# robotvisionmu/DenseMonoSLAM

Hardware: AMD Instinct MI355X
Metric: frames/sec ICP+RGB+fusion @640x480 (higher is better)
Workload: dtype f32; 1 GPU; TUM fr1/desk-like 640x480 full 3-level ICP+RGB tracking (SO3 + {10,5,4} GN iterations) + surfel index-map fusion; synthetic box-room RGB-D stream, loop closure off (--o), NID keyframing off (--nkf); cameras_per_gpu=1, n_pred=2, n_pred_project_passes=1, surfels_per_map=246557, surfels_total=246557, exchange=none (1 camera)

## Files before the change

densemonoslam_amd/csrc/fill.hpp:

```cpp
#pragma once
#include "surfel.hpp"

namespace dms {

struct FillArgs {
  const float4* ex_vertex;
  const float4* ex_normal;
  const uchar4* ex_image;
  const unsigned short* depth;
  const uchar4* rgba;
  const unsigned* mirror_src;
  unsigned* mirror_dst;
  int mirror_words;
  int* dense_flag;
  int rows_blocks;
  unsigned* dense_cnt;
  const unsigned* sample_mask;
  unsigned char* thumb_block;
  const unsigned* thumb_mask;
  int thumb_w, thumb_h;
  const float* thumb_pose_src;
  float* thumb_pose_dst;
  int* thumb_tick_dst;
  int thumb_tick;
  float4* out_vertex;
  float4* out_normal;
  uchar4* out_image;
  int cols, rows;
  float cx, cy, ifx, ify;
  int pass_geom, pass_rgb;
};

__device__ __forceinline__ f3 fill_vertex_at(const FillArgs& a, int sx, int sy, int x, int y) {
  const float z = (float)a.depth[(size_t)sy * a.cols + sx] / 1000.0f;
  return mk3((((float)x - a.cx) * z) * a.ifx, (((float)y - a.cy) * z) * a.ify, z);
}

__device__ __forceinline__ void fill_pixel_out(const FillArgs& a, int px, int py, const float4& sv, const float4& sn, const uchar4& si, float4& ov,
                                               float4& on, uchar4& oi) {
  const size_t i = (size_t)py * a.cols + px;
  const float colsf = (float)a.cols, rowsf = (float)a.rows;
  const float tcx = ((float)px + 0.5f) / colsf, tcy = ((float)py + 0.5f) / rowsf;
  const int x = (int)(tcx * colsf), y = (int)(tcy * rowsf);
  {
    if (sv.z == 0.f || a.pass_geom == 1) {
      const f3 v = fill_vertex_at(a, px, py, x, y);
      ov = make_float4(v.x, v.y, v.z, 1.f);
    } else {
      ov = sv;
    }
    a.out_vertex[i] = ov;
  }
  {
    if (sn.z == 0.f || a.pass_geom == 1) {
      const f3 v = fill_vertex_at(a, px, py, x, y);
      const int sxp = texel(tcx + (1.0f / colsf), colsf, a.cols);
      const int syp = texel(tcy + (1.0f / rowsf), rowsf, a.rows);
      const f3 vx = fill_vertex_at(a, sxp, py, x + 1, y);
      const f3 vy = fill_vertex_at(a, px, syp, x, y + 1);
      const f3 n = normalized3(cross3(vx - v, vy - v));
      on = make_float4(n.x, n.y, n.z, 1.f);
    } else {
      on = sn;
    }
    a.out_normal[i] = on;
  }
  {
    if ((si.x == 0 && si.y == 0 && si.z == 0) || a.pass_rgb == 1)
      oi = a.rgba[i];
    else
      oi = si;
    a.out_image[i] = oi;
  }
}
__device__ __forceinline__ void fill_pixel(const FillArgs& a, int px, int py, const float4& sv, const float4& sn, const uchar4& si) {
  float4 ov, on;
  uchar4 oi;
  fill_pixel_out(a, px, py, sv, sn, si, ov, on, oi);
}

__device__ __forceinline__ void fill_thumb(const FillArgs& a, int px, int py, const float4& ov, const float4& on, const uchar4& oi) {
  const unsigned cw = a.thumb_mask[px >> 5], rw = a.thumb_mask[64 + (py >> 5)];
  if (!((cw >> (px & 31)) & (rw >> (py & 31)) & 1u)) return;
  const int i = (int)a.thumb_mask[128 + (px >> 5)] + __popc(cw & ((1u << (px & 31)) - 1u));
  const int j = (int)a.thumb_mask[192 + (py >> 5)] + __popc(rw & ((1u << (py & 31)) - 1u));
  const size_t n = (size_t)a.thumb_w * a.thumb_h, k = (size_t)j * a.thumb_w + i;
  reinterpret_cast<uchar4*>(a.thumb_block)[k] = oi;
  reinterpret_cast<float4*>(a.thumb_block + thumb_vertex_off(n))[k] = ov;
  reinterpret_cast<float4*>(a.thumb_block + thumb_normal_off(n))[k] = on;
}

inline bool thumb_sample_masks(int cols, int rows, unsigned* words256) {
  for (int i = 0; i < 256; ++i) words256[i] = 0u;
  const int tw = cols / 8, th = rows / 8;
  if (tw < 1 || th < 1 || cols > 2048 || rows > 2048) return false;
  int last = -1;
  for (int i = 0; i < tw; ++i) {
    const int sx = texel(((float)i + 0.5f) / (float)tw, (float)cols, cols);
    if (sx <= last) return false;
    last = sx;
    words256[sx >> 5] |= 1u << (sx & 31);
  }
  last = -1;
  for (int j = 0; j < th; ++j) {
    const int sy = texel(((float)j + 0.5f) / (float)th, (float)rows, rows);
    if (sy <= last) return false;
    last = sy;
    words256[64 + (sy >> 5)] |= 1u << (sy & 31);
  }
  for (int w = 1; w < 64; ++w) {
    words256[128 + w] = words256[128 + w - 1] + (unsigned)__builtin_popcount(words256[w - 1]);
    words256[192 + w] = words256[192 + w - 1] + (unsigned)__builtin_popcount(words256[64 + w - 1]);
  }
  return true;
}

inline void fill_sample_masks(int cols, int rows, unsigned* words128) {
  for (int i = 0; i < 128; ++i) words128[i] = 0u;
  const int dw = cols / 20, dh = rows / 20;
  for (int i = 0; i < dw; ++i) {
    const int sx = texel(((float)i + 0.5f) / (float)dw, (float)cols, cols);
    words128[sx >> 5] |= 1u << (sx & 31);
  }
  for (int j = 0; j < dh; ++j) {
    const int sy = texel(((float)j + 0.5f) / (float)dh, (float)rows, rows);
    words128[64 + (sy >> 5)] |= 1u << (sy & 31);
  }
}

template <int NT>
__device__ __forceinline__ void fill_dense_test(const FillArgs& a, int t, int* s_sum ) {
  const int dw = a.cols / 20, dh = a.rows / 20;
  int sum = 0;
  for (int k = t; k < dw * dh; k += NT) {
    const int i = k % dw, j = k / dw;
    const float u = ((float)i + 0.5f) / (float)dw, v = ((float)j + 0.5f) / (float)dh;
    const int sx = texel(u, (float)a.cols, a.cols), sy = texel(v, (float)a.rows, a.rows);
    const uchar4 c = a.ex_image[(size_t)sy * a.cols + sx];
    sum += (c.x > 0 && c.y > 0 && c.z > 0) ? 1 : 0;
  }
  for (int off = 32; off > 0; off >>= 1) sum += __shfl_down(sum, off, 64);
  if ((t & 63) == 0) s_sum[t >> 6] = sum;
  __syncthreads();
  if (t == 0) {
    int tot = 0;
    for (int w = 0; w < NT / 64; ++w) tot += s_sum[w];
    const bool dense = (float)tot / (float)(dh * dw) > 0.95f;
    *a.dense_flag = dense ? 0 : 1;
  }
}

__device__ __forceinline__ int dense_from_counters(const unsigned* cnt, int samples) {
  unsigned tot = 0;
#pragma unroll
  for (int k = 0; k < 16; ++k) tot += cnt[k * 16];
  return ((float)(int)tot / (float)samples > 0.95f) ? 0 : 1;
}

}
```

densemonoslam_amd/csrc/fusion_frame.hip:

```cpp
#include <atomic>
#include <chrono>
#include <map>
#include <string>
#include <vector>

#include "../../include/dmslam_render_cloud.h"
#include "internal.hpp"
#include "host_util.hpp"
#include "late_frame.hpp"
#include "smallmath.hpp"
#include "surfel.hpp"
#include "canon.hpp"
#include "frame_state.hpp"
#include "live_bodies.hpp"
#include "fill.hpp"
#include "track_init.hpp"

namespace dms {

__global__ void k_rgb_to_rgba(const unsigned char* __restrict__ rgb, uchar4* __restrict__ rgba, int n) {
  for (int i = blockIdx.x * blockDim.x + threadIdx.x; i < n; i += blockDim.x * gridDim.x)
    rgba[i] = make_uchar4(rgb[3 * i + 0], rgb[3 * i + 1], rgb[3 * i + 2], 255);
}

// ... 153 lines not shown
  char* gloop = nullptr;
  char* h_gloop = nullptr;
  size_t gloop_bytes = 0;
  LoopState* loop = nullptr;
  char* h_loop = nullptr;
  size_t loop_bytes = 0;
  char* arena = nullptr;
  size_t arena_bytes = 0;
  struct LiveImages {
    dms_image2d rgba, depth_raw, depth_filtered, depth_metric, depth_metric_filtered;
  } live[2];
  dms_image2d rgba, depth_raw, depth_filtered, depth_metric, depth_metric_filtered;
  hipStream_t s_prep = nullptr;
  hipEvent_t ev_prep_done[2] = {nullptr, nullptr}, ev_main_done[4] = {nullptr, nullptr, nullptr, nullptr}, ev_inputs = nullptr;
  bool fused_live = true;
  int prep_blocks = 38;
  LateFrame late;
  int late_owner = -1;
  double host_wait_prep_ms = 0.0;
  int host_lag = 2;
  bool inputs_armed = false;
  int last_prep = -1;
  long frames = 0;
  dms_image2d kf_img[DMS_NUM_PYRS], kf_dmap[DMS_NUM_PYRS], kf_old_img[DMS_NUM_PYRS], kf_old_dmap[DMS_NUM_PYRS];
  void* nid_ws = nullptr;
  size_t nid_ws_bytes = 0;
  float* nid_host = nullptr;
  int frames_since_fusion = 0;
  float last_nid = 0.f;
  bool loop_solver = false;
  int graph_sample_rate = 5000;
  dms_deform* deform = nullptr;
  int deforms = 0;
  std::vector<float> relative_cons;
  bool in_frame = false, cur_bootstrap = false, cur_fuse_now = true;
  int live_set = 0, lastnext_set = 0;
  bool prev_handed_on = false;
  bool tracking_ok = true, lost = false;
  int tracking_count = 0;
  int cur_k2 = 0;
  dms_image2d depth_synth;
  dms_indexmap_out imap;
  dms_predict_out pred, fill;
  void* rgba_tmp = nullptr;
  void* untr = nullptr;
  unsigned long long* zbuf = nullptr;
  unsigned long long* zbuf2 = nullptr;
  unsigned long long* zbuf_assoc = nullptr;
  bool zbuf_assoc_dirty = false;
  bool zbuf_assoc_keep_dirty = false;
  unsigned* tickets = nullptr;
  bool fold_track_init = true;
  bool dense_by_counters = false;
  double host_wait_ms = 0.0;
  bool pre_valid = false;
  int pre_tick = 0;
  unsigned long pre_version = 0;
  struct LazyRecord {
    bool pending = false;
    float confidence = 0.f, maxDepth = 0.f;
    int tick = 0, timeIdx = 0, timeDelta = 0;
    int pass_geom = 0, pass_rgb = 0;
    dms_image2d depth_filtered, rgba;
    dms_model* model = nullptr;
    unsigned long version = 0;
    hipStream_t stream = nullptr;
  } lazy;
  dms_pose_block* lazy_pose = nullptr;
  bool lazy_observed = false;
  long lazy_deferred = 0, lazy_materialised = 0, lazy_stale = 0;
  FrameState* state = nullptr;
  FrameState* h_state_dev = nullptr;
  FrameState* h_state = nullptr;
  int last_slot = 0;
  int timeouts_reported = 0;
  int range_failures_reported = 0;
  void* h_track = nullptr;
  int tick = 1;
  bool map_initialised = false;
  int fused_last = 0;
  bool profiling = false;
  StageClock clock;
};

namespace {

dms_image2d mk_img(void* p, int rows, int cols, size_t elem) {
  dms_image2d i;
  i.data = p;
  i.pitch = (size_t)cols * elem;
  i.rows = rows;
  i.cols = cols;
  return i;
}

void layout(dms_fusion* f, Carver& c) {
  const int W = f->p.width, H = f->p.height;
  const size_t N = (size_t)W * H;
  for (int k = 0; k < 2; ++k) {
    f->live[k].rgba = mk_img(c.take(N * 4), H, W, 4);
    f->live[k].depth_raw = mk_img(c.take(N * 2), H, W, 2);
    f->live[k].depth_filtered = mk_img(c.take(N * 2), H, W, 2);
    f->live[k].depth_metric = mk_img(c.take(N * 4), H, W, 4);
    f->live[k].depth_metric_filtered = mk_img(c.take(N * 4), H, W, 4);
  }
  f->rgba = f->live[0].rgba;
// ... 1 lines not shown
  f->depth_filtered = f->live[0].depth_filtered;
  f->depth_metric = f->live[0].depth_metric;
  f->depth_metric_filtered = f->live[0].depth_metric_filtered;
  f->fb_rgba = mk_img(c.take(N * 4), H, W, 4);
  f->fb_dm = mk_img(c.take(N * 4), H, W, 4);
  f->fb_dmf = mk_img(c.take(N * 4), H, W, 4);
  f->imap.index = mk_img(c.take(N * 4), H, W, 4);
  f->imap.vertConf = mk_img(c.take(N * 16), H, W, 16);
  f->imap.colorTime = mk_img(c.take(N * 16), H, W, 16);
  f->imap.normRad = mk_img(c.take(N * 16), H, W, 16);
  f->pred.image = mk_img(c.take(N * 4), H, W, 4);
  f->pred.vertex = mk_img(c.take(N * 16), H, W, 16);
  f->pred.normal = mk_img(c.take(N * 16), H, W, 16);
  f->pred.time = mk_img(c.take(N * 2), H, W, 2);
  f->fill.image = mk_img(c.take(N * 4), H, W, 4);
  f->fill.vertex = mk_img(c.take(N * 16), H, W, 16);
  f->fill.normal = mk_img(c.take(N * 16), H, W, 16);
  f->fill.time = f->pred.time;
  for (int l = 0; l < DMS_NUM_PYRS; ++l) {
    const int h = H >> l, w = W >> l;
    f->kf_img[l] = mk_img(c.take((size_t)h * w), h, w, 1);
    f->kf_dmap[l] = mk_img(c.take((size_t)h * w * 4), h, w, 4);
    f->kf_old_img[l] = mk_img(c.take((size_t)h * w), h, w, 1);
    f->kf_old_dmap[l] = mk_img(c.take((size_t)h * w * 4), h, w, 4);
  }
  {
    const int nb = f->p.nid_bins_depth > f->p.nid_bins_img ? f->p.nid_bins_depth : f->p.nid_bins_img;
    f->nid_ws_bytes = nid_workspace_bytes(nb > 0 ? nb : 1);
    f->nid_ws = c.take(f->nid_ws_bytes);
  }
  memset(&f->pred_old, 0, sizeof(f->pred_old));
  if (f->p.local_loop_closure || f->p.hybrid_loops) {
    f->pred_old.image = mk_img(c.take(N * 4), H, W, 4);
    f->pred_old.vertex = mk_img(c.take(N * 16), H, W, 16);
    f->pred_old.normal = mk_img(c.take(N * 16), H, W, 16);
    f->pred_old.time = mk_img(c.take(N * 2), H, W, 2);
  }
  if (f->p.hybrid_loops) {
    f->gloop_bytes = 256 + (size_t)(W / 20) * (H / 20) * 8 * sizeof(float);
    f->gloop = (char*)c.take(f->gloop_bytes);
    f->orb_pose = (dms_pose_block*)c.take(2 * sizeof(dms_pose_block));
  }
  if (f->p.local_loop_closure) {
    f->loop_bytes = up256(sizeof(LoopState)) + (size_t)(W / 20) * (H / 20) * 8 * sizeof(float);
    f->loop = (LoopState*)c.take(f->loop_bytes);
  }
  f->depth_synth = mk_img(c.take(N * 4), H, W, 4);
  f->rgba_tmp = c.take(N * 4);
  f->untr = c.take(N * 16);
  f->zbuf = (unsigned long long*)c.take(N * 8);
  f->zbuf2 = (unsigned long long*)c.take(N * 8);
  f->zbuf_assoc = (unsigned long long*)c.take(N * 8);
  f->tickets = (unsigned*)c.take(2048 + 512 + 1024);
  f->state = (FrameState*)c.take(sizeof(FrameState));
  f->lazy_pose = (dms_pose_block*)c.take(sizeof(dms_pose_block));
}

void drain(dms_fusion* f) {
  static const bool timeline = getenv("DMS_TIMELINE") != nullptr;
  if (timeline && !f->clock.pending.empty()) {
    hipEvent_t base = f->clock.pending.front().start;
    for (auto& p : f->clock.pending) {
      float a = 0.f, b = 0.f;
      (void)hipEventElapsedTime(&a, base, p.start);
      (void)hipEventElapsedTime(&b, base, p.stop);
      fprintf(stderr, "[timeline] %-14s %9.3f -> %9.3f ms\n", p.name.c_str(), a, b);
    }
  }
  f->clock.drain();
}

enum class Predict { view, final, tracking };
struct PredictOpts {
  float confidence;
  void* state_mirror = nullptr;
  bool one_call = false;
  bool have_prior = false;
  const TrackInitArgs* track_init = nullptr;
  bool* track_init_taken = nullptr;
};

int predict_body(dms_fusion* f, hipStream_t s, Predict kind, const PredictOpts& o) {
  const bool dense_test = kind == Predict::tracking;
  int rc;
  f->lazy.pending = false;
  FillArgs fa;
  const FillArgs* fused = nullptr;
  if ((rc = fill_args(&f->pred, &f->depth_filtered, &f->rgba, &f->cam, f->lost ? 1 : 0, (f->lost || f->p.frameToFrameRGB) ? 1 : 0, &f->fill,
                      o.state_mirror ? f->state : nullptr, o.state_mirror, (int)sizeof(FrameState), dense_test ? &f->state->fill_in : nullptr, &fa)))
    return rc;
  f->dense_by_counters = false;
  if (f->p.fused_fill_in && f->p.width <= 2048 && f->p.height <= 2048 && (!dense_test || f->p.hybrid_tracking)) {
    fused = &fa;
    if (dense_test) {
      fa.dense_cnt = f->tickets;
      fa.sample_mask = f->tickets + 512;
      f->dense_by_counters = true;
    }
    if (kind == Predict::final && f->armed_now.block && f->thumb_masks_ok) {
      fa.thumb_block = f->armed_now.block;
      fa.thumb_mask = f->tickets + 640;
      fa.thumb_w = f->p.width / 8;
      fa.thumb_h = f->p.height / 8;
      fa.thumb_pose_src = f->state->cur.pose;
      fa.thumb_pose_dst = f->armed_now.pose_dst;
      fa.thumb_tick_dst = f->armed_now.tick_dst;
      fa.thumb_tick = f->armed_now.tick;
      f->armed_written = true;
    }
  }
  {
    StageTimer t(f->clock, s, "predict", f->profiling);
    const int W = f->p.width, H = f->p.height;
    bool done = false;
    if (kind == Predict::tracking && f->pre_valid) {
      if (!o.have_prior && f->pre_tick == f->tick && f->pre_version == f->model->version) {
        if ((rc = splat_predict(f->model, &f->state->cur, &f->cam, f->p.maxDepthProcessed, o.confidence, f->tick, f->p.timeIdx, f->tick,
                                f->p.timeDelta, 1, f->zbuf2, &f->pred, nullptr, 1, s, nullptr, nullptr, 1, fused, fused ? o.track_init : nullptr)))
          return rc;
        done = true;
      } else if ((rc = clear_zbuf(f->zbuf2, W * H, s))) {
        return rc;
      }
      f->pre_valid = false;
    }
    if (!done) {
      const int next_tick = f->lost ? f->tick : f->tick + 1;
      const float second[3] = {0.7f, (float)next_tick, (float)next_tick};
      const bool dual = kind == Predict::final && f->p.share_projection && f->p.hybrid_tracking && f->model->sharers == 1;
      if (dual && f->pre_valid && (rc = clear_zbuf(f->zbuf2, W * H, s))) return rc;
      const bool defer = dual && o.one_call && fused && o.state_mirror && f->p.lazy_final_prediction && !f->lazy_observed && !f->armed_now.block &&
                         !f->p.nid_keyframing && !f->p.local_loop_closure && !f->p.hybrid_loops && !f->lost && !f->cur_bootstrap;
      if (defer) {
        const ProjectRider rider = {(const unsigned*)f->state, (unsigned*)o.state_mirror, (int)(sizeof(FrameState) / 4),
                                    (const unsigned*)&f->state->cur, (unsigned*)f->lazy_pose, (int)(sizeof(dms_pose_block) / 4)};
        if ((rc = splat_project_only(f->model, &f->state->cur, &f->cam, f->p.maxDepthProcessed, second[0], next_tick, f->p.timeIdx, next_tick,
                                     f->p.timeDelta, 1, f->zbuf2, s, &rider)))
          return rc;
        dms_fusion::LazyRecord& r = f->lazy;
        r.pending = true;
        r.confidence = o.confidence;
        r.maxDepth = f->p.maxDepthProcessed;
        r.tick = f->tick;
        r.timeIdx = f->p.timeIdx;
        r.timeDelta = f->p.timeDelta;
        r.pass_geom = 0;
        r.pass_rgb = f->p.frameToFrameRGB ? 1 : 0;
        r.depth_filtered = f->depth_filtered;
        r.rgba = f->rgba;
        r.model = f->model;
        r.version = f->model->version;
        r.stream = s;
        f->lazy_deferred += 1;
      } else if ((rc = splat_predict(f->model, &f->state->cur, &f->cam, f->p.maxDepthProcessed, o.confidence, f->tick, f->p.timeIdx, f->tick,
                              f->p.timeDelta, 1, f->zbuf, &f->pred, nullptr, 1, s, dual ? second : nullptr, dual ? f->zbuf2 : nullptr, 0,
                              fused, fused ? o.track_init : nullptr)))
        return rc;
      if (dual) {
        f->pre_valid = true;
        f->pre_tick = next_tick;
        f->pre_version = f->model->version;
      }
    }
  }
  if (o.track_init_taken) *o.track_init_taken = fused != nullptr && o.track_init && o.track_init->blocks > 0;
  if (!fused) {
    StageTimer t(f->clock, s, "fill_in", f->profiling);
    if ((rc = fill_in(&f->pred, &f->depth_filtered, &f->rgba, &f->cam, f->lost ? 1 : 0, (f->lost || f->p.frameToFrameRGB) ? 1 : 0, &f->fill,
                      s, o.state_mirror ? f->state : nullptr, o.state_mirror, (int)sizeof(FrameState), dense_test ? &f->state->fill_in : nullptr)))
      return rc;
  }
  return DMS_OK;
}

int predict_view(dms_fusion* f, float confidence, hipStream_t s) { return predict_body(f, s, Predict::view, PredictOpts{confidence}); }

int predict_tracking(dms_fusion* f, hipStream_t s, bool have_prior, const TrackInitArgs* track_init, bool* track_init_taken) {
  return predict_body(f, s, Predict::tracking, PredictOpts{0.7f, nullptr, false, have_prior, track_init, track_init_taken});
}

int predict_final(dms_fusion* f, hipStream_t s, void* state_mirror, bool one_call) {
  return predict_body(f, s, Predict::final, PredictOpts{f->p.confidence, state_mirror, one_call});
}

int materialise_final_prediction(dms_fusion* f, hipStream_t consumer, bool consumer_known) {
  f->lazy_observed = true;
  if (!f->lazy.pending) return DMS_OK;
  const dms_fusion::LazyRecord r = f->lazy;
  f->lazy.pending = false;
  f->lazy_materialised += 1;
  if (r.model != f->model || r.version != f->model->version) f->lazy_stale += 1;
  int rc;
  FillArgs fa;
  if ((rc = fill_args(&f->pred, &r.depth_filtered, &r.rgba, &f->cam, r.pass_geom, r.pass_rgb, &f->fill, nullptr, nullptr, 0, nullptr, &fa))) return rc;
  {
    StageTimer t(f->clock, r.stream, "predict", f->profiling);
    if ((rc = splat_predict(f->model, f->lazy_pose, &f->cam, r.maxDepth, r.confidence, r.tick, r.timeIdx, r.tick, r.timeDelta, 1, f->zbuf, &f->pred,
                            nullptr, 1, r.stream, nullptr, nullptr, 0, &fa, nullptr)))
      return rc;
  }
  if (!consumer_known || consumer != r.stream) DMS_HIP(hipStreamSynchronize(r.stream));
  return DMS_OK;
}

int global_loop_device(dms_fusion* f, const float* orbTcwOld, const float* orbTcwNew, int active_new, hipStream_t s) {
  int rc;
  Pose16 a, b;
  memcpy(a.v, orbTcwOld, sizeof(a.v));
  memcpy(b.v, orbTcwNew, sizeof(b.v));
  hipLaunchKernelGGL(k_pose_blocks2, dim3(1), dim3(64), 0, s, f->orb_pose, a, b);
  DMS_CHECK_LAUNCH();
  f->lazy.pending = false;
  StageTimer t(f->clock, s, "global_loop", f->profiling);
  const int act = active_new ? 1 : 0;
  if ((rc = splat_predict(f->model, f->orb_pose + act, &f->cam, f->p.maxDepthProcessed, f->p.confidence, f->tick, f->p.timeIdx, f->tick,
                          f->p.timeDelta, 1, f->zbuf, &f->pred, nullptr, 1, s)))
    return rc;
  if ((rc = splat_predict(f->model, f->orb_pose + (1 - act), &f->cam, f->p.maxDepthProcessed, f->p.confidence, 0, f->p.timeIdx,
                          f->tick - f->p.timeDelta, f->p.timeDelta, 0, f->zbuf, &f->pred_old, nullptr, 1, s)))
    return rc;
  hipLaunchKernelGGL(k_global_loop_constraints, dim3(1), dim3(256), 0, s, (const float4*)f->pred.vertex.data,
                     (const unsigned short*)f->pred_old.time.data, f->p.width, f->p.height, f->p.maxDepthProcessed, f->orb_pose, active_new ? 1 : 0,
                     (int*)f->gloop, (float*)(f->gloop + 256));
  DMS_CHECK_LAUNCH();
  DMS_HIP(hipMemcpyAsync(f->h_gloop, f->gloop, f->gloop_bytes, hipMemcpyDeviceToHost, s));
  f->gloop_ran = true;
  return DMS_OK;
}

}

// ... 46 lines not shown
                           unsigned char* slot_flag, unsigned int* winner, size_t winner_count, dms_stream s) {
  return model_fuse_scratch(m, slot_pos4, slot_col4, slot_nrm4, slot_best, slot_flag, winner, winner_count, (hipStream_t)s);
}
int dms_model_clean(dms_model* m, const dms_pose_block* pose, int time, int timeIdx, const dms_indexmap_out* im,
                    const dms_image2d* depth_synth, const dms_camera* cam, float confThreshold, const float* graph_host, int graph_nodes,
                    int timeDelta, float maxDepth, int isFern, dms_stream s) {
  return model_clean(m, pose, time, timeIdx, im, depth_synth, cam, confThreshold, graph_host, graph_nodes, timeDelta, maxDepth, isFern, 0,
                     nullptr, (hipStream_t)s);
}
int dms_fill_in(const dms_predict_out* ex, const dms_image2d* d, const dms_image2d* rgba, const dms_camera* cam, int pg, int pr,
                dms_predict_out* out, dms_stream s) {
  return fill_in(ex, d, rgba, cam, pg, pr, out, (hipStream_t)s);
}
int dms_resize_nn(const dms_image2d* src, dms_image2d* dst, int elem, dms_stream s) { return resize_nn(src, dst, elem, (hipStream_t)s); }

void dms_fusion_default_params(dms_fusion_params* p, int width, int height, float fx, float fy, float cx, float cy) {
  if (!p) return;
  memset(p, 0, sizeof(*p));
  p->width = width;
  p->height = height;
  p->fx = fx;
  p->fy = fy;
  p->cx = cx;
  p->cy = cy;
  p->timeDelta = 200;
  p->confidence = 10.0f;
  p->depthCut = 3.0f;
  p->icpWeight = 10.0f;
  p->fastOdom = 0;
  p->so3 = 1;
  p->frameToFrameRGB = 0;
  p->pyramid = 1;
  p->hybrid_tracking = 1;
  p->rgbOnly = 0;
  p->timeIdx = 0;
  p->maxDepthProcessed = 25.0f;
  p->model_capacity = 0;
  p->pipeline_ingest = 1;
  p->global_predict = 0;
  p->nid_keyframing = 0;
  p->nid_threshold = 0.80f;
  p->nid_depth_lambda = 0.7f;
  p->nid_bins_img = 64;
  p->nid_bins_depth = 500;
  p->nid_pyramid_level = 0;
  p->local_loop_closure = 0;
  p->reloc = 0;
  p->num_sensors = 3;
  p->share_projection = 1;
  p->fused_fill_in = 1;
  p->hybrid_loops = 0;
  p->lazy_final_prediction = 1;
  p->fused_associate = 1;
}

static int set_depth_bias(dms_fusion* f) {
  const int b = canon::depth_exp_bias(f->p.depthCut);
  int rc = dms_odometry_debug_set(f->odom, "depth_exp_bias", b);
  if (!rc && f->odom_m2m) rc = dms_odometry_debug_set(f->odom_m2m, "depth_exp_bias", b);
  return rc;
}

static std::atomic<int> g_live_contexts{0};
int dms_fusion_allow_late_frame(dms_fusion* f, int allow) {
  DMS_REQUIRE(f && allow >= -1 && allow <= 1, "bad argument");
  f->late_owner = allow;
  return DMS_OK;
}

int dms_fusion_create(dms_fusion** out, const dms_fusion_params* p) {
  DMS_REQUIRE(out && p, "null argument");
  DMS_REQUIRE(p->width >= 40 && p->height >= 40, "resolution too small");
  DMS_REQUIRE(p->timeIdx >= 0 && p->timeIdx < DMS_MAX_SENSORS, "timeIdx out of range");
  DMS_REQUIRE(p->num_sensors >= 0 && p->num_sensors <= DMS_MAX_SENSORS, "num_sensors out of range");
  DMS_REQUIRE(p->timeIdx < (p->num_sensors == 0 ? 3 : p->num_sensors), "timeIdx must be one of the num_sensors time slots");
  DMS_REQUIRE(!p->nid_keyframing || (p->nid_bins_img >= 1 && p->nid_bins_img <= 256 && p->nid_bins_depth >= 1 && p->nid_bins_depth <= 4096 &&
                                     p->nid_pyramid_level >= 0 && p->nid_pyramid_level < DMS_NUM_PYRS),
              "bad NID key-framing parameters");
  dms_fusion* f = new dms_fusion();
  f->p = *p;
  f->cam.fx = p->fx;
  f->cam.fy = p->fy;
  f->cam.cx = p->cx;
  f->cam.cy = p->cy;
  if (f->p.num_sensors == 0) f->p.num_sensors = 3;
  int rc = dms_model_create(&f->model, p->model_capacity, p->width, p->height);
  if (rc) {
    delete f;
    return rc;
  }
  (void)dms_model_set_num_sensors(f->model, f->p.num_sensors);
  f->own_model = f->model;
  f->clusters[0] = f->model;
  rc = dms_odometry_create(&f->odom, p->width, p->height, p->cx, p->cy, p->fx, p->fy, 0.f, 0.f);
  if (rc) {
    dms_model_destroy(f->own_model ? f->own_model : f->model);
    delete f;
    return rc;
  }
  rc = odometry_enable_ring(f->odom);
  if (!rc && p->local_loop_closure) rc = dms_odometry_create(&f->odom_m2m, p->width, p->height, p->cx, p->cy, p->fx, p->fy, 0.f, 0.f);
  if (!rc) rc = set_depth_bias(f);
  if (!rc && f->odom_m2m) odometry_set_early_exit(f->odom_m2m, 1);
  if (rc) {
    dms_odometry_destroy(f->odom);
    dms_model_destroy(f->own_model ? f->own_model : f->model);
    delete f;
    return rc;
  }
  Carver sz;
  sz.pad = 16;
  layout(f, sz);
  f->arena_bytes = up256(sz.off);
  hipError_t e = hipMalloc((void**)&f->arena, f->arena_bytes);
  if (e == hipSuccess) {
    int prio = 1;
    if (const char* pp = getenv("DMS_PREP_PRIORITY")) prio = atoi(pp);
    int least = 0, greatest = 0;
    if (prio != 0 && hipDeviceGetStreamPriorityRange(&least, &greatest) == hipSuccess && least != greatest)
      e = hipStreamCreateWithPriority(&f->s_prep, hipStreamNonBlocking, prio > 0 ? least : greatest);
    else
      e = hipStreamCreateWithFlags(&f->s_prep, hipStreamNonBlocking);
  }
  for (int k = 0; k < 2 && e == hipSuccess; ++k) e = hipEventCreateWithFlags(&f->ev_prep_done[k], hipEventDisableTiming);
  for (int k = 0; k < 4 && e == hipSuccess; ++k) e = hipEventCreateWithFlags(&f->ev_main_done[k], hipEventDisableTiming);
  {
    const int tiles = ((p->width + 63) / 64) * ((p->height + 15) / 16);
    int cap = 40;
    const int free_cus = odometry_free_cus(f->odom);
    if (free_cus >= 16 && free_cus < cap) cap = free_cus;
    const int rounds = (tiles + cap - 1) / cap;
    f->prep_blocks = (tiles + rounds - 1) / rounds;
  }
  if (const char* pb = getenv("DMS_PREP_BLOCKS")) f->prep_blocks = atoi(pb);
  if (const char* fl = getenv("DMS_FUSED_LIVE")) f->fused_live = atoi(fl) != 0;
  if (const char* ft = getenv("DMS_FOLD_TRACK_INIT")) f->fold_track_init = atoi(ft) != 0;
  if (const char* hl = getenv("DMS_HOST_LAG")) f->host_lag = atoi(hl) == 3 ? 3 : 2;
  if (const char* lm = getenv("DMS_LATE_MAIN")) f->late.forced = atoi(lm) != 0 ? 1 : 0;
  if (const char* lz = getenv("DMS_LAZY_FINAL_PREDICTION")) f->p.lazy_final_prediction = atoi(lz) != 0 ? 1 : 0;
  if (const char* fa = getenv("DMS_FUSED_ASSOCIATE")) f->p.fused_associate = atoi(fa) != 0 ? 1 : 0;
  if (e == hipSuccess) e = hipEventCreateWithFlags(&f->ev_inputs, hipEventDisableTiming);
  if (e == hipSuccess) e = hipMemset(f->arena, 0, f->arena_bytes);
  if (e == hipSuccess) e = hipHostMalloc((void**)&f->h_state, 4 * sizeof(FrameState), hipHostMallocMapped);
  if (e == hipSuccess) e = hipHostGetDevicePointer((void**)&f->h_state_dev, f->h_state, 0);
  if (e == hipSuccess) e = hipHostMalloc((void**)&f->nid_host, 2 * sizeof(float), hipHostMallocDefault);
  if (e == hipSuccess && f->loop_bytes) {
    e = hipHostMalloc((void**)&f->h_loop, 4 * f->loop_bytes, hipHostMallocDefault);
    if (e == hipSuccess) memset(f->h_loop, 0, 4 * f->loop_bytes);
  }
  if (e == hipSuccess && f->gloop_bytes) {
    e = hipHostMalloc((void**)&f->h_gloop, f->gloop_bytes, hipHostMallocDefault);
    if (e == hipSuccess) memset(f->h_gloop, 0, f->gloop_bytes);
  }
  if (e != hipSuccess) {
    if (f->arena) (void)hipFree(f->arena);
    if (f->odom_m2m) dms_odometry_destroy(f->odom_m2m);
    dms_odometry_destroy(f->odom);
    dms_model_destroy(f->own_model ? f->own_model : f->model);
    delete f;
    return hip_fail(e, "dms_fusion_create allocation", __FILE__, __LINE__);
  }
  Carver c;
  c.base = f->arena;
  c.pad = 16;
  layout(f, c);
  {
    unsigned masks[128];
    fill_sample_masks(p->width < 2048 ? p->width : 2048, p->height < 2048 ? p->height : 2048, masks);
    (void)hipMemcpy(f->tickets + 512, masks, sizeof(masks), hipMemcpyHostToDevice);
    unsigned tm[256];
    f->thumb_masks_ok = thumb_sample_masks(p->width, p->height, tm);
    (void)hipMemcpy(f->tickets + 640, tm, sizeof(tm), hipMemcpyHostToDevice);
  }
  Pose16 I;
  for (int i = 0; i < 16; ++i) I.v[i] = (i % 5 == 0) ? 1.f : 0.f;
  hipLaunchKernelGGL(k_pose_set, dim3(1), dim3(64), 0, 0, f->state, I);
  (void)clear_zbuf(f->zbuf, p->width * p->height, 0);
  (void)clear_zbuf(f->zbuf2, p->width * p->height, 0);
  (void)clear_zbuf(f->zbuf_assoc, p->width * p->height, 0);
  for (int l = 0; l < DMS_NUM_PYRS; ++l)
    (void)hipMemsetD32((hipDeviceptr_t)f->kf_old_dmap[l].data, 0x7fffffff, (size_t)f->kf_old_dmap[l].rows * f->kf_old_dmap[l].cols);
  (void)hipDeviceSynchronize();
  memset(f->h_state, 0, 4 * sizeof(FrameState));
  g_live_contexts += 1;
  *out = f;
  return DMS_OK;
}

int dms_fusion_destroy(dms_fusion* f) {
  if (!f) return DMS_OK;
  g_live_contexts -= 1;
  (void)hipDeviceSynchronize();
  drain(f);
  for (int k = 0; k < 2; ++k)
    if (f->ev_prep_done[k]) (void)hipEventDestroy(f->ev_prep_done[k]);
  for (int k = 0; k < 4; ++k)
    if (f->ev_main_done[k]) (void)hipEventDestroy(f->ev_main_done[k]);
  if (f->ev_inputs) (void)hipEventDestroy(f->ev_inputs);
  if (f->s_prep) (void)hipStreamDestroy(f->s_prep);
  if (f->arena) (void)hipFree(f->arena);
  if (f->h_state) (void)hipHostFree(f->h_state);
  if (f->nid_host) (void)hipHostFree(f->nid_host);
  if (f->h_loop) (void)hipHostFree(f->h_loop);
  if (f->h_gloop) (void)hipHostFree(f->h_gloop);
  if (f->odom_m2m) dms_odometry_destroy(f->odom_m2m);
  if (f->deform) dms_deform_destroy(f->deform);
  dms_odometry_destroy(f->odom);
  dms_model* const own = f->own_model ? f->own_model : f->model;
  if (f->model && f->model != own) f->model->sharers -= 1;
  for (auto& kv : f->clusters)
    if (kv.second && kv.second != own) dms_model_destroy(kv.second);
  dms_model_destroy(own);
  delete f;
  return DMS_OK;
}

static int snapshot_feedback(dms_fusion* f, hipStream_t s) {
  const size_t N = (size_t)f->p.width * f->p.height;
  DMS_HIP(hipMemcpyAsync(f->fb_rgba.data, f->rgba.data, N * 4, hipMemcpyDeviceToDevice, s));
  DMS_HIP(hipMemcpyAsync(f->fb_dm.data, f->depth_metric.data, N * 4, hipMemcpyDeviceToDevice, s));
  DMS_HIP(hipMemcpyAsync(f->fb_dmf.data, f->depth_metric_filtered.data, N * 4, hipMemcpyDeviceToDevice, s));
  f->fb_time = f->tick;
  f->fb_valid = true;
  return DMS_OK;
}
// ... 207 lines not shown

static int join_prep_stream(dms_fusion* f, int k2, hipStream_t s, hipStream_t sp) {
  DMS_HIP(hipEventRecord(f->ev_prep_done[k2], sp));
  if (f->late.on) {
    const auto t0 = std::chrono::steady_clock::now();
    DMS_HIP(hipEventSynchronize(f->ev_prep_done[k2]));
    f->host_wait_prep_ms += std::chrono::duration<double, std::milli>(std::chrono::steady_clock::now() - t0).count();
  } else {
    DMS_HIP(hipStreamWaitEvent(s, f->ev_prep_done[k2], 0));
  }
  f->last_prep = k2;
  return DMS_OK;
}

static int bootstrap_frame(dms_fusion* f, const float* inPose16, hipStream_t s) {
  int rc;
  Pose16 prior;
  if (inPose16)
    memcpy(prior.v, inPose16, sizeof(prior.v));
  else
    for (int i = 0; i < 16; ++i) prior.v[i] = (i % 5 == 0) ? 1.f : 0.f;
  hipLaunchKernelGGL(k_pose_set, dim3(1), dim3(64), 0, s, f->state, prior);
  DMS_CHECK_LAUNCH();
  if (!f->adopting) {
    StageTimer t(f->clock, s, "initialise", f->profiling);
    if ((rc = model_initialise(f->model, &f->rgba, &f->depth_metric, &f->depth_metric_filtered, &f->cam, f->tick, f->p.timeIdx,
                               (float)(int)f->p.maxDepthProcessed, s)))
      return rc;
    if ((rc = snapshot_feedback(f, s))) return rc;
    if (f->req_cluster != f->cur_cluster && !f->clusters.count(f->req_cluster) && f->model == f->own_model) {
      f->clusters[f->cur_cluster] = nullptr;
      f->clusters[f->req_cluster] = f->model;
      f->cur_cluster = f->req_cluster;
    }
  }
  f->map_initialised = true;
  f->prev_handed_on = true;
  return DMS_OK;
}

static int track_frame(dms_fusion* f, const float* inPose16, float weightMultiplier, hipStream_t s) {
  int rc;
  if (inPose16) {
    Pose16 prior;
    memcpy(prior.v, inPose16, sizeof(prior.v));
    hipLaunchKernelGGL(k_frame_begin, dim3(1), dim3(64), 0, s, f->state, prior, 1);
    DMS_CHECK_LAUNCH();
  }
  const TrackFold fold = {f->state->cur.pose, f->p.pyramid, f->p.fastOdom, f->p.so3, 0};
  TrackInitArgs early;
  memset(&early, 0, sizeof(early));
  bool early_taken = false;
  const bool want_early = f->p.hybrid_tracking && f->fold_track_init && !f->lost && odometry_early_init_args(f->odom, &fold, &early) != 0;
  if ((rc = predict_tracking(f, s, inPose16 != nullptr, want_early ? &early : nullptr, &early_taken))) return rc;
  if (want_early && !early_taken) odometry_early_init_args(f->odom, nullptr, &early);
  if (!f->p.hybrid_tracking) {
    hipLaunchKernelGGL(k_frame_after_track, dim3(1), dim3(64), 0, s, f->state, weightMultiplier);
    DMS_CHECK_LAUNCH();
    return DMS_OK;
  }
  {
    StageTimer t(f->clock, s, "odom_init", f->profiling);
    if ((rc = odometry_initModel_fused(f->odom, f->pred.vertex.data, f->pred.normal.data, f->pred.image.data, f->fill.vertex.data,
                                       f->fill.normal.data, f->fill.image.data, &f->state->fill_in, f->p.frameToFrameRGB ? 1 : 0,
                                       f->state->cur.pose, s, 1,
                                       f->dense_by_counters ? f->tickets : nullptr, (f->p.width / 20) * (f->p.height / 20),
                                       f->fold_track_init ? &fold : nullptr)))
      return rc;
    odometry_alias_next_depth(f->odom);
  }
  {
    StageTimer t(f->clock, s, "track", f->profiling);
    if ((rc = odometry_track_enqueue(f->odom, nullptr, nullptr, f->state->cur.pose, f->p.rgbOnly, f->p.icpWeight, f->p.pyramid,
                                     f->p.fastOdom, f->p.so3, 0, s, f->state, weightMultiplier)))
      return rc;
    f->prev_handed_on = f->p.so3 != 0;
  }
  return DMS_OK;
}

static int check_relocalisation(dms_fusion* f, hipStream_t s) {
  int rc;
  dms_track_result tr;
  if ((rc = dms_odometry_fetch_result(f->odom, &tr, s))) return rc;
  f->tracking_ok = (double)tr.lastICPError < 1e-04;
  if (f->lost) return DMS_OK;
  double cov[36];
  if ((rc = dms_odometry_getCovariance(f->odom, cov))) return rc;
  for (int i = 0; i < 6; ++i)
    if (cov[i * 7] > 1e-04) {
      f->tracking_ok = false;
      break;
    }
  if (!f->tracking_ok) {
    f->tracking_count += 1;
    if (f->tracking_count > 10) f->lost = true;
  } else {
    f->tracking_count = 0;
  }
  return DMS_OK;
}

static int local_loop_candidate(dms_fusion* f, hipStream_t s) {
  int rc;
  {
    StageTimer t(f->clock, s, "predict_old", f->profiling);
    if ((rc = splat_predict(f->model, &f->state->cur, &f->cam, f->p.maxDepthProcessed, f->p.confidence, 0, f->p.timeIdx,
                            f->tick - f->p.timeDelta, f->p.timeDelta, 0, f->zbuf, &f->pred_old, nullptr, 1, s)))
      return rc;
  }
  {
    StageTimer t(f->clock, s, "loop_init", f->profiling);
    if ((rc = odometry_initModel_fused(f->odom_m2m, f->pred_old.vertex.data, f->pred_old.normal.data, f->pred_old.image.data,
                                       f->pred_old.vertex.data, f->pred_old.normal.data, f->pred_old.image.data, &f->state->fill_in, 0,
                                       f->state->cur.pose, s)))
      return rc;
// ... 170 lines not shown
      if ((rc = fuse_measurements(f, s))) return rc;
      if ((rc = index_map_for_clean(f, timeDeltaEff, s))) return rc;
      if (graph_nodes > 0 && (rc = synthesise_depth(f, timeDeltaEff, s))) return rc;
      if ((rc = clean_map(f, graph_host, graph_dev, graph_nodes, timeDeltaEff, s))) return rc;
      surfels_written = true;
      fused = 1;
    }
    f->frames_since_fusion = fuse_now ? 0 : f->frames_since_fusion + 1;
  }
  if (!surfels_written) {
    hipLaunchKernelGGL(k_frame_end, dim3(1), dim3(64), 0, s, f->state, f->model->d_count);
    DMS_CHECK_LAUNCH();
  }
  const int k4 = (int)(f->frames % 4);
  if ((rc = predict_final(f, s, f->h_state_dev + k4, one_call))) return rc;
  f->last_slot = k4;
  DMS_HIP(hipEventRecord(f->ev_main_done[k4], s));
  f->fused_last = fused;
  if (!f->lost) f->tick += 1;
  f->frames += 1;
  return DMS_OK;
}

static int close_local_loop(dms_fusion* f, hipStream_t s, const float** table_dev, int* nodes, const float** est_pose) {
  *nodes = 0;
  DMS_HIP(hipStreamSynchronize(s));
  const char* slot = f->h_loop + (size_t)f->last_slot * f->loop_bytes;
  const LoopState* L = (const LoopState*)slot;
  if (!L->ok || L->n_constraints <= 0) return DMS_OK;
  int rc;
  if ((rc = dms_deform_sample_model(f->deform, f->model, f->graph_sample_rate, (dms_stream)s))) return rc;
  if ((rc = dms_deform_clear_constraints(f->deform))) return rc;
  const float* rows = (const float*)((const char*)f->loop + up256(sizeof(LoopState)));
  if ((rc = deform_add_rows(f->deform, rows, 8, L->n_constraints, f->tick, f->deforms == 0, s))) return rc;
  if ((rc = dms_deform_constrain(f->deform, f->tick, 0, (dms_stream)s))) return rc;
  dms_deform_result res;
  const float* rel = nullptr;
  if ((rc = deform_fetch(f->deform, &res, &rel))) return rc;
  if (!res.applied || res.nodes <= 0) return DMS_OK;
  const int* count_dev;
  if ((rc = dms_deform_graph_device(f->deform, table_dev, &count_dev))) return rc;
  *nodes = res.nodes;
  *est_pose = L->est_pose;
  f->deforms += 1;
  const int n = res.relative_rows, step = n / 3 > 0 ? n / 3 : 1;
  for (int i = 0; i < n; i += step) f->relative_cons.insert(f->relative_cons.end(), rel + (size_t)i * 8, rel + (size_t)(i + 1) * 8);
  return DMS_OK;
}

int dms_fusion_process_frame(dms_fusion* f, const void* rgb_dev, int rgb_channels, const unsigned short* depth_dev, const float* inPose16,
                             float weightMultiplier, dms_stream st) {
  DMS_REQUIRE(!f || !f->loop_solver || (f->model->sharers == 1 && f->clusters.size() == 1 && f->req_cluster == 0),
              "the loop solver needs a map this camera owns alone, without clusters");
  int rc = dms_fusion_process_frame_begin(f, rgb_dev, rgb_channels, depth_dev, inPose16, weightMultiplier, st);
  if (rc) return rc;
  if (f->loop_solver && f->p.local_loop_closure && !f->cur_bootstrap && !f->lost) {
    const float* table_dev = nullptr;
    const float* est_pose = nullptr;
    int nodes = 0;
    if ((rc = close_local_loop(f, (hipStream_t)st, &table_dev, &nodes, &est_pose))) {
      const int rc_end = process_frame_end(f, nullptr, 0, nullptr, st, true);
      (void)rc_end;
      return rc;
    }
    if (nodes > 0) return process_frame_end(f, nullptr, nodes, est_pose, st, true, table_dev);
  }
  return process_frame_end(f, nullptr, 0, nullptr, st, true);
}

int dms_fusion_set_loop_solver(dms_fusion* f, int on, int sampleRate) {
  DMS_REQUIRE(f, "null argument");
  DMS_REQUIRE(!f->in_frame, "between process_frame_begin and _end");
  if (!on) {
    f->loop_solver = false;
    return DMS_OK;
  }
  if (sampleRate <= 0) sampleRate = 5000;
  DMS_REQUIRE(sampleRate >= 2, "sampleRate below 2");
  DMS_REQUIRE(f->p.local_loop_closure, "the context was created without local_loop_closure");
  DMS_REQUIRE(f->model == f->clusters[0] && f->model->sharers == 1 && f->clusters.size() == 1 && f->req_cluster == 0,
              "the loop solver needs a map this camera owns alone, without clusters");
  const int cons = (f->p.width / 20) * (f->p.height / 20);
  DMS_REQUIRE(cons >= 1 && cons <= DMS_DEFORM_MAX_CONSTRAINTS, "the frame size gives more constraint samples than the solver takes");
  if (!f->deform) {
    if (int rc = dms_deform_create(&f->deform, DMS_DEFORM_MAX_NODES - 1, cons)) return rc;
  }
  f->loop_solver = true;
  f->graph_sample_rate = sampleRate;
  return DMS_OK;
}

dms_deform* dms_fusion_deformation(dms_fusion* f) { return f ? f->deform : nullptr; }
int dms_fusion_get_deforms(dms_fusion* f) { return f ? f->deforms : 0; }
int dms_fusion_get_relative_constraints(dms_fusion* f, float* rows8_host, int max_rows, int* n) {
  DMS_REQUIRE(f && n && (rows8_host || max_rows == 0), "null argument");
  *n = (int)(f->relative_cons.size() / 8);
  for (int i = 0; i < *n && i < max_rows; ++i) memcpy(rows8_host + (size_t)i * 8, f->relative_cons.data() + (size_t)i * 8, 8 * sizeof(float));
  return DMS_OK;
}

int dms_fusion_process_frame_end(dms_fusion* f, const float* graph_host, int graph_nodes, const float* newPose16, dms_stream st) {
  return process_frame_end(f, graph_host, graph_nodes, newPose16, st, false);
}

int dms_fusion_get_lazy_stats(dms_fusion* f, int* eager, long* deferred, long* materialised, long* stale) {
  DMS_REQUIRE(f, "null argument");
  if (eager) *eager = (f->p.lazy_final_prediction && !f->lazy_observed) ? 0 : 1;
  if (deferred) *deferred = f->lazy_deferred;
  if (materialised) *materialised = f->lazy_materialised;
  if (stale) *stale = f->lazy_stale;
  return DMS_OK;
}

static int report_timeouts(dms_fusion* f, const FrameState* hs) {
  if (hs->track_range_failures != f->range_failures_reported) {
    const int n = hs->track_range_failures - f->range_failures_reported;
    f->range_failures_reported = hs->track_range_failures;
    if (hs->track_timeouts == f->timeouts_reported) {
      set_error("dms_fusion: %d frame(s) since the last fetch found no fixed-point range for a cross-pixel sum of the tracker (non-finite "
                "input maps?); those frames kept their prior pose and were not fused", n);
      return DMS_ERR_TIMEOUT;
    }
  }
  if (hs->track_timeouts == f->timeouts_reported) return DMS_OK;
  const int n = hs->track_timeouts - f->timeouts_reported;
  f->timeouts_reported = hs->track_timeouts;
  (void)dms_odometry_fall_back_to_launches(f->odom);
  if (f->odom_m2m) (void)dms_odometry_fall_back_to_launches(f->odom_m2m);
  set_error("dms_fusion: %d frame(s) since the last fetch had a resident tracker kernel time out at a grid-wide wait (its blocks were not "
            "all on the device: another process on this GPU?); those frames kept their prior pose and were not fused.  "
            "This camera's trackers have switched to launch-per-phase kernels (DMS_TRACK_MODE=launches)",
            n);
  return DMS_ERR_TIMEOUT;
}

static void fill_loop(const dms_fusion* f, dms_frame_result* r) {
  r->tracking_ok = f->tracking_ok ? 1 : 0;
  r->lost = f->lost ? 1 : 0;
  if (!f->h_loop || f->lost) return;
  const LoopState* L = (const LoopState*)(f->h_loop + (size_t)f->last_slot * f->loop_bytes);
  r->loop_ok = L->ok;
  r->loop_constraints = L->n_constraints;
  r->loop_icp_error = L->icp_error;
  r->loop_icp_count = L->icp_count;
  memcpy(r->loop_pose, L->est_pose, sizeof(r->loop_pose));
  memcpy(r->loop_cov_diag, L->cov_diag, sizeof(r->loop_cov_diag));
}

int dms_fusion_fetch_loop(dms_fusion* f, dms_frame_result* r, dms_stream st) {
  DMS_REQUIRE(f && r, "null argument");
  DMS_REQUIRE(f->in_frame && (f->p.local_loop_closure || f->gloop_ran),
              "only between process_frame_begin and _end, with local_loop_closure or after dms_fusion_set_orb_loop");
  memset(r, 0, sizeof(*r));
  DMS_HIP(hipStreamSynchronize((hipStream_t)st));
  if (f->cur_bootstrap) return DMS_OK;
  if (!(f->p.local_loop_closure && !f->lost)) {
    const int k4 = (int)(f->frames % 4);
    DMS_HIP(hipMemcpyAsync(f->h_state + k4, f->state, sizeof(FrameState), hipMemcpyDeviceToHost, (hipStream_t)st));
    DMS_HIP(hipStreamSynchronize((hipStream_t)st));
    f->last_slot = k4;
  }
  const FrameState* hs = f->h_state + f->last_slot;
  memcpy(r->pose, hs->cur.pose, sizeof(r->pose));
// ... 364 lines not shown
```

densemonoslam_amd/csrc/fusion_map.hip:

```cpp
#include <vector>

#include "exact_arith.hpp"
#include "scan.hpp"
#include "smallmath.hpp"
#include "surfel.hpp"
#include "fill.hpp"
#include "internal.hpp"
#include "host_util.hpp"
#include "track_init.hpp"

namespace dms {

static void model_layout(dms_model* m, Carver& c) {
  for (int b = 0; b < 2; ++b) {
    m->buf[b].pos = c.take<float4>(m->cap);
    m->buf[b].col = c.take<float4>(m->cap);
    m->buf[b].nrm = c.take<float4>(m->cap);
    m->buf[b].times = c.take<float>(m->cap * DMS_MAX_SENSORS);
  }
  m->d_count = c.take<unsigned>(8);
  m->d_count_alt = m->d_count ? m->d_count + 4 : nullptr;
  m->slot_pos = c.take<float4>(m->slots);
  m->slot_col = c.take<float4>(m->slots);
  m->slot_nrm = c.take<float4>(m->slots);
  m->slot_best = c.take<unsigned>(m->slots);
  m->slot_flag = c.take<unsigned char>(m->slots);
  m->winner = c.take<unsigned>(m->cap);
  const size_t total = m->cap + (size_t)m->width * m->height;
  m->keep = c.take<unsigned char>(total);
  m->block_count = c.take<unsigned>(total / kScanChunk + 2);
  m->block_offset = c.take<unsigned>(total / kScanChunk + 2);
  m->clean_first = c.take<unsigned>(4);
  m->nodes = c.take<float>((size_t)m->max_nodes * 16);
}

__global__ void k_fill_u32(unsigned* p, size_t n, unsigned v) {
  for (size_t i = blockIdx.x * (size_t)blockDim.x + threadIdx.x; i < n; i += (size_t)blockDim.x * gridDim.x) p[i] = v;
}

}

using namespace dms;

extern "C" {

int dms_model_create(dms_model** out, size_t capacity, int width, int height) {
  DMS_REQUIRE(out && width >= 16 && height >= 16, "bad argument");
  dms_model* m = new dms_model();
  m->cap = capacity ? capacity : (size_t)5700 * 5700;
  m->width = width;
  m->height = height;
  m->slot_h = (height + 1) / 2;
  m->slots = ((width + 1) / 2) * m->slot_h;
  Carver sz;
  model_layout(m, sz);
  m->arena_bytes = up256(sz.off);
  hipError_t e = hipMalloc((void**)&m->arena, m->arena_bytes);
  if (e != hipSuccess) {
    delete m;
    return hip_fail(e, "hipMalloc(model)", __FILE__, __LINE__);
  }
  Carver c;
// ... 879 lines not shown
        else
          hi = mid;
      }
      const int j = lo;
      SplatSurfel s;
      s.pos = mk3(s_par[0][j], s_par[1][j], s_par[2][j]);
      s.nrm = mk3(s_par[3][j], s_par[4][j], s_par[5][j]);
      s.rad = s_par[6][j];
      const int x0 = s_box[0][j], w = s_box[1][j];
      const int py = s_box[2][j] + (int)(u - s_off[j]);
      const unsigned long long id = (unsigned long long)(base + (unsigned)j);
      const int pass = DUAL ? s_box[3][j] : 1;
      const float dyn = (((float)py + 0.5f) - s_par[8][j]) * (1.f / a.fy);
      const float left = s_par[9][j] - dyn * dyn;
      if (left < 0.f) continue;
      const float rx = fminf(sqrtf(left) * a.fx, 1.0e9f), xwc = s_par[7][j];
      const int xa = max(x0, (int)ceilf(fmaxf(xwc - rx - 0.5f, -1.0e9f)));
      const int xb = min(x0 + w - 1, (int)floorf(fminf(xwc + rx - 0.5f, 1.0e9f)));
      const bool use1 = !DUAL || (pass & 1), use2 = DUAL && (pass & 2);
      for (int px0 = xa; px0 <= xb; px0 += 4) {
        unsigned long long z1[4], z2[4];
#pragma unroll
        for (int k = 0; k < 4; ++k) {
          const int px = px0 + k;
          const size_t q = (size_t)px * a.rows + py;
          const bool in = px <= xb;
          z1[k] = (in && use1) ? zbuf[q] : 0ull;
          z2[k] = (in && use2) ? zbuf2[q] : 0ull;
        }
        unsigned long long key[4];
#pragma unroll
        for (int k = 0; k < 4; ++k) {
          const int px = px0 + k;
          key[k] = ~0ull;
          f3 c;
          float zw;
          if (px <= xb && splat_fragment_lean(ray, a, s, px, py, c, zw)) {
            const unsigned d = depth24(zw);
            if (d < 0xFFFFFFu) key[k] = ((unsigned long long)d << 32) | id;
          }
        }
#pragma unroll
        for (int k = 0; k < 4; ++k) {
          const size_t q = (size_t)(px0 + k) * a.rows + py;
          if (key[k] < z1[k]) atomicMin(zbuf + q, key[k]);
          if (DUAL && key[k] < z2[k]) atomicMin(zbuf2 + q, key[k]);
        }
      }
    }
    __syncthreads();
  }
}

template <bool DEPTH_ONLY, bool FILL>
__global__ __launch_bounds__(256) void k_splat_resolve(ProjArgs a, SurfelPlanes sp, size_t cap, unsigned long long* __restrict__ zbuf,
                                                       uchar4* __restrict__ image, float4* __restrict__ vertex, float4* __restrict__ normal,
                                                       unsigned short* __restrict__ timeImg, float* __restrict__ depthOut, int clear_after,
                                                       FillArgs fa, TrackInitArgs ti) {
  const unsigned nres = gridDim.x - (FILL ? (unsigned)ti.blocks : 0u);
  if (FILL && blockIdx.x >= nres) {
    track_init_body((int)(blockIdx.x - nres), ti.blocks, (int)threadIdx.x, (int)blockDim.x, ti.st, ti.prior, ti.prior_pose16, ti.fx, ti.fy, ti.cx, ti.cy,
                    ti.so3, ti.first_level, ti.sync_words, ti.n_sync, ti.inject_timeout, nullptr);
    return;
  }
  if (FILL) {
    if (fa.mirror_words > 0 && blockIdx.x == 0 && (int)threadIdx.x < fa.mirror_words) fa.mirror_dst[threadIdx.x] = fa.mirror_src[threadIdx.x];
    if (fa.thumb_block && blockIdx.x == 0) {
      if (fa.thumb_pose_dst && threadIdx.x < 16) fa.thumb_pose_dst[threadIdx.x] = fa.thumb_pose_src[threadIdx.x];
      if (fa.thumb_tick_dst && threadIdx.x == 16) *fa.thumb_tick_dst = fa.thumb_tick;
    }
  }
  const int tiles_y = (a.rows + 7) >> 3, tiles_x = (a.cols + 7) >> 3, ntiles = tiles_x * tiles_y;
  const int lane = threadIdx.x & 63, wave = threadIdx.x >> 6, waves_per_block = blockDim.x >> 6;
  for (int t = xcd_block(blockIdx.x, nres, a.xcd) * waves_per_block + wave; t < ntiles; t += nres * waves_per_block) {
    const int tx = t / tiles_y, ty = t - tx * tiles_y;
    const int px = tx * 8 + (lane >> 3), py = ty * 8 + (lane & 7);
    if (px >= a.cols || py >= a.rows) continue;
    const int p = py * a.cols + px;
    const unsigned long long key = zbuf[(size_t)px * a.rows + py];
    if (clear_after) zbuf[(size_t)px * a.rows + py] = kZClear;
    bool sampled = false;
    if (FILL) {
      if (fa.dense_cnt) sampled = ((fa.sample_mask[px >> 5] >> (px & 31)) & (fa.sample_mask[64 + (py >> 5)] >> (py & 31)) & 1u) != 0u;
    }
    if ((unsigned)(key >> 32) >= 0xFFFFFFu) {
      if (DEPTH_ONLY) {
        depthOut[p] = 0.f;
      } else {
        image[p] = make_uchar4(0, 0, 0, 0);
        vertex[p] = make_float4(0.f, 0.f, 0.f, 0.f);
        normal[p] = make_float4(0.f, 0.f, 0.f, 0.f);
        timeImg[p] = 0;
        if (FILL) {
          float4 ov, on;
          uchar4 oi;
          fill_pixel_out(fa, px, py, make_float4(0.f, 0.f, 0.f, 0.f), make_float4(0.f, 0.f, 0.f, 0.f), make_uchar4(0, 0, 0, 0), ov, on, oi);
          if (fa.thumb_block) fill_thumb(fa, px, py, ov, on, oi);
        }
      }
      continue;
    }
    const unsigned i = (unsigned)(key & 0xFFFFFFFFull);
    SplatSurfel s;
    splat_vertex(a, sp.pos[i], sp.nrm + i, sp.times[(size_t)a.timeIdx * cap + i], s);
    f3 c;
    float zw;
    splat_fragment(a, s, px, py, c, zw);
    if (DEPTH_ONLY) {
      depthOut[p] = c.z;
      continue;
    }
    const float4 cc = sp.col[i];
    const f3 rgb = decode_color(cc.x);
    const uchar4 o_img = make_uchar4((unsigned char)f2i_rn(rgb.x * 255.0f), (unsigned char)f2i_rn(rgb.y * 255.0f),
                                     (unsigned char)f2i_rn(rgb.z * 255.0f), 255);
    image[p] = o_img;
    if (FILL && sampled && o_img.x > 0 && o_img.y > 0 && o_img.z > 0) atomicAdd(fa.dense_cnt + ((px + py) & 15) * 16, 1u);
    const float z = c.z;
    const float fcx = (float)px + 0.5f, fcy = (float)py + 0.5f;
    const float4 o_v = make_float4(((fcx - a.cx) * z) * (1.f / a.fx), ((fcy - a.cy) * z) * (1.f / a.fy), z, s.conf);
    const float4 o_n = make_float4(s.nrm.x, s.nrm.y, s.nrm.z, s.rad);
    vertex[p] = o_v;
    normal[p] = o_n;
    const float tz = cc.z;
    unsigned tv = tz > 0.f ? (unsigned)f2i_rz(tz) : 0u;
    if (tv > 65535u) tv = 65535u;
    timeImg[p] = (unsigned short)tv;
    if (FILL) {
      float4 ov, on;
      uchar4 oi;
      fill_pixel_out(fa, px, py, o_v, o_n, o_img, ov, on, oi);
      if (fa.thumb_block) fill_thumb(fa, px, py, ov, on, oi);
    }
  }
}

int splat_predict(dms_model* m, const dms_pose_block* pose, const dms_camera* cam, float maxDepth, float confThreshold, int time,
                  int timeIdx, int maxTime, int timeDelta, int active, unsigned long long* zbuf, dms_predict_out* out,
                  dms_image2d* depth_out, int zclean, hipStream_t s, const float* second_conf_time_maxtime, unsigned long long* zbuf2,
                  int resolve_only, const FillArgs* fill, const TrackInitArgs* init) {
  DMS_REQUIRE(m && pose && cam && zbuf, "null argument");
  DMS_REQUIRE(!init || init->blocks == 0 || (fill && !depth_out), "the tracker set-up rides on the fused resolve + fill-in pass only");
  DMS_REQUIRE(!m->pending_update, "a deferred update pass is still pending (index_map applies it)");
  DMS_REQUIRE(timeIdx >= 0 && timeIdx < DMS_MAX_SENSORS, "timeIdx out of range");
  DMS_REQUIRE(fabsf(cam->fx) > 1e-18f && fabsf(cam->fx) < 1e18f && fabsf(cam->fy) > 1e-18f && fabsf(cam->fy) < 1e18f && maxDepth > 1e-18f && maxDepth < 1e18f,
              "focal lengths and depth cut-off must be finite, non-zero and within 1e-18 .. 1e18");
  const int W = m->width, H = m->height;
  if (depth_out)
    DMS_REQUIRE(dense_img(*depth_out, 4, W, H), "depth target must be dense W×H f32");
  else
    DMS_REQUIRE(out && dense_img(out->image, 4, W, H) && dense_img(out->vertex, 16, W, H) && dense_img(out->normal, 16, W, H) &&
                    dense_img(out->time, 2, W, H),
                "prediction targets must be dense W×H");
  ProjArgs a;
  fill_proj(a, m, pose, cam, maxDepth, time, timeIdx, timeDelta);
  a.confThreshold = confThreshold;
  a.maxTime = maxTime;
  a.actv = active ? 1 : 0;
  const int n = W * H;
  if (!zclean) {
    hipLaunchKernelGGL(k_clear_zbuf, dim3(min((n + 255) / 256, 2048)), dim3(256), 0, s, zbuf, n);
    DMS_CHECK_LAUNCH();
  }
  SplatSecond b2 = {0.f, 0, 0};
  const ProjectRider no_rider = {nullptr, nullptr, 0, nullptr, nullptr, 0};
  if (resolve_only) {
  } else if (second_conf_time_maxtime && zbuf2) {
    b2.confThreshold = second_conf_time_maxtime[0];
    b2.time = (int)second_conf_time_maxtime[1];
    b2.maxTime = (int)second_conf_time_maxtime[2];
    hipLaunchKernelGGL(k_splat_project<true>, dim3(surfel_grid(m->count_upper)), dim3(256), 0, s, a, m->buf[m->cur], m->cap, m->d_count, zbuf, b2,
                       zbuf2, no_rider);
  } else {
    hipLaunchKernelGGL(k_splat_project<false>, dim3(surfel_grid(m->count_upper)), dim3(256), 0, s, a, m->buf[m->cur], m->cap, m->d_count, zbuf,
                       b2, (unsigned long long*)nullptr, no_rider);
  }
  DMS_CHECK_LAUNCH();
  const FillArgs no_fill = {};
  TrackInitArgs no_init;
  memset(&no_init, 0, sizeof(no_init));
  const dim3 rg(min((n + 255) / 256, 2048));
  if (depth_out) {
    hipLaunchKernelGGL((k_splat_resolve<true, false>), rg, dim3(256), 0, s, a, m->buf[m->cur], m->cap, zbuf, (uchar4*)nullptr,
                       (float4*)nullptr, (float4*)nullptr, (unsigned short*)nullptr, (float*)depth_out->data, zclean, no_fill, no_init);
  } else if (fill) {
    DMS_REQUIRE(fill->ex_image == (const uchar4*)out->image.data && fill->ex_vertex == (const float4*)out->vertex.data &&
                    fill->ex_normal == (const float4*)out->normal.data && fill->cols == W && fill->rows == H &&
                    (!fill->dense_cnt || (fill->sample_mask && W <= 2048 && H <= 2048)) && fill->mirror_words <= 256,
                "fill-in arguments do not describe this prediction");
    const TrackInitArgs& ti = (init && init->blocks > 0) ? *init : no_init;
    hipLaunchKernelGGL((k_splat_resolve<false, true>), dim3(rg.x + ti.blocks), dim3(256), 0, s, a, m->buf[m->cur], m->cap, zbuf, (uchar4*)out->image.data,
                       (float4*)out->vertex.data, (float4*)out->normal.data, (unsigned short*)out->time.data, (float*)nullptr, zclean, *fill, ti);
  } else {
    hipLaunchKernelGGL((k_splat_resolve<false, false>), rg, dim3(256), 0, s, a, m->buf[m->cur], m->cap, zbuf, (uchar4*)out->image.data,
                       (float4*)out->vertex.data, (float4*)out->normal.data, (unsigned short*)out->time.data, (float*)nullptr, zclean, no_fill, no_init);
  }
  DMS_CHECK_LAUNCH();
  return DMS_OK;
}

int splat_project_only(dms_model* m, const dms_pose_block* pose, const dms_camera* cam, float maxDepth, float confThreshold, int time,
                       int timeIdx, int maxTime, int timeDelta, int active, unsigned long long* zbuf, hipStream_t s, const ProjectRider* rider) {
  DMS_REQUIRE(m && pose && cam && zbuf, "null argument");
  DMS_REQUIRE(!m->pending_update, "a deferred update pass is still pending (index_map applies it)");
  DMS_REQUIRE(timeIdx >= 0 && timeIdx < DMS_MAX_SENSORS, "timeIdx out of range");
  DMS_REQUIRE(fabsf(cam->fx) > 1e-18f && fabsf(cam->fx) < 1e18f && fabsf(cam->fy) > 1e-18f && fabsf(cam->fy) < 1e18f && maxDepth > 1e-18f && maxDepth < 1e18f,
              "focal lengths and depth cut-off must be finite, non-zero and within 1e-18 .. 1e18");
  DMS_REQUIRE(!rider || (rider->mirror_words >= 0 && rider->mirror_words <= 256 && rider->copy_words >= 0 && rider->copy_words <= 256 &&
                         (rider->mirror_words == 0 || (rider->mirror_src && rider->mirror_dst)) &&
                         (rider->copy_words == 0 || (rider->copy_src && rider->copy_dst))),
              "a rider copies at most 256 dwords (one block)");
  ProjArgs a;
  fill_proj(a, m, pose, cam, maxDepth, time, timeIdx, timeDelta);
  a.confThreshold = confThreshold;
  a.maxTime = maxTime;
  a.actv = active ? 1 : 0;
  const SplatSecond b2 = {0.f, 0, 0};
  const ProjectRider no_rider = {nullptr, nullptr, 0, nullptr, nullptr, 0};
  hipLaunchKernelGGL(k_splat_project<false>, dim3(surfel_grid(m->count_upper)), dim3(256), 0, s, a, m->buf[m->cur], m->cap, m->d_count, zbuf,
                     b2, (unsigned long long*)nullptr, rider ? *rider : no_rider);
  DMS_CHECK_LAUNCH();
  return DMS_OK;
}

}

extern "C" {
int dms_model_consume(dms_model* dst, const dms_model* src, const float* relativeTransform16, dms_stream s) {
  return dms::model_consume(dst, src, relativeTransform16, (hipStream_t)s);
}
int dms_model_consume_records(dms_model* dst, const float* records_dev, unsigned int count, const float* relativeTransform16, dms_stream s) {
  return dms::model_consume_records(dst, records_dev, count, relativeTransform16, (hipStream_t)s);
}
int dms_model_export_records(dms_model* m, float* records_dev, unsigned int max_count, unsigned int* count, dms_stream s) {
  return dms::model_export_records(m, records_dev, max_count, count, (hipStream_t)s);
}
}
// ... 1 lines not shown
```

densemonoslam_amd/csrc/internal.hpp:

```cpp
#pragma once
#include "common.hpp"
#include "../../include/dmslam_deform.h"
#include "../../include/dmslam_render_panels.h"

namespace dms {


struct TrackInitArgs;
struct FillArgs;
struct FrameState;
struct LoopState;

struct ProjectRider {
  const unsigned* mirror_src;
  unsigned* mirror_dst;
  int mirror_words;
  const unsigned* copy_src;
  unsigned* copy_dst;
  int copy_words;
};

int pyrDown(const dms_image2d* src, dms_image2d* dst, hipStream_t s);
int createVMap(const dms_camera* intr, const dms_image2d* depth, dms_image2d* vmap, float cutoff, hipStream_t s);
int createNMap(const dms_image2d* vmap, dms_image2d* nmap, hipStream_t s);
int transformMaps(const dms_image2d* vs, const dms_image2d* ns, const dms_mat33* R, const dms_float3* t, dms_image2d* vd,
                  dms_image2d* nd, hipStream_t s);
int copyMaps(const float* vsrc, const float* nsrc, dms_image2d* vd, dms_image2d* nd, hipStream_t s);
int resizeMap(const dms_image2d* in, dms_image2d* out, bool normalize, hipStream_t s);
int pyrDownGaussF(const dms_image2d* src, dms_image2d* dst, hipStream_t s);
int pyrDownUcharGauss(const dms_image2d* src, dms_image2d* dst, hipStream_t s);
int verticesToDepth(const float* vsrc, dms_image2d* dst, float cutOff, hipStream_t s);
int modelPyramidFused(const void* vA, const void* nA, const void* iA, const void* vB, const void* nB, const void* iB, const int* flag_dev,
                      int force_b_img, const float* pose16_dev, dms_image2d* vmaps, dms_image2d* nmaps, dms_image2d* depths,
                      dms_image2d* images, float cutOff, hipStream_t s, bool skip_last_step = false, const unsigned* dense_cnt = nullptr,
                      int dense_samples = 0, int* flag_out = nullptr, const TrackInitArgs* init = nullptr);
int verticesToDepth2D(const dms_image2d* vsrc, dms_image2d* dst, float cutOff, hipStream_t s);
int imageToIntensity(const dms_image2d* rgba, dms_image2d* dst, hipStream_t s);
int derivativeGate(const dms_image2d* src, dms_image2d* dx, dms_image2d* dy, dms_image2d* gate, float minScale, hipStream_t s);
int derivativeImages(const dms_image2d* src, dms_image2d* dx, dms_image2d* dy, hipStream_t s);
int projectToPointCloud(const dms_image2d* depth, dms_image2d* cloud, const dms_camera* intr, int level, hipStream_t s);
int liveLevelsFused(const dms_image2d* depth, const dms_image2d* vmap, const dms_image2d* nmap, const dms_image2d* image, const dms_image2d* dx,
                    const dms_image2d* dy, const dms_image2d* gate, const dms_camera* cam0, float cutoff, const float* minScale, hipStream_t s);
int selectCopy16(void* dst, const void* a, const void* b, const int* flag_dev, int force_b, size_t n16, hipStream_t s);
int transformMapsDev(dms_image2d* v, dms_image2d* n, const float* pose16_dev, hipStream_t s);

size_t reduce_workspace_bytes();
int icpStep(const dms_mat33* Rcurr, const dms_float3* tcurr, const dms_image2d* vmap_curr, const dms_image2d* nmap_curr,
            const dms_mat33* Rprev_inv, const dms_float3* tprev, const dms_camera* intr, const dms_image2d* vmap_g_prev,
            const dms_image2d* nmap_g_prev, float distThres, float angleThres, void* workspace, size_t workspace_bytes, float* A,
            float* b, float* residual, int threads, int blocks, hipStream_t s);
int rgbStep(const dms_image2d* corresImg, float sigma, const dms_image2d* cloud, float fx, float fy, const dms_image2d* dIdx,
            const dms_image2d* dIdy, float sobelScale, void* workspace, size_t workspace_bytes, float* A, float* b, int threads,
            int blocks, hipStream_t s);
int computeRgbResidual(float minScale, const dms_image2d* dIdx, const dms_image2d* dIdy, const dms_image2d* lastDepth,
                       const dms_image2d* nextDepth, const dms_image2d* lastImage, const dms_image2d* nextImage,
                       dms_image2d* corresImg, void* workspace, size_t workspace_bytes, float maxDepthDelta, const dms_float3* kt,
                       const dms_mat33* krkinv, int* sigmaSum, int* count, int threads, int blocks, hipStream_t s);
int so3Step(const dms_image2d* lastImage, const dms_image2d* nextImage, const dms_mat33* imageBasis, const dms_mat33* kinv,
            const dms_mat33* krlr, void* workspace, size_t workspace_bytes, float* A, float* b, float* residual, int threads,
            int blocks, hipStream_t s);

int depth_bilateral(const dms_image2d* src, dms_image2d* dst, float maxD, hipStream_t s, int narrow_blocks = 0,
                    const dms_image2d* metric_filtered = nullptr, const dms_image2d* depth_l0 = nullptr, const dms_image2d* vmap_l0 = nullptr,
                    const dms_camera* cam_l0 = nullptr, float vmap_cutoff = 0.f);
int depth_metric(const dms_image2d* src, dms_image2d* dst, float maxD, hipStream_t s);
int fill_in(const dms_predict_out* ex, const dms_image2d* depth, const dms_image2d* rgba, const dms_camera* cam, int pass_geom,
            int pass_rgb, dms_predict_out* out, hipStream_t s, const void* mirror_src = nullptr, void* mirror_dst = nullptr,
            int mirror_bytes = 0, int* dense_flag = nullptr);
int fill_args(const dms_predict_out* ex, const dms_image2d* depth, const dms_image2d* rgba, const dms_camera* cam, int pass_geom, int pass_rgb,
              dms_predict_out* out, const void* mirror_src, void* mirror_dst, int mirror_bytes, int* dense_flag, FillArgs* res);
int resize_nn(const dms_image2d* src, dms_image2d* dst, int elem, hipStream_t s);

int model_initialise(dms_model* m, const dms_image2d* rgba, const dms_image2d* dm, const dms_image2d* dmf, const dms_camera* cam, int time,
                     int timeIdx, float maxDepth, hipStream_t s);
int index_map(dms_model* m, const dms_pose_block* pose, const dms_camera* cam, int time, int timeIdx, float maxDepth, int timeDelta,
              unsigned long long* zbuf, dms_indexmap_out* out, int transposed, int zclean, hipStream_t s,
              unsigned long long* zbuf_also = nullptr);
int index_project(dms_model* m, const dms_pose_block* pose, const dms_camera* cam, int time, int timeIdx, float maxDepth, int timeDelta,
                  unsigned long long* zbuf, int zclean, hipStream_t s);
int clear_zbuf(unsigned long long* zbuf, int n, hipStream_t s);
int untranspose(const void* src, void* dst, int cols, int rows, int elem, hipStream_t s);
int splat_predict(dms_model* m, const dms_pose_block* pose, const dms_camera* cam, float maxDepth, float confThreshold, int time,
                  int timeIdx, int maxTime, int timeDelta, int active, unsigned long long* zbuf, dms_predict_out* out,
                  dms_image2d* depth_out, int zclean, hipStream_t s, const float* second_conf_time_maxtime = nullptr,
                  unsigned long long* zbuf2 = nullptr, int resolve_only = 0, const FillArgs* fill = nullptr, const TrackInitArgs* init = nullptr);
int splat_project_only(dms_model* m, const dms_pose_block* pose, const dms_camera* cam, float maxDepth, float confThreshold, int time,
                       int timeIdx, int maxTime, int timeDelta, int active, unsigned long long* zbuf, hipStream_t s, const ProjectRider* rider);
int model_sample_graph(dms_model* m, int sampleRate, float* rows4_host, int max_rows, int* n_host, hipStream_t s);
int model_flush_pending(dms_model* m, hipStream_t s);

int model_fuse(dms_model* m, const dms_pose_block* pose, int time, int timeIdx, const dms_image2d* rgba, const dms_image2d* dr,
               const dms_image2d* drf, const dms_indexmap_out* im, const dms_camera* cam, float depthCutoff, float weighting,
               const float* weighting_dev, int transposed, hipStream_t s, int defer_update = 0);
int model_fuse_zbuf(dms_model* m, const dms_pose_block* pose, int time, int timeIdx, const dms_image2d* rgba, const dms_image2d* dr,
                    const dms_image2d* drf, const unsigned long long* zbuf, const dms_camera* cam, float depthCutoff, float weighting,
                    const float* weighting_dev, hipStream_t s, int defer_update = 0);
int model_fuse_scratch(dms_model* m, float* slot_pos4, float* slot_col4, float* slot_nrm4, unsigned* slot_best, unsigned char* slot_flag,
                       unsigned* winner, size_t winner_count, hipStream_t s);
int model_clean(dms_model* m, const dms_pose_block* pose, int time, int timeIdx, const dms_indexmap_out* im, const dms_image2d* depth_synth,
                const dms_camera* cam, float confThreshold, const float* graph_host, int graph_nodes, int timeDelta, float maxDepth,
                int isFern, int transposed, unsigned* count_out2, hipStream_t s, const float* graph_dev = nullptr);

int deform_add_rows(dms_deform* d, const float* rows_dev, int stride, int n, int srcTime, int pin, hipStream_t s);
int deform_fetch(dms_deform* d, dms_deform_result* res, const float** rel8);

struct TrackFold {
  const float* prior_pose16;
  int pyramid, fastOdom, so3, interMap;
};
int odometry_track_enqueue(dms_odometry* o, const float* trans, const float* rot, const float* prior_pose16_dev, int rgbOnly,
                           float icpWeight, int pyramid, int fastOdom, int so3, int interMap, hipStream_t s, FrameState* frame = nullptr,
                           float weightMultiplier = 1.f);
int odometry_result_pose(dms_odometry* o, float* pose16_dev, hipStream_t s);
int odometry_early_init_args(dms_odometry* o, const TrackFold* fold, TrackInitArgs* ti);
int odometry_initModel_fused(dms_odometry* o, const void* vA, const void* nA, const void* iA, const void* vB, const void* nB,
                             const void* iB, const int* flag_dev, int force_b_img, const float* pose16_dev, hipStream_t s,
                             int defer_last_step = 0, unsigned* dense_cnt = nullptr, int dense_samples = 0, const TrackFold* fold = nullptr);
int odometry_initLive_fused(dms_odometry* o, const void* verts, const void* norms, const void* rgba, const int* any_flag_dev,
                            hipStream_t s);
int odometry_enable_ring(dms_odometry* o);
int odometry_free_cus(const dms_odometry* o);
void odometry_set_early_exit(dms_odometry* o, int on);
int odometry_next_buffers(dms_odometry* o, int level, dms_image2d* nextImage, dms_image2d* nextDepth);
int odometry_loop_candidate(dms_odometry* o, FrameState* frame, const dms_image2d* vertex, const dms_image2d* oldTime, float maxDepth,
                            LoopState* out, float* cons, hipStream_t s);
void odometry_bind_live(dms_odometry* o, int k);
void odometry_bind_lastnext(dms_odometry* o, int k);
int odometry_initRGB_image(dms_odometry* o, const dms_image2d* rgba, hipStream_t s);
int odometry_live_views(dms_odometry* o, dms_image2d* depth, dms_image2d* vmap, dms_image2d* nmap, dms_image2d* image, dms_image2d* dx,
                        dms_image2d* dy, dms_image2d* gate, float* minScale, bool mark_derivatives);
void odometry_alias_next_depth(dms_odometry* o);

size_t nid_workspace_bytes(int num_bins);
int computeNIDImg(const dms_image2d* img_kf, const dms_image2d* img_kf_old, const dms_image2d* dmap_kf, const dms_image2d* dmap_kf_old,
                  const dms_image2d* img_curr, int num_bins, void* workspace, size_t workspace_bytes, float* nid_host, float* nid_dev,
                  hipStream_t s);
int computeNIDDepth(const dms_image2d* dmap_kf, const dms_image2d* dmap_kf_old, const dms_image2d* dmap_curr, int num_bins, float max_depth,
                    void* workspace, size_t workspace_bytes, float* nid_host, float* nid_dev, hipStream_t s);

int drawPanelColumn(dms_render_target* t, dms_panels* p, const dms_image2d* rgba, const dms_image2d* depth_u16, const dms_image2d* model_rgba,
                    const dms_image2d* vertex, const dms_viewport* viewports, float depth_cutoff, int which_mask, hipStream_t s);

}
```

densemonoslam_amd/csrc/model_bodies.hpp:

```cpp
#pragma once
#include "common.hpp"
#include "fill.hpp"
#include "live_bodies.hpp"

namespace dms {

struct ModelSrc {
  const float4* vA;
  const float4* nA;
  const uchar4* iA;
  const float4* vB;
  const float4* nB;
  const uchar4* iB;
  const int* flag;
  const unsigned* dense_cnt;
  int dense_samples;
  int* flag_out;
  int force_b_img;
  const float* pose16;
};

__device__ __forceinline__ bool model_use_b(const ModelSrc& m) {
  return (m.dense_cnt ? dense_from_counters(m.dense_cnt, m.dense_samples) : *m.flag) != 0;
}

struct Pose34 {
  M33 R;
  f3 t;
};
__device__ __forceinline__ Pose34 load_pose34(const float* pose16) {
  Pose34 p;
  if (!pose16) {
    p.R.r0 = p.R.r1 = p.R.r2 = p.t = mk3(0.f, 0.f, 0.f);
    return p;
  }
  p.R.r0 = mk3(pose16[0], pose16[1], pose16[2]);
  p.R.r1 = mk3(pose16[4], pose16[5], pose16[6]);
  p.R.r2 = mk3(pose16[8], pose16[9], pose16[10]);
  p.t = mk3(pose16[3], pose16[7], pose16[11]);
  return p;
}
__device__ __forceinline__ void raw_maps(const float4 v, const float4 q, f3& rv, f3& rn) {
  const bool ok = !(v.z == 0.f);
  const float n = qnan();
  rv = ok ? mk3(v.x, v.y, v.z) : mk3(n, n, n);
  rn = ok ? mk3(q.x, q.y, q.z) : mk3(n, n, n);
}
__device__ __forceinline__ void store_transformed(View<float> vmap, View<float> nmap, int rows, int y, int x, const f3& rv, const f3& rn,
                                                  const Pose34& P, bool xf) {
  if (!isnan(rv.x)) {
    const f3 d = xf ? mul(P.R, rv) + P.t : rv;
    vmap.at(y, x) = d.x;
    vmap.at(y + rows, x) = d.y;
    vmap.at(y + 2 * rows, x) = d.z;
  } else {
    vmap.at(y, x) = qnan();
  }
  if (!isnan(rn.x)) {
    const f3 d = xf ? mul(P.R, rn) : rn;
    nmap.at(y, x) = d.x;
    nmap.at(y + rows, x) = d.y;
    nmap.at(y + 2 * rows, x) = d.z;
  } else {
    nmap.at(y, x) = qnan();
  }
}

__device__ __forceinline__ void model_level0_body(int tx, int ty, int BYv, int bx, int by, const ModelSrc& m, int rows, int cols, View<float> vmap,
                                                  View<float> nmap, View<float> depth, View<unsigned char> inten, float cutOff) {
  const int x = bx * 64 + tx;
  const int y = by * BYv + ty;
  if (x >= cols || y >= rows) return;
  const bool useB = model_use_b(m);
  const size_t i = (size_t)y * cols + x;
  const float4 v = useB ? m.vB[i] : m.vA[i];
  const float4 q = useB ? m.nB[i] : m.nA[i];
  const uchar4 c = (useB || m.force_b_img) ? m.iB[i] : m.iA[i];
  const Pose34 P = load_pose34(m.pose16);
  f3 rv, rn;
  raw_maps(v, q, rv, rn);
  store_transformed(vmap, nmap, rows, y, x, rv, rn, P, m.pose16 != nullptr);
  depth.at(y, x) = (v.z > cutOff || v.z <= 0.f) ? qnan() : v.z;
  const float f = ((float)c.x * 0.114f + (float)c.y * 0.299f) + (float)c.z * 0.587f;
  inten.at(y, x) = (unsigned char)f2i_rz(f);
}

template <bool NORMALIZE>
__device__ __forceinline__ f3 resize4(const f3& a, const f3& b, const f3& c, const f3& d) {
  if (isnan(a.x) || isnan(b.x) || isnan(c.x) || isnan(d.x)) return mk3(qnan(), qnan(), qnan());
  f3 n;
  n.x = (a.x + b.x + c.x + d.x) / 4;
  n.y = (a.y + b.y + c.y + d.y) / 4;
  n.z = (a.z + b.z + c.z + d.z) / 4;
  if (NORMALIZE) n = normalized3(n);
  return n;
}

__device__ __forceinline__ void model_levels12_body(int tx, int ty, int BYv, int bx, int by, const ModelSrc& m, int cols0, int rows1, int cols1, int rows2,
                                                    int cols2, View<float> v1, View<float> n1, View<float> v2, View<float> n2) {
  const int lane = tx, k = lane & 3;
  const int x2 = bx * 16 + (lane >> 2);
  const int y2 = by * BYv + ty;
  const int x1 = 2 * x2 + (k & 1), y1 = 2 * y2 + (k >> 1);
  const bool useB = model_use_b(m);
  const float4* vs = useB ? m.vB : m.vA;
  const float4* ns = useB ? m.nB : m.nA;
  const Pose34 P = load_pose34(m.pose16);
  f3 lv = mk3(0.f, 0.f, 0.f), ln = mk3(0.f, 0.f, 0.f);
  if (x1 < cols1 && y1 < rows1) {
    f3 rv[4], rn[4];
#pragma unroll
    for (int j = 0; j < 4; ++j) {
      const size_t i = (size_t)(2 * y1 + (j >> 1)) * cols0 + (2 * x1 + (j & 1));
      raw_maps(vs[i], ns[i], rv[j], rn[j]);
    }
    lv = resize4<false>(rv[0], rv[1], rv[2], rv[3]);
    ln = resize4<true>(rn[0], rn[1], rn[2], rn[3]);
    store_transformed(v1, n1, rows1, y1, x1, lv, ln, P, m.pose16 != nullptr);
  }
  f3 qv[4], qn[4];
#pragma unroll
  for (int j = 0; j < 4; ++j) {
    const int src = (lane & ~3) | j;
    qv[j] = mk3(__shfl(lv.x, src, 64), __shfl(lv.y, src, 64), __shfl(lv.z, src, 64));
    qn[j] = mk3(__shfl(ln.x, src, 64), __shfl(ln.y, src, 64), __shfl(ln.z, src, 64));
  }
  if (k == 0 && x2 < cols2 && y2 < rows2) {
    const f3 a = resize4<false>(qv[0], qv[1], qv[2], qv[3]);
    const f3 b = resize4<true>(qn[0], qn[1], qn[2], qn[3]);
    store_transformed(v2, n2, rows2, y2, x2, a, b, P, m.pose16 != nullptr);
  }
}

template <int BYV>
__device__ __forceinline__ void model_pyr_step1_body(int tx, int ty, int bx, int by, const ModelSrc& m, int rows0, int cols0, float cutOff, View<float> ddst,
                                                     View<unsigned char> idst) {
  constexpr int BX = 64, BY = BYV;
  constexpr int TW = 2 * BX + 3, TH = 2 * BY + 3;
  __shared__ float s_d[TH][TW + 1];
  __shared__ unsigned char s_c[TH][TW + 1];
  const bool useB = model_use_b(m);
  const float4* vs = useB ? m.vB : m.vA;
  const uchar4* is = (useB || m.force_b_img) ? m.iB : m.iA;
  const int sx0 = 2 * (bx * BX) - 2, sy0 = 2 * (by * BY) - 2;
  for (int e = ty * BX + tx; e < TH * TW; e += BX * BY) {
    const int r = e / TW, c = e - r * TW;
    const int gy = sy0 + r, gx = sx0 + c;
    float sv = qnan();
    unsigned char cv = 0;
    if (gx >= 0 && gy >= 0 && gx < cols0 && gy < rows0) {
      const size_t i = (size_t)gy * cols0 + gx;
      const float z = vs[i].z;
      sv = (z > cutOff || z <= 0.f) ? qnan() : z;
      const uchar4 cc = is[i];
      cv = (unsigned char)f2i_rz(((float)cc.x * 0.114f + (float)cc.y * 0.299f) + (float)cc.z * 0.587f);
    }
    s_d[r][c] = sv;
    s_c[r][c] = cv;
  }
  __syncthreads();
  const int x = bx * BX + tx;
  const int y = by * BY + ty;
  if (x >= ddst.cols || y >= ddst.rows) return;
  const live::Tile<float, TW + 1> dt = {&s_d[0][0], sy0, sx0};
  const live::Tile<unsigned char, TW + 1> ct = {&s_c[0][0], sy0, sx0};
  ddst.at(y, x) = live::float_half(dt, x, y, cols0, rows0);
  idst.at(y, x) = live::u8_half(ct, x, y, cols0, rows0);
}

template <int NT>
__device__ __forceinline__ void model_pyr_step2_body(int t, int bx, int by, const ModelSrc& m, int rows0, int cols0, float cutOff, int rows1, int cols1,
                                                     View<float> ddst2, View<unsigned char> idst2) {
  constexpr int OX = 16, OY = 8;
  constexpr int W1 = 2 * OX + 3, H1 = 2 * OY + 3, W0 = 2 * W1 + 3, H0 = 2 * H1 + 3;
  __shared__ float s_d0[H0][W0 + 1];
  __shared__ unsigned char s_c0[H0][W0 + 1];
  __shared__ float s_d1[H1][W1 + 1];
  __shared__ unsigned char s_c1[H1][W1 + 1];
  const bool useB = model_use_b(m);
  const float4* vs = useB ? m.vB : m.vA;
  const uchar4* is = (useB || m.force_b_img) ? m.iB : m.iA;
  const int x1o = 2 * (bx * OX) - 2, y1o = 2 * (by * OY) - 2;
  const int x0o = 2 * x1o - 2, y0o = 2 * y1o - 2;
  for (int e = t; e < H0 * W0; e += NT) {
    const int r = e / W0, c = e - r * W0;
    const int gy = y0o + r, gx = x0o + c;
    float sv = qnan();
    unsigned char cv = 0;
    if (gx >= 0 && gy >= 0 && gx < cols0 && gy < rows0) {
      const size_t i = (size_t)gy * cols0 + gx;
      const float z = vs[i].z;
      sv = (z > cutOff || z <= 0.f) ? qnan() : z;
      const uchar4 cc = is[i];
      cv = (unsigned char)f2i_rz(((float)cc.x * 0.114f + (float)cc.y * 0.299f) + (float)cc.z * 0.587f);
    }
    s_d0[r][c] = sv;
    s_c0[r][c] = cv;
  }
  __syncthreads();
  {
    const live::Tile<float, W0 + 1> dt = {&s_d0[0][0], y0o, x0o};
    const live::Tile<unsigned char, W0 + 1> ct = {&s_c0[0][0], y0o, x0o};
    for (int e = t; e < H1 * W1; e += NT) {
      const int r = e / W1, c = e - r * W1;
      const int gy = y1o + r, gx = x1o + c;
      if (gx >= 0 && gy >= 0 && gx < cols1 && gy < rows1) {
        s_d1[r][c] = live::float_half(dt, gx, gy, cols0, rows0);
        s_c1[r][c] = live::u8_half(ct, gx, gy, cols0, rows0);
      }
    }
  }
  __syncthreads();
  for (int e = t; e < OX * OY; e += NT) {
    const int x = bx * OX + (e % OX), y = by * OY + (e / OX);
    if (x >= ddst2.cols || y >= ddst2.rows) continue;
    const live::Tile<float, W1 + 1> dt = {&s_d1[0][0], y1o, x1o};
    const live::Tile<unsigned char, W1 + 1> ct = {&s_c1[0][0], y1o, x1o};
    ddst2.at(y, x) = live::float_half(dt, x, y, cols1, rows1);
    idst2.at(y, x) = live::u8_half(ct, x, y, cols1, rows1);
  }
}

}
```

densemonoslam_amd/csrc/track.hip:

```cpp
#include <hip/hip_ext.h>
#include <math.h>

#include <map>
#include <string>
#include <vector>

#include "internal.hpp"
#include "host_util.hpp"
#include "pixel_ops.hpp"
#include "smallmath.hpp"
#include "gn_scalar.hpp"
#include "canon.hpp"
#include "pyr_body.hpp"
#include "frame_state.hpp"
#include "track_init.hpp"
#include "model_bodies.hpp"
#include "surfel.hpp"
#include <mutex>

namespace dms {

constexpr bool kTrackerFma = true;

struct Buf {
  void* p = nullptr;
  size_t pitch = 0;
  int rows = 0, cols = 0;
  dms_image2d img() const {
    dms_image2d i;
    i.data = p;
    i.pitch = pitch;
    i.rows = rows;
    i.cols = cols;
    return i;
  }
};

}

using namespace dms;

struct dms_odometry {
  bool early_exit = false;
  bool resident = true;
  int early_exit_force = -1;
  int persist_target = 160;
  int max_resident_blocks = 256;
  int budget_cap = 0;
  bool unchained_ok = false;
  bool fell_back = false;
  int last_shape_P[DMS_NUM_PYRS] = {1, 1, 1}, last_shape_nb[DMS_NUM_PYRS] = {0, 0, 0};
  bool deferred_pyr = false;
  bool init_folded = false;
  bool early_init = false, so3_in_model = false;
  bool so3_beside_model = false;
  int folded_so3 = 0, folded_first_level = 0;
  const float* folded_prior = nullptr;
  unsigned* dense_cnt_zero = nullptr;
  int inject_timeouts = 0;
  int width, height;
  float cx, cy, fx, fy, distThres, angleThres;
  float sobelScale, maxDepthDeltaRGB, maxDepthRGB;
  float minGrad[DMS_NUM_PYRS];
  char* arena = nullptr;
  size_t arena_bytes = 0;
  Buf depth_tmp[3], vmaps_g_prev[3], nmaps_g_prev[3], vmaps_curr[3], nmaps_curr[3];
  Buf lastDepth[3], nextDepth[3], lastImage[3], nextImage[3], lastNextImage[3];
  Buf nextdIdx[3], nextdIdy[3], nextGate[3], pointClouds[3], corresImg[3];
  struct LiveSet {
    Buf depth_tmp[3], vmaps_curr[3], nmaps_curr[3], nextImage[3], nextdIdx[3], nextdIdy[3], nextGate[3];
  };
  LiveSet ring[3];
  char* ring_arena = nullptr;
  bool ring_enabled = false;
  const void* deriv_of = nullptr;
  float* vmaps_tmp = nullptr;
  float* nmaps_tmp = nullptr;
  long long* part_icp = nullptr;
  long long* part_rgb = nullptr;
  long long* part_so3 = nullptr;
  int* part_cnt = nullptr;
  unsigned* tickets = nullptr;
  unsigned long long* ar = nullptr;
  int first_delay = -1;
  bool long_levels_resident = true;
  bool fuse_coarse = false;
  unsigned* rider_cnt = nullptr;
  unsigned rider_issued = 0;
  int first_delay_lvl[4] = {-1, -1, -1, -1};
  int first_delay_for(int nb, int stage = -1) const {
    if (stage >= 0 && stage < 4 && first_delay_lvl[stage] >= 0) return first_delay_lvl[stage];
    return first_delay >= 0 ? first_delay : (nb >= 96 ? 24 : 8);
  }
  int depth_bias = 0;
  int exp_bias = 0;
  long long* prof = nullptr;
  TrackState* state = nullptr;
  TrackState* host_state = nullptr;
  bool profiling = false;
  bool profiling_level0_only = false;
  StageClock clock;
};

namespace dms {

__global__ void k_track_init(TrackState* st, Prior prior, const float* __restrict__ prior_pose16, float fx, float fy, float cx, float cy,
// ... 1050 lines not shown
      const float dx = tc[0] - s.tprev[0], dy = tc[1] - s.tprev[1], dz = tc[2] - s.tprev[2];
      const float n = sqrtf(dx * dx + dy * dy + dz * dz);
      const bool timed_out = __hip_atomic_load(&st->sync_timeout, __ATOMIC_RELAXED, __HIP_MEMORY_SCOPE_AGENT) != 0;
      if (timed_out || (L.fin_rgb && (double)n > 0.3)) {
        for (int i = 0; i < 9; ++i) Rc[i] = sv->Rcurr[i] = s.Rprev[i];
        for (int i = 0; i < 3; ++i) tc[i] = sv->tcurr[i] = s.tprev[i];
        if (!timed_out) sv->rejected_jump = 1;
      }
      for (int i = 0; i < 3; ++i) sv->out_trans[i] = tc[i];
      for (int i = 0; i < 9; ++i) sv->out_rot[i] = Rc[i];
      const bool own = L.frame && L.pose16_out == L.frame->cur.pose;
      if (L.pose16_out) {
        for (int i = 0; i < 3; ++i) {
          for (int j = 0; j < 3; ++j) L.pose16_out[i * 4 + j] = Rc[i * 3 + j];
          L.pose16_out[i * 4 + 3] = tc[i];
        }
        if (!own) {
          L.pose16_out[12] = 0.f;
          L.pose16_out[13] = 0.f;
          L.pose16_out[14] = 0.f;
          L.pose16_out[15] = 1.f;
        }
      }
      if (L.frame) {
        if (own) {
          for (int i = 0; i < 3; ++i) {
            for (int j = 0; j < 3; ++j) s_held[i * 4 + j] = Rc[i * 3 + j];
            s_held[i * 4 + 3] = tc[i];
          }
        }
        frame_after_track_body(L.frame, L.weightMultiplier, __hip_atomic_load(&st->sync_timeout, __ATOMIC_RELAXED, __HIP_MEMORY_SCOPE_AGENT), own ? s_held : nullptr);
      }
    }
  }
  phase(8);
  if (L.prof && blockIdx.x == 0 && tid == 0) {
    phase(9);
    for (int i = 0; i < 10; ++i) L.prof[L.level * 16 + i] += s_prof[i];
  }
}

template <bool ICP, bool RGB, int P, bool EXIT>
__global__ __launch_bounds__(kPB) void k_gn_level(TrackState* st, GnArgs a, LevelArgs L) {
  gn_level_body<ICP, RGB, P, EXIT, false>(st, st, a, L, (int)gridDim.x);
}

struct So3Extra {
  int nb_so3, gx, gy;
  unsigned* zero16;
  View<const float> dsrc;
  View<float> ddst;
  View<const unsigned char> isrc;
  View<unsigned char> idst;
};

struct So3Args {
  const unsigned char* lastImage;
  size_t last_pitch;
  const unsigned char* nextImage;
  size_t next_pitch;
  int cols, rows;
  unsigned long long* ar;
  SolveCam cam;
  int first_gn_level, max_iter, exp_bias, first_delay;
};

template <bool FUSED>
__device__ __forceinline__ void so3_body(TrackState* st, TrackState& s, const So3Args& q, const int nb) {
  const unsigned char* lastImage = q.lastImage;
  const unsigned char* nextImage = q.nextImage;
  const size_t last_pitch = q.last_pitch, next_pitch = q.next_pitch;
  const int cols = q.cols, rows = q.rows, first_gn_level = q.first_gn_level, max_iter = q.max_iter, exp_bias = q.exp_bias, first_delay = q.first_delay;
  unsigned long long* ar = q.ar;
  const SolveCam cam = q.cam;
  __shared__ int s_viol;
  __shared__ int s_E[4];
  __shared__ double s_bias[2][32];
  __shared__ double s_red[kPWaves][32];
  __shared__ float s_sums[32];
  int eb_mine = 0;
  const int tid = threadIdx.x;
  if (!FUSED) {
    const int* src = reinterpret_cast<const int*>(st);
    int* dst = reinterpret_cast<int*>(&s);
    for (int i = tid; i < (int)(sizeof(TrackState) / 4); i += kPB) dst[i] = src[i];
  }
  if (tid == 0) {
    int E[4];
    canon::static_so3(cols * rows, E);
    for (int c = 0; c < 4; ++c) s_E[c] = canon::clamp_e(E[c] + exp_bias);
  }
  __syncthreads();
  if (s.so3_done) return;
  if (tid < 32) {
    canon::write_bias<3>(s_E, s_bias, tid);
    eb_mine = canon::value_exp<3>(s_E, tid);
  }
  __syncthreads();
  const int N = cols * rows;
  const int i = blockIdx.x * kPB + tid;
  const bool live = i < N;
  const int ic = live ? i : i % N;
  const int y = ic / cols, x = ic - y * cols;
  int pool_used = 0, retries = 0;
  bool on_pool = false, failed = false;
  for (int it = 0; it < max_iter;) {
    const So3Params p = so3_params_of(&s, cols, rows);
// ... 30 lines not shown
        break;
      }
      if (tid == 0) canon::retry_step<3>(s_E);
      __syncthreads();
      if (tid < 32) {
        canon::write_bias<3>(s_E, s_bias, tid);
        eb_mine = canon::value_exp<3>(s_E, tid);
      }
      __syncthreads();
      continue;
    }
    on_pool = false;
    if (tid == 0) {
      sc::so3_solve_core(&s, s_sums, cam.fx, cam.fy, cam.cx, cam.cy, it == max_iter - 1 ? 1 : 0, first_gn_level);
    } else if (tid >= 64 && tid < 96) {
      int E[4];
#pragma unroll
      for (int c = 0; c < 4; ++c) E[c] = s_E[c];
      canon::next_exponents<3>(s_sums, E);
      canon::write_bias<3>(E, s_bias, tid - 64);
      if (tid - 64 < 4) s_E[tid - 64] = E[tid - 64];
    }
    __syncthreads();
    if (s.so3_done) break;
    if (tid < 32) eb_mine = canon::value_exp<3>(s_E, tid);
    ++it;
  }
  __syncthreads();
  if (FUSED || blockIdx.x == 0) {
    if (tid == 0) {
      if (failed) __hip_atomic_store(&st->sync_timeout, 2, __ATOMIC_RELAXED, __HIP_MEMORY_SCOPE_AGENT);
      s.sync_timeout = __hip_atomic_load(&st->sync_timeout, __ATOMIC_RELAXED, __HIP_MEMORY_SCOPE_AGENT);
      s.canon_retries += retries;
      if (failed && !s.so3_done) {
        s.so3_done = 1;
        double Rt[16];
        for (int q2 = 0; q2 < 16; ++q2) Rt[q2] = s.resultRt[q2];
        sc::gn_params(Rt, sc::kpre_of(cam.fx, cam.fy, cam.cx, cam.cy, first_gn_level), s.krkinv, s.kt);
      }
    }
    __syncthreads();
    if (!FUSED) {
      const int* src = reinterpret_cast<const int*>(&s);
      int* dst = reinterpret_cast<int*>(st);
      for (int k = tid; k < (int)(sizeof(TrackState) / 4); k += kPB) dst[k] = src[k];
    }
  }
}

__global__ __launch_bounds__(kPB) void k_so3_level(TrackState* st, const unsigned char* lastImage, size_t last_pitch,
                                                   const unsigned char* nextImage, size_t next_pitch, int cols, int rows,
                                                   unsigned long long* ar, SolveCam cam, int first_gn_level, int max_iter, int exp_bias, int first_delay, So3Extra ex) {
  if ((int)blockIdx.x >= ex.nb_so3) {
    const int c = (int)blockIdx.x - ex.nb_so3, by = c / ex.gx, bx = c - by * ex.gx;
    model_pyr_step_pixel(bx * 64 + (int)(threadIdx.x & 63), by * (kPB / 64) + (int)(threadIdx.x >> 6), ex.dsrc, ex.ddst, ex.isrc, ex.idst);
    return;
  }
  if (ex.zero16 && blockIdx.x == 0 && threadIdx.x < 16) ex.zero16[threadIdx.x * 16] = 0u;
  __shared__ TrackState s;
  const So3Args q = {lastImage, last_pitch, nextImage, next_pitch, cols, rows, ar, cam, first_gn_level, max_iter, exp_bias, first_delay};
  so3_body<false>(st, s, q, ex.nb_so3);
}

struct ModelGroups {
  ModelSrc m;
  int g0x, g0y, g12x, g12y, gsx, gsy, g2x, g2y;
  int rows0, cols0, rows1, cols1, rows2, cols2;
  float cutOff;
  View<float> v0, n0, depth0, v1, n1, v2, n2, depth1, depth2;
  View<unsigned char> inten0, inten1, inten2;
};

__global__ __launch_bounds__(kPB) void k_so3_model(TrackState* st, So3Args q, int nb_so3, ModelGroups G) {
  if ((int)blockIdx.x < nb_so3) {
    __shared__ TrackState s;
    so3_body<false>(st, s, q, nb_so3);
    return;
  }
  const int t = (int)threadIdx.x, tx = t & 63, ty = t >> 6;
  constexpr int BYv = kPB / 64;
  const int b = (int)blockIdx.x - nb_so3;
  if (G.m.dense_cnt && b == 0 && t == 0) *G.m.flag_out = model_use_b(G.m) ? 1 : 0;
  const int nb12 = G.g12x * G.g12y, nbs = G.gsx * G.gsy, nb2 = G.g2x * G.g2y;
  if (b < nb12) {
    model_levels12_body(tx, ty, BYv, b % G.g12x, b / G.g12x, G.m, G.cols0, G.rows1, G.cols1, G.rows2, G.cols2, G.v1, G.n1, G.v2, G.n2);
  } else if (b < nb12 + nbs) {
    const int c = b - nb12;
    model_pyr_step1_body<BYv>(tx, ty, c % G.gsx, c / G.gsx, G.m, G.rows0, G.cols0, G.cutOff, G.depth1, G.inten1);
  } else if (b < nb12 + nbs + nb2) {
    const int c = b - nb12 - nbs;
    model_pyr_step2_body<kPB>(t, c % G.g2x, c / G.g2x, G.m, G.rows0, G.cols0, G.cutOff, G.rows1, G.cols1, G.depth2, G.inten2);
  } else {
    const int c = b - nb12 - nbs - nb2;
    model_level0_body(tx, ty, BYv, c % G.g0x, c / G.g0x, G.m, G.rows0, G.cols0, G.v0, G.n0, G.depth0, G.inten0, G.cutOff);
  }
}

struct CoarseArgs {
  So3Args so3;
  GnArgs a2, a1;
  LevelArgs L2, L1;
  int run_so3, run_l2, run_l1;
  unsigned* rider_cnt;
  unsigned rider_target;
};

template <bool ICP, bool RGB, int P1, bool EXIT>
// ... 649 lines not shown
  return (o->resident && nbp <= kMaxPersistBlocks && nbp <= budget_of(o)) ? nbp : 0;
}

int odometry_track_enqueue(dms_odometry* o, const float* trans, const float* rot, const float* prior_pose16_dev, int rgbOnly,
                           float icpWeight, int pyramid, int fastOdom, int so3, int interMap, hipStream_t s, FrameState* frame,
                           float weightMultiplier) {
  DMS_REQUIRE(o && ((trans && rot) || prior_pose16_dev), "null argument");
  const bool icp = !rgbOnly && icpWeight > 0;
  const bool rgb = rgbOnly || icpWeight < 100;
  DMS_REQUIRE(icp || rgb, "neither ICP nor RGB term active");
  int rc;

  Prior prior;
  memset(&prior, 0, sizeof(prior));
  if (!prior_pose16_dev) {
    memcpy(prior.v, trans, 3 * sizeof(float));
    memcpy(prior.v + 3, rot, 9 * sizeof(float));
  }

  if (rgb && o->deriv_of != o->nextImage[0].p) {
    if ((rc = nextDerivatives(o, s))) return rc;
  }

  int iterations[DMS_NUM_PYRS];
  iterations[0] = interMap ? 50 : fastOdom ? 3 : 10;
  iterations[1] = interMap ? 50 : pyramid ? 5 : 0;
  iterations[2] = interMap ? 50 : pyramid ? 4 : 0;
  int first_level = 0;
  for (int l = DMS_NUM_PYRS - 1; l >= 0; --l)
    if (iterations[l] > 0) {
      first_level = l;
      break;
    }

  const bool folded = o->init_folded;
  So3Extra ex;
  memset(&ex, 0, sizeof(ex));
  const bool so3_ran = o->so3_in_model;
  unsigned* first_gn_zero16 = nullptr;
  if (so3_ran) {
    o->so3_in_model = false;
    o->early_init = false;
    DMS_REQUIRE(so3 && o->folded_so3 == 1 && o->folded_first_level == first_level && o->folded_prior == prior_pose16_dev && prior_pose16_dev && !o->deferred_pyr,
                "track call differs from the one its early set-up and SO3 stage were prepared for");
    first_gn_zero16 = o->dense_cnt_zero;
    o->dense_cnt_zero = nullptr;
  } else if (folded) {
    o->init_folded = false;
    DMS_REQUIRE(so3 && so3_resident_blocks(o) > 0 && o->folded_so3 == (so3 ? 1 : 0) && o->folded_first_level == first_level &&
                    o->folded_prior == prior_pose16_dev && prior_pose16_dev,
                "track call differs from the one its folded set-up was prepared for");
    ex.zero16 = o->dense_cnt_zero;
    o->dense_cnt_zero = nullptr;
    if (o->deferred_pyr) {
      o->deferred_pyr = false;
      dms_image2d d1 = o->lastDepth[1].img(), d2 = o->lastDepth[2].img(), i1 = o->lastImage[1].img(), i2 = o->lastImage[2].img();
      ex.gx = (d2.cols + 63) / 64;
      ex.gy = (d2.rows + kPB / 64 - 1) / (kPB / 64);
      ex.dsrc = view<const float>(&d1);
      ex.ddst = view<float>(&d2);
      ex.isrc = view<const unsigned char>(&i1);
      ex.idst = view<unsigned char>(&i2);
    }
  } else {
    StageTimer t(o->clock, s, "track_init", timed(o));
    const int zero_pairs = o->resident ? (int)((size_t)kArSets * kArWords / 2) : 0;
    const int ni = o->resident ? 16 : 1;
    unsigned* zero16 = o->dense_cnt_zero;
    o->dense_cnt_zero = nullptr;
    if (o->deferred_pyr) {
      o->deferred_pyr = false;
      dms_image2d d1 = o->lastDepth[1].img(), d2 = o->lastDepth[2].img(), i1 = o->lastImage[1].img(), i2 = o->lastImage[2].img();
      const int gx = (d2.cols + 63) / 64, gy = (d2.rows + 3) / 4;
      hipLaunchKernelGGL(k_track_init_pyr, dim3(gx * gy + ni), dim3(64, 4), 0, s, o->state, prior, prior_pose16_dev, o->fx, o->fy, o->cx, o->cy,
                         so3 ? 1 : 0, first_level, o->ar, zero_pairs, o->inject_timeouts > 0 ? 1 : 0, zero16, gx, gy, ni, view<const float>(&d1),
                         view<float>(&d2), view<const unsigned char>(&i1), view<unsigned char>(&i2));
    } else {
      hipLaunchKernelGGL(k_track_init, dim3(ni), dim3(256), 0, s, o->state, prior, prior_pose16_dev, o->fx, o->fy, o->cx, o->cy, so3 ? 1 : 0,
                         first_level, o->ar, zero_pairs, o->inject_timeouts > 0 ? 1 : 0, zero16);
    }
    DMS_CHECK_LAUNCH();
    if (o->inject_timeouts > 0) o->inject_timeouts -= 1;
  }

  PersistSection persist(s, budget_of(o), o->unchained_ok);

  auto level_below_of = [&](int l) {
    for (int q = l - 1; q >= 0; --q)
      if (iterations[q] > 0) return q;
    return l;
  };
  auto gn_args_of = [&](int l) {
    const int div = 1 << l;
    GnArgs a;
    memset(&a, 0, sizeof(a));
    a.maps.vcurr = (const float*)o->vmaps_curr[l].p;
    a.maps.vcurr_pitch = o->vmaps_curr[l].pitch;
    a.maps.ncurr = (const float*)o->nmaps_curr[l].p;
    a.maps.ncurr_pitch = o->nmaps_curr[l].pitch;
    a.maps.vprev = (const float*)o->vmaps_g_prev[l].p;
    a.maps.vprev_pitch = o->vmaps_g_prev[l].pitch;
    a.maps.nprev = (const float*)o->nmaps_g_prev[l].p;
    a.maps.nprev_pitch = o->nmaps_g_prev[l].pitch;
    a.fx = o->fx / div;
    a.fy = o->fy / div;
    a.cx = o->cx / div;
    a.cy = o->cy / div;
// ... 55 lines not shown
    pnb = 0;
    if (o->resident && (iterations[l] <= kArRing || o->long_levels_resident))
      persistent_shape(o->vmaps_curr[l].cols * (o->vmaps_curr[l].rows / 3), o->persist_target, budget_of(o), pP, pnb);
    o->last_shape_P[l] = pP;
    o->last_shape_nb[l] = pnb;
  };

  bool coarse = false;
  int cP1 = 1, cnb = 0;
  if (o->fuse_coarse && o->resident && so3 && !so3_ran && iterations[2] > 0 && iterations[1] > 0 && iterations[2] <= kArRing && iterations[1] <= kArRing) {
    int P2 = 1, nb2 = 0;
    level_shape(2, P2, nb2);
    level_shape(1, cP1, cnb);
    const int nbs = so3_resident_blocks(o);
    coarse = nbs > 0 && nb2 > 0 && cnb > 0 && P2 == 1 && cP1 <= 2 && nb2 <= cnb && nbs <= cnb;
  }
  if (coarse) {
    const Buf& li = o->lastNextImage[2];
    const Buf& ni = o->nextImage[2];
    CoarseArgs F;
    memset(&F, 0, sizeof(F));
    F.so3 = {(const unsigned char*)li.p, li.pitch, (const unsigned char*)ni.p, ni.pitch, ni.cols, ni.rows, o->ar, SolveCam{o->fx, o->fy, o->cx, o->cy},
             first_level, 10, o->exp_bias + o->depth_bias, o->first_delay_for(cnb, 3)};
    F.a2 = gn_args_of(2);
    F.a1 = gn_args_of(1);
    F.L2 = level_args_of(2, cnb);
    F.L1 = level_args_of(1, cnb);
    F.run_so3 = F.run_l2 = F.run_l1 = 1;
    F.rider_cnt = o->rider_cnt;
    o->rider_issued += (unsigned)(ex.gx * ex.gy);
    F.rider_target = o->rider_issued;
    ex.nb_so3 = cnb;
    persist.begin();
    StageTimer t(o->clock, s, "track_coarse", timed(o));
    const bool ee = F.L1.early_exit != 0;
    if (icp && rgb)
      launch_track_coarse<true, true>(cP1, ee, cnb + ex.gx * ex.gy, s, o->state, F, ex);
    else if (icp)
      launch_track_coarse<true, false>(cP1, ee, cnb + ex.gx * ex.gy, s, o->state, F, ex);
    else
      launch_track_coarse<false, true>(cP1, ee, cnb + ex.gx * ex.gy, s, o->state, F, ex);
    DMS_CHECK_LAUNCH();
  } else if (so3 && !so3_ran) {
    const int L = 2;
    const Buf& li = o->lastNextImage[L];
    const Buf& ni = o->nextImage[L];
    const int nb = reduce_blocks_for(li.rows * li.cols);
    const int nbp = so3_resident_blocks(o);
    if (nbp > 0) {
      persist.begin();
      StageTimer t(o->clock, s, "so3_level", timed(o));
      SolveCam cam = {o->fx, o->fy, o->cx, o->cy};
      ex.nb_so3 = nbp;
      hipLaunchKernelGGL(k_so3_level, dim3(nbp + ex.gx * ex.gy), dim3(kPB), 0, s, o->state, (const unsigned char*)li.p, li.pitch,
                         (const unsigned char*)ni.p, ni.pitch, ni.cols, ni.rows, o->ar, cam, first_level, 10, o->exp_bias + o->depth_bias, o->first_delay_for(nbp, 3), ex);
      DMS_CHECK_LAUNCH();
    } else
    for (int i = 0; i < 10; ++i) {
      {
        StageTimer t(o->clock, s, "so3_pass", timed(o));
        SolveCam cam = {o->fx, o->fy, o->cx, o->cy};
        hipLaunchKernelGGL(k_so3_pass, dim3(nb), dim3(kBlock), 0, s, o->state, (const unsigned char*)li.p, li.pitch,
                           (const unsigned char*)ni.p, ni.pitch, ni.cols, ni.rows, o->part_so3, o->tickets, cam, i, i == 9 ? 1 : 0, first_level,
                           o->exp_bias + o->depth_bias);
        DMS_CHECK_LAUNCH();
      }
    }
  }

  bool finalized_in_kernel = false;
  for (int l = DMS_NUM_PYRS - 1; l >= 0; --l) {
    if (coarse && l >= 1) continue;
    int pP = 1, pnb = 0;
    level_shape(l, pP, pnb);
    const bool persistent = pnb > 0;
    if (rgb && !persistent) {
      dms_camera k = {o->fx, o->fy, o->cx, o->cy};
      dms_image2d d = o->lastDepth[l].img(), c = o->pointClouds[l].img();
      if ((rc = projectToPointCloud(&d, &c, &k, l, s))) return rc;
    }
    if (iterations[l] == 0) continue;
    const GnArgs a = gn_args_of(l);
    const int nb = track_blocks_for(a.cols * a.rows);
    const int level_below = level_below_of(l);
    if (persistent) {
      LevelArgs L = level_args_of(l, pnb);
      if (first_gn_zero16) {
        L.zero16 = first_gn_zero16;
        first_gn_zero16 = nullptr;
      }
      if (l == 0) finalized_in_kernel = true;
      persist.begin();
      static const char* const kLevelTimer[3] = {"gn_level0", "gn_level1", "gn_level2"};
      StageTimer t(o->clock, s, kLevelTimer[l], timed(o, l == 0));
      hipEvent_t done = (l == 0) ? persist.closing_event() : nullptr;
      if (icp && rgb)
        launch_gn_level<true, true>(pP, pnb, s, o->state, a, L, done);
      else if (icp)
        launch_gn_level<true, false>(pP, pnb, s, o->state, a, L, done);
      else
        launch_gn_level<false, true>(pP, pnb, s, o->state, a, L, done);
      DMS_CHECK_LAUNCH();
      continue;
    }
    for (int j = 0; j < iterations[l]; ++j) {
      const int next_level = (j == iterations[l] - 1) ? level_below : l;
      SolveArgs q;
// ... 260 lines not shown
    dx[l] = o->nextdIdx[l].img();
    dy[l] = o->nextdIdy[l].img();
    gate[l] = o->nextGate[l].img();
    minScale[l] = rgb_min_scale(o, l);
  }
  if (mark_derivatives) o->deriv_of = o->nextImage[0].p;
  return DMS_OK;
}

int odometry_initRGB_image(dms_odometry* o, const dms_image2d* rgba, hipStream_t s) {
  int rc = populateImage(rgba, o->nextImage, s);
  if (rc) return rc;
  return nextDerivatives(o, s);
}

void odometry_alias_next_depth(dms_odometry* o) {
  for (int i = 0; i < DMS_NUM_PYRS; ++i) o->nextDepth[i] = o->lastDepth[i];
}

int odometry_next_buffers(dms_odometry* o, int level, dms_image2d* nextImage, dms_image2d* nextDepth) {
  DMS_REQUIRE(o && level >= 0 && level < DMS_NUM_PYRS, "bad argument");
  if (nextImage) *nextImage = o->nextImage[level].img();
  if (nextDepth) *nextDepth = o->nextDepth[level].img();
  return DMS_OK;
}

int odometry_early_init_args(dms_odometry* o, const TrackFold* fold, TrackInitArgs* ti) {
  if (!o) return 0;
  if (!fold && o->early_init && ti->inject_timeout) o->inject_timeouts += 1;
  memset(ti, 0, sizeof(*ti));
  o->early_init = false;
  if (!fold || !o->so3_beside_model || !o->resident || !fold->prior_pose16 || !fold->so3 || fold->interMap || so3_resident_blocks(o) <= 0) return 0;
  const int it1 = fold->pyramid ? 5 : 0, it2 = fold->pyramid ? 4 : 0;
  ti->st = o->state;
  ti->prior_pose16 = fold->prior_pose16;
  ti->fx = o->fx;
  ti->fy = o->fy;
  ti->cx = o->cx;
  ti->cy = o->cy;
  ti->so3 = 1;
  ti->first_level = it2 > 0 ? 2 : (it1 > 0 ? 1 : 0);
  ti->sync_words = o->ar;
  ti->n_sync = (int)((size_t)kArSets * kArWords / 2);
  ti->inject_timeout = o->inject_timeouts > 0 ? 1 : 0;
  if (o->inject_timeouts > 0) o->inject_timeouts -= 1;
  ti->blocks = 16;
  o->early_init = true;
  o->folded_so3 = 1;
  o->folded_first_level = ti->first_level;
  o->folded_prior = fold->prior_pose16;
  return 1;
}

int odometry_initModel_fused(dms_odometry* o, const void* vA, const void* nA, const void* iA, const void* vB, const void* nB,
                             const void* iB, const int* flag_dev, int force_b_img, const float* pose16_dev, hipStream_t s,
                             int defer_last_step, unsigned* dense_cnt, int dense_samples, const TrackFold* fold) {
  dms_image2d v[DMS_NUM_PYRS], n[DMS_NUM_PYRS], d[DMS_NUM_PYRS], im[DMS_NUM_PYRS];
  for (int i = 0; i < DMS_NUM_PYRS; ++i) {
    v[i] = o->vmaps_g_prev[i].img();
    n[i] = o->nmaps_g_prev[i].img();
    d[i] = o->lastDepth[i].img();
    im[i] = o->lastImage[i].img();
  }
  o->deferred_pyr = defer_last_step != 0;
  DMS_REQUIRE(!dense_cnt || defer_last_step, "dense counters are zeroed by the track call that takes the deferred pyramid step");
  o->dense_cnt_zero = dense_cnt;
  TrackInitArgs ti;
  memset(&ti, 0, sizeof(ti));
  o->init_folded = false;
  if (fold && fold->prior_pose16 && fold->so3 && !fold->interMap && defer_last_step && so3_resident_blocks(o) > 0) {
    const int it1 = fold->pyramid ? 5 : 0, it2 = fold->pyramid ? 4 : 0;
    ti.st = o->state;
    ti.prior_pose16 = fold->prior_pose16;
    ti.fx = o->fx;
    ti.fy = o->fy;
    ti.cx = o->cx;
    ti.cy = o->cy;
    ti.so3 = 1;
    ti.first_level = it2 > 0 ? 2 : (it1 > 0 ? 1 : 0);
    ti.sync_words = o->ar;
    ti.n_sync = (int)((size_t)kArSets * kArWords / 2);
    ti.inject_timeout = (!o->early_init && o->inject_timeouts > 0) ? 1 : 0;
    if (!o->early_init && o->inject_timeouts > 0) o->inject_timeouts -= 1;
    ti.blocks = 16;
    o->init_folded = true;
    o->folded_so3 = 1;
    o->folded_first_level = ti.first_level;
    o->folded_prior = fold->prior_pose16;
  }
  if (o->early_init && o->init_folded) {
    o->init_folded = false;
    o->deferred_pyr = false;
    o->so3_in_model = true;
    ModelGroups G;
    memset(&G, 0, sizeof(G));
    G.m.vA = (const float4*)vA;
    G.m.nA = (const float4*)nA;
    G.m.iA = (const uchar4*)iA;
    G.m.vB = (const float4*)vB;
    G.m.nB = (const float4*)nB;
    G.m.iB = (const uchar4*)iB;
    G.m.flag = flag_dev;
    G.m.dense_cnt = dense_cnt;
    G.m.dense_samples = dense_samples;
    G.m.flag_out = const_cast<int*>(flag_dev);
    G.m.force_b_img = force_b_img;
    G.m.pose16 = pose16_dev;
    G.rows0 = v[0].rows / 3;
    G.cols0 = v[0].cols;
    G.rows1 = v[1].rows / 3;
    G.cols1 = v[1].cols;
    G.rows2 = v[2].rows / 3;
    G.cols2 = v[2].cols;
    DMS_REQUIRE(G.rows1 == G.rows0 / 2 && G.cols1 == G.cols0 / 2 && G.rows2 == G.rows1 / 2 && G.cols2 == G.cols1 / 2, "pyramid shapes");
    constexpr int BYv = kPB / 64;
    G.g0x = (G.cols0 + 63) / 64;
    G.g0y = (G.rows0 + BYv - 1) / BYv;
    G.g12x = ((G.cols1 + 1) / 2 + 15) / 16;
    G.g12y = ((G.rows1 + 1) / 2 + BYv - 1) / BYv;
    G.gsx = (d[1].cols + 63) / 64;
    G.gsy = (d[1].rows + BYv - 1) / BYv;
    G.g2x = (d[2].cols + 15) / 16;
    G.g2y = (d[2].rows + 7) / 8;
    G.cutOff = o->maxDepthRGB;
    G.v0 = view<float>(&v[0]);
    G.n0 = view<float>(&n[0]);
    G.depth0 = view<float>(&d[0]);
    G.inten0 = view<unsigned char>(&im[0]);
    G.v1 = view<float>(&v[1]);
    G.n1 = view<float>(&n[1]);
    G.v2 = view<float>(&v[2]);
    G.n2 = view<float>(&n[2]);
    G.depth1 = view<float>(&d[1]);
    G.inten1 = view<unsigned char>(&im[1]);
    G.depth2 = view<float>(&d[2]);
    G.inten2 = view<unsigned char>(&im[2]);
    const Buf& li = o->lastNextImage[2];
    const Buf& ni = o->nextImage[2];
    const int nbs = so3_resident_blocks(o);
    const So3Args q = {(const unsigned char*)li.p, li.pitch, (const unsigned char*)ni.p, ni.pitch, ni.cols, ni.rows, o->ar, SolveCam{o->fx, o->fy, o->cx, o->cy},
                       o->folded_first_level, 10, o->exp_bias + o->depth_bias, o->first_delay_for(nbs, 3)};
    PersistSection persist(s, budget_of(o), o->unchained_ok);
// ... 217 lines not shown
```

densemonoslam_amd/fusion.py:

```python
import ctypes as C
import os

import numpy as np

from . import capi
from .capi import Camera, DeviceBuffer, DeviceImage, Image2D, TrackResult, check, lib

MAX_SENSORS = capi.MAX_SENSORS
SURFEL_DTYPE = np.dtype([("pos", "<f4", (4,)), ("col", "<f4", (4,)), ("nrm", "<f4", (4,)), ("times", "<f4", (MAX_SENSORS,))])


class PoseBlock(C.Structure):
    _fields_ = [("pose", C.c_float * 16), ("t_inv", C.c_float * 16)]


class IndexMapOut(C.Structure):
    _fields_ = [("index", Image2D), ("vertConf", Image2D), ("colorTime", Image2D), ("normRad", Image2D)]


class PredictOut(C.Structure):
    _fields_ = [("image", Image2D), ("vertex", Image2D), ("normal", Image2D), ("time", Image2D)]


class FusionParams(C.Structure):
    _fields_ = [
        ("width", C.c_int), ("height", C.c_int),
        ("fx", C.c_float), ("fy", C.c_float), ("cx", C.c_float), ("cy", C.c_float),
        ("timeDelta", C.c_int), ("confidence", C.c_float), ("depthCut", C.c_float), ("icpWeight", C.c_float),
        ("fastOdom", C.c_int), ("so3", C.c_int), ("frameToFrameRGB", C.c_int), ("pyramid", C.c_int),
        ("hybrid_tracking", C.c_int), ("rgbOnly", C.c_int), ("timeIdx", C.c_int),
        ("maxDepthProcessed", C.c_float), ("model_capacity", C.c_size_t),
        ("pipeline_ingest", C.c_int), ("global_predict", C.c_int),
        ("nid_keyframing", C.c_int), ("nid_threshold", C.c_float), ("nid_depth_lambda", C.c_float), ("nid_bins_img", C.c_int),
        ("nid_bins_depth", C.c_int), ("nid_pyramid_level", C.c_int),
        ("local_loop_closure", C.c_int), ("reloc", C.c_int), ("num_sensors", C.c_int), ("share_projection", C.c_int),
        ("fused_fill_in", C.c_int), ("hybrid_loops", C.c_int), ("lazy_final_prediction", C.c_int),
        ("fused_associate", C.c_int),
    ]


class FrameResult(C.Structure):
    _fields_ = [
        ("pose", C.c_float * 16), ("surfels", C.c_uint), ("tick", C.c_int), ("fused", C.c_int), ("fill_in", C.c_int),
        ("weighting", C.c_float), ("nid_score", C.c_float), ("track", TrackResult),
        ("loop_ok", C.c_int), ("loop_constraints", C.c_int), ("loop_icp_error", C.c_float), ("loop_icp_count", C.c_float),
        ("loop_pose", C.c_float * 16), ("loop_cov_diag", C.c_double * 6),
        ("tracking_ok", C.c_int), ("lost", C.c_int),
    ]


_P, _I, _F = C.c_void_p, C.c_int, C.c_float
_I2 = C.POINTER(Image2D)
_K = C.POINTER(Camera)
lib.dms_model_create.argtypes = [C.POINTER(_P), C.c_size_t, _I, _I]
lib.dms_model_destroy.argtypes = [_P]
lib.dms_model_count.argtypes = [_P, C.POINTER(C.c_uint), _P]
lib.dms_model_capacity.argtypes = [_P]
lib.dms_model_set_num_sensors.argtypes = [_P, _I]
lib.dms_model_set_clean_suffix_min.argtypes = [_P, C.c_size_t]
lib.dms_model_consume.argtypes = [_P, _P, C.POINTER(C.c_float), _P]
lib.dms_model_export_records.argtypes = [_P, _P, C.c_uint, C.POINTER(C.c_uint), _P]
lib.dms_model_consume_records.argtypes = [_P, _P, C.c_uint, C.POINTER(C.c_float), _P]
lib.dms_model_capacity.restype = C.c_size_t
lib.dms_model_download.argtypes = [_P, _P, C.c_uint, C.POINTER(C.c_uint), _P]
lib.dms_model_upload.argtypes = [_P, _P, C.c_uint, _P]
lib.dms_model_download_ref.argtypes = [_P, _P, C.c_uint, C.POINTER(C.c_uint), _P]
lib.dms_model_upload_ref.argtypes = [_P, _P, C.c_uint, _P]
lib.dms_depth_bilateral.argtypes = [_I2, _I2, _F, _P]
lib.dms_depth_metric.argtypes = [_I2, _I2, _F, _P]
lib.dms_model_initialise.argtypes = [_P, _I2, _I2, _I2, _K, _I, _I, _F, _P]
lib.dms_pose_block_set.argtypes = [_P, C.POINTER(C.c_float), _P]
lib.dms_index_map.argtypes = [_P, _P, _K, _I, _I, _F, _I, _P, C.POINTER(IndexMapOut), _P]
lib.dms_splat_predict.argtypes = [_P, _P, _K, _F, _F, _I, _I, _I, _I, _I, _P, C.POINTER(PredictOut), _P]
lib.dms_splat_depth.argtypes = [_P, _P, _K, _F, _F, _I, _I, _I, _I, _P, _I2, _P]
lib.dms_model_fuse.argtypes = [_P, _P, _I, _I, _I2, _I2, _I2, C.POINTER(IndexMapOut), _K, _F, _F, _P, _P]
lib.dms_index_project.argtypes = [_P, _P, _K, _I, _I, _F, _I, _P, _P]
lib.dms_model_fuse_ex.argtypes = [_P, _P, _I, _I, _I2, _I2, _I2, C.POINTER(IndexMapOut), _P, _K, _F, _F, _P, _I, _P]
lib.dms_model_apply_pending.argtypes = [_P, _P]
lib.dms_model_fuse_scratch.argtypes = [_P, _P, _P, _P, _P, _P, _P, C.c_size_t, _P]
lib.dms_fusion_debug_keep_assoc_zbuf.argtypes = [_P, _I]
lib.dms_model_clean.argtypes = [_P, _P, _I, _I, C.POINTER(IndexMapOut), _I2, _K, _F, C.POINTER(C.c_float), _I, _I, _F, _I, _P]
lib.dms_fill_in.argtypes = [C.POINTER(PredictOut), _I2, _I2, _K, _I, _I, C.POINTER(PredictOut), _P]
lib.dms_resize_nn.argtypes = [_I2, _I2, _I, _P]
lib.dms_fusion_default_params.argtypes = [C.POINTER(FusionParams), _I, _I, _F, _F, _F, _F]
lib.dms_fusion_default_params.restype = None
lib.dms_fusion_create.argtypes = [C.POINTER(_P), C.POINTER(FusionParams)]
lib.dms_fusion_destroy.argtypes = [_P]
lib.dms_fusion_process_frame.argtypes = [_P, _P, _I, _P, C.POINTER(C.c_float), _F, _P]
lib.dms_fusion_fetch.argtypes = [_P, C.POINTER(FrameResult), _P]
lib.dms_fusion_inputs_ready.argtypes = [_P, _P]
lib.dms_fusion_inputs_consumed.argtypes = [_P, _P]
lib.dms_fusion_model.argtypes = [_P]
lib.dms_fusion_set_orb_loop.argtypes = [_P, C.POINTER(C.c_float), C.POINTER(C.c_float)]
lib.dms_fusion_get_global_loop_constraints.argtypes = [_P, C.POINTER(C.c_float), _I, C.POINTER(C.c_int), _P]
lib.dms_fusion_apply_global_loop_begin.argtypes = [_P, C.POINTER(C.c_float), C.POINTER(C.c_float), _P]
lib.dms_fusion_apply_global_loop_end.argtypes = [_P, C.POINTER(C.c_float), _I, _I, _P]
lib.dms_fusion_model.restype = _P
lib.dms_fusion_odometry.argtypes = [_P]
lib.dms_fusion_odometry.restype = _P
lib.dms_fusion_pose_device.argtypes = [_P]
lib.dms_fusion_pose_device.restype = _P
lib.dms_model_sample_graph.argtypes = [_P, _I, C.POINTER(C.c_float), _I, C.POINTER(C.c_int), _P]
lib.dms_fusion_thumbnails.argtypes = [_P, _P, _P]
lib.dms_fusion_frame_block.argtypes = [_P, _P, _P, _P, C.c_int, _P]
lib.dms_fusion_arm_frame_block.argtypes = [_P, _P, _P, _P, C.c_int]
lib.dms_fusion_frame_block_written.argtypes = [_P]
lib.dms_fusion_get_image.argtypes = [_P, _I, _I2]
lib.dms_fusion_process_frame_begin.argtypes = [_P, _P, _I, _P, C.POINTER(C.c_float), _F, _P]
lib.dms_fusion_fetch_loop.argtypes = [_P, C.POINTER(FrameResult), _P]
lib.dms_fusion_process_frame_end.argtypes = [_P, C.POINTER(C.c_float), _I, C.POINTER(C.c_float), _P]
lib.dms_fusion_get_loop_constraints.argtypes = [_P, C.POINTER(C.c_float), _I, C.POINTER(C.c_int)]
lib.dms_fusion_join_map.argtypes = [_P, _P, C.POINTER(C.c_float), _P]
lib.dms_fusion_set_cluster.argtypes = [_P, C.c_int]
lib.dms_fusion_compute_feedback.argtypes = [_P, _P]
lib.dms_fusion_clusters.argtypes = [_P, C.POINTER(C.c_int), C.c_int, C.POINTER(C.c_int), C.POINTER(C.c_int)]
lib.dms_fusion_cluster_model.argtypes = [_P, C.c_int]
lib.dms_fusion_cluster_model.restype = _P
lib.dms_fusion_import_camera.argtypes = [_P, _P, C.POINTER(C.c_float), _I, _P, _I, _P, _P]
lib.dms_relative_transform.argtypes = [C.POINTER(C.c_float), C.POINTER(C.c_float), C.POINTER(C.c_float)]
lib.dms_pose_compose.argtypes = [C.POINTER(C.c_float), C.POINTER(C.c_float), C.POINTER(C.c_float)]
lib.dms_fusion_set_profiling.argtypes = [_P, _I]
lib.dms_fusion_get_lazy_stats.argtypes = [_P, C.POINTER(C.c_int), C.POINTER(C.c_long), C.POINTER(C.c_long), C.POINTER(C.c_long)]


class InterMapResult(C.Structure):
    _fields_ = [("accepted", C.c_int), ("cov_ok", C.c_int), ("relativeTransform", C.c_float * 16), ("refinedPose", C.c_float * 16),
                ("cov_diag", C.c_double * 6), ("lastICPError", C.c_float), ("lastICPCount", C.c_float), ("lastRGBError", C.c_float),
                ("lastRGBCount", C.c_float), ("iterations_run", C.c_int * 3), ("so3_iterations_run", C.c_int)]


lib.dms_refframe_create.argtypes = [C.POINTER(_P), _I, _I, _F, _F, _F, _F]
lib.dms_refframe_destroy.argtypes = [_P]
lib.dms_refframe_refine.argtypes = [_P, _P, C.POINTER(C.c_float), C.POINTER(C.c_float), _P, _P, _P, _I, _F, _I, _I, _I, _F, _F, _F,
                                    C.POINTER(InterMapResult), _P]
lib.dms_refframe_odometry.argtypes = [_P]
lib.dms_refframe_odometry.restype = _P
lib.dms_refframe_get_prediction.argtypes = [_P, C.POINTER(PredictOut)]
lib.dms_fusion_get_kernel_time.argtypes = [_P, C.c_char_p, C.POINTER(C.c_double), C.POINTER(C.c_int)]


def _cam(K):
    return Camera(*[float(v) for v in K])


def _img(a, dtype=None):
    if isinstance(a, DeviceImage):
        return a
    return DeviceImage.from_array(a if dtype is None else np.asarray(a, dtype))


def _f16(a):
    a = np.ascontiguousarray(a, np.float32).reshape(16)
    return a, a.ctypes.data_as(C.POINTER(C.c_float))


def relative_transform(recoveryPose, currPose):
    a, ap = _f16(recoveryPose)
    b, bp = _f16(currPose)
    o, op = _f16(np.zeros(16, np.float32))
    check(lib.dms_relative_transform(ap, bp, op), "dms_relative_transform")
    return o.reshape(4, 4)


def pose_compose(a, b):
    a, ap = _f16(a)
    b, bp = _f16(b)
    o, op = _f16(np.zeros(16, np.float32))
    check(lib.dms_pose_compose(ap, bp, op), "dms_pose_compose")
    return o.reshape(4, 4)


class DevicePose:

    def __init__(self, pose=None):
        self.buf = DeviceBuffer(C.sizeof(PoseBlock))
# ... 431 lines not shown
        check(lib.dms_depth_norm(panels.h, C.byref(views[PANEL_DEPTH_NORM]), float(np.float32(0.3) * np.float32(1000.0)), float(cut * np.float32(1000.0)),
                                 stream), "dms_depth_norm")
        check(lib.dms_model_depth_image(panels.h, C.byref(views[PANEL_MODEL]), float(cut), stream), "dms_model_depth_image")
        white = (C.c_float * 3)(1.0, 1.0, 1.0)
        for k in range(4):
            if not (which_mask >> k) & 1:
                continue
            vp = Viewport(*[int(v) for v in viewports[k]])
            if k in (PANEL_DEPTH_NORM, PANEL_MODEL):
                panels.blit(target, k, viewports[k], stream=stream)
            else:
                check(lib.dms_render_blit(target.h, C.byref(views[k]), PANEL_RGBA8, PANEL_LINEAR if k == PANEL_RGB else PANEL_NEAREST, C.byref(vp),
                                          white, stream), "dms_render_blit")

    def feedbackBuffers(self):
        return {FeedbackBuffer.RAW: FeedbackBuffer(self, CLOUD_RAW), FeedbackBuffer.FILTERED: FeedbackBuffer(self, CLOUD_FILTERED)}

    def clusters(self):
        ids = (C.c_int * 64)()
        n, cur = C.c_int(0), C.c_int(0)
        check(lib.dms_fusion_clusters(self.h, ids, 64, C.byref(n), C.byref(cur)), "dms_fusion_clusters")
        return [int(ids[i]) for i in range(min(n.value, 64))], int(cur.value)

    def image(self, which):
        v = Image2D()
        check(lib.dms_fusion_get_image(self.h, which, C.byref(v)), "dms_fusion_get_image")
        dt, k = _IMG_TYPES[which]
        return capi.download_view(v, dt, k)

    def imagePtr(self, which):
        v = Image2D()
        check(lib.dms_fusion_get_image(self.h, which, C.byref(v)), "dms_fusion_get_image")
        return int(v.data)

    def thumbnails(self, block_ptr, stream=None):
        check(lib.dms_fusion_thumbnails(self.h, C.c_void_p(block_ptr), stream), "dms_fusion_thumbnails")

    def frameBlock(self, block_ptr, pose_ptr, tick_ptr, tick, stream=None):
        check(lib.dms_fusion_frame_block(self.h, C.c_void_p(block_ptr), C.c_void_p(pose_ptr), C.c_void_p(tick_ptr), int(tick), stream),
              "dms_fusion_frame_block")

    def armFrameBlock(self, block_ptr, pose_ptr, tick_ptr, tick):
        check(lib.dms_fusion_arm_frame_block(self.h, C.c_void_p(block_ptr), C.c_void_p(pose_ptr), C.c_void_p(tick_ptr), int(tick)),
              "dms_fusion_arm_frame_block")

    def frameBlockWritten(self):
        return bool(lib.dms_fusion_frame_block_written(self.h))

    def lazyStats(self):
        e, d, m, st = C.c_int(0), C.c_long(0), C.c_long(0), C.c_long(0)
        check(lib.dms_fusion_get_lazy_stats(self.h, C.byref(e), C.byref(d), C.byref(m), C.byref(st)), "dms_fusion_get_lazy_stats")
        return {"eager": bool(e.value), "deferred": int(d.value), "materialised": int(m.value), "stale": int(st.value)}

    def loopConstraints(self):
        n = C.c_int(0)
        cap = (self.width // 20) * (self.height // 20)
        out = np.zeros((cap, 7), np.float32)
        check(lib.dms_fusion_get_loop_constraints(self.h, out.ctypes.data_as(C.POINTER(C.c_float)), cap, C.byref(n)),
              "dms_fusion_get_loop_constraints")
        return out[:n.value].copy()

    def setLoopSolver(self, on=True, sampleRate=5000):
        lib.dms_fusion_set_loop_solver.argtypes = [_P, _I, _I]
        check(lib.dms_fusion_set_loop_solver(self.h, int(bool(on)), int(sampleRate)), "dms_fusion_set_loop_solver")

    def deformation(self):
        from . import deform

        lib.dms_fusion_deformation.restype = C.c_void_p
        lib.dms_fusion_deformation.argtypes = [_P]
        h = lib.dms_fusion_deformation(self.h)
        return deform.Deformation.view(h, (self.width // 20) * (self.height // 20)) if h else None

    def deforms(self):
        lib.dms_fusion_get_deforms.argtypes = [_P]
        return int(lib.dms_fusion_get_deforms(self.h))

    def relativeConstraints(self):
        lib.dms_fusion_get_relative_constraints.argtypes = [_P, C.POINTER(C.c_float), _I, C.POINTER(C.c_int)]
        n = C.c_int(0)
        check(lib.dms_fusion_get_relative_constraints(self.h, None, 0, C.byref(n)), "dms_fusion_get_relative_constraints")
        out = np.zeros((max(1, n.value), 8), np.float32)
        check(lib.dms_fusion_get_relative_constraints(self.h, out.ctypes.data_as(C.POINTER(C.c_float)), n.value, C.byref(n)),
              "dms_fusion_get_relative_constraints")
        return out[:n.value].copy()

    OPTIONS = {"rgbOnly": 0, "icpWeight": 1, "pyramid": 2, "fastOdom": 3, "so3": 4, "frameToFrameRGB": 5, "confidence": 6, "depthCut": 7}

    def setOption(self, name, value):
        check(lib.dms_fusion_set_option(self.h, self.OPTIONS[name], C.c_double(float(value))), "dms_fusion_set_option")

    def getOption(self, name):
        v = C.c_double(0.0)
        check(lib.dms_fusion_get_option(self.h, self.OPTIONS[name], C.byref(v)), "dms_fusion_get_option")
        return v.value

    def set_profiling(self, on):
        check(lib.dms_fusion_set_profiling(self.h, int(on)))

    def kernel_time(self, name):
        ms, n = C.c_double(0), C.c_int(0)
        check(lib.dms_fusion_get_kernel_time(self.h, name.encode(), C.byref(ms), C.byref(n)))
        return ms.value, n.value


class ReferenceFrameRefiner:
# ... 315 lines not shown
```

include/dmslam_fusion.h:

```cpp
#ifndef DMSLAM_FUSION_H_
#define DMSLAM_FUSION_H_

#include "dmslam.h"

#ifdef __cplusplus
extern "C" {
#endif

typedef struct dms_model dms_model;

int dms_model_create(dms_model** out, size_t capacity, int width, int height);
int dms_model_destroy(dms_model* m);
int dms_model_set_num_sensors(dms_model* m, int num_sensors);
int dms_model_set_clean_suffix_min(dms_model* m, size_t surfels);
int dms_model_count(dms_model* m, unsigned int* count, dms_stream s);
size_t dms_model_capacity(dms_model* m);
size_t dms_model_count_bound(dms_model* m);

int dms_model_download_ref(dms_model* m, float* host_vertices15, unsigned int max_count, unsigned int* count, dms_stream s);
int dms_model_upload_ref(dms_model* m, const float* host_vertices15, unsigned int count, dms_stream s);
int dms_model_download(dms_model* m, float* host_records, unsigned int max_count, unsigned int* count, dms_stream s);
int dms_model_upload(dms_model* m, const float* host_records, unsigned int count, dms_stream s);


// ... 50 lines not shown
                   const float* weighting_dev, dms_stream s);
int dms_model_fuse_ex(dms_model* m, const dms_pose_block* pose_dev, int time, int timeIdx, const dms_image2d* rgba,
                      const dms_image2d* depth_metric, const dms_image2d* depth_metric_filtered,
                      const dms_indexmap_out* indexmap, const unsigned long long* zbuf, const dms_camera* cam, float depthCutoff,
                      float weighting, const float* weighting_dev, int defer_update, dms_stream s);
int dms_model_apply_pending(dms_model* m, dms_stream s);
int dms_model_fuse_scratch(dms_model* m, float* slot_pos4, float* slot_col4, float* slot_nrm4, unsigned int* slot_best,
                           unsigned char* slot_flag, unsigned int* winner, size_t winner_count, dms_stream s);

int dms_model_clean(dms_model* m, const dms_pose_block* pose_dev, int time, int timeIdx,
                    const dms_indexmap_out* indexmap, const dms_image2d* depth_synth, const dms_camera* cam,
                    float confThreshold, const float* graph_host, int graph_nodes, int timeDelta, float maxDepth,
                    int isFern, dms_stream s);

int dms_fill_in(const dms_predict_out* existing, const dms_image2d* depth_filtered_u16, const dms_image2d* rgba,
                const dms_camera* cam, int passthrough_geom, int passthrough_rgb, dms_predict_out* filled, dms_stream s);

int dms_resize_nn(const dms_image2d* src, dms_image2d* dst, int elem_bytes, dms_stream s);

typedef struct dms_fusion dms_fusion;

typedef struct dms_fusion_params {
  int width, height;
  float fx, fy, cx, cy;
  int timeDelta;
  float confidence;
  float depthCut;
  float icpWeight;
  int fastOdom;
  int so3;
  int frameToFrameRGB;
  int pyramid;
  int hybrid_tracking;
  int rgbOnly;
  int timeIdx;
  float maxDepthProcessed;
  size_t model_capacity;
  int pipeline_ingest;
  int global_predict;
  int nid_keyframing;
  float nid_threshold;
  float nid_depth_lambda;
  int nid_bins_img;
  int nid_bins_depth;
  int nid_pyramid_level;
  int local_loop_closure;
  int reloc;
  int num_sensors;
  int share_projection;
  int fused_fill_in;
  int hybrid_loops;
  int lazy_final_prediction;
  int fused_associate;
} dms_fusion_params;

void dms_fusion_default_params(dms_fusion_params* p, int width, int height, float fx, float fy, float cx, float cy);

int dms_fusion_create(dms_fusion** out, const dms_fusion_params* p);
int dms_fusion_destroy(dms_fusion* f);

typedef struct dms_frame_result {
  float pose[16];
  unsigned int surfels;
  int tick;
  int fused;
  int fill_in;
  float weighting;
  float nid_score;
  dms_track_result track;
  int loop_ok;
  int loop_constraints;
  float loop_icp_error;
  float loop_icp_count;
  float loop_pose[16];
  double loop_cov_diag[6];
  int tracking_ok;
  int lost;
} dms_frame_result;

int dms_fusion_process_frame(dms_fusion* f, const void* rgb_dev, int rgb_channels, const unsigned short* depth_dev,
                             const float* inPose16, float weightMultiplier, dms_stream s);
int dms_fusion_fetch(dms_fusion* f, dms_frame_result* r, dms_stream s);

int dms_fusion_inputs_ready(dms_fusion* f, dms_stream producer);
int dms_fusion_inputs_consumed(dms_fusion* f, dms_stream s);

int dms_fusion_process_frame_begin(dms_fusion* f, const void* rgb_dev, int rgb_channels, const unsigned short* depth_dev,
                                   const float* inPose16, float weightMultiplier, dms_stream s);
int dms_fusion_fetch_loop(dms_fusion* f, dms_frame_result* r, dms_stream s);
int dms_fusion_process_frame_end(dms_fusion* f, const float* graph_host, int graph_nodes, const float* newPose16, dms_stream s);
int dms_fusion_get_lazy_stats(dms_fusion* f, int* eager, long* deferred, long* materialised, long* stale);
int dms_fusion_debug_keep_assoc_zbuf(dms_fusion* f, int on);

int dms_fusion_set_orb_loop(dms_fusion* f, const float* orbTcwOld16, const float* orbTcwNew16);
int dms_fusion_get_global_loop_constraints(dms_fusion* f, float* rows7_host, int max_rows, int* n, dms_stream s);
int dms_fusion_apply_global_loop_begin(dms_fusion* f, const float* orbTcwOld16, const float* orbTcwNew16, dms_stream s);
int dms_fusion_apply_global_loop_end(dms_fusion* f, const float* graph_host, int graph_nodes, int accepted, dms_stream s);

int dms_fusion_join_map(dms_fusion* f, dms_fusion* owner, const float* relativeTransform16, dms_stream s);
int dms_fusion_import_camera(dms_fusion* f, dms_fusion* owner, const float* pose16, int tick, const void* last_rgb_dev, int rgb_channels,
                             const unsigned short* last_depth_dev, dms_stream s);
int dms_relative_transform(const float* recoveryPose16, const float* currPose16, float* out16);
int dms_pose_compose(const float* a16, const float* b16, float* out16);

typedef struct dms_refframe dms_refframe;
typedef struct dms_intermap_result {
  int accepted;
  int cov_ok;
  float relativeTransform[16];
  float refinedPose[16];
  double cov_diag[6];
  float lastICPError, lastICPCount, lastRGBError, lastRGBCount;
  int iterations_run[DMS_NUM_PYRS];
  int so3_iterations_run;
} dms_intermap_result;
int dms_refframe_create(dms_refframe** out, int width, int height, float cx, float cy, float fx, float fy);
int dms_refframe_destroy(dms_refframe* r);
int dms_refframe_refine(dms_refframe* r, dms_model* map, const float* recoveryPose16, const float* currPose16, const float* vertex_dev,
                        const float* normal_dev, const void* image_rgba_dev, int depthCutoff, float confidenceThreshold, int timeIdx,
                        int timeDelta, int maxTime, float covThresh, float icpErrThresh, float icpCountThresh, dms_intermap_result* out,
                        dms_stream s);
dms_odometry* dms_refframe_odometry(dms_refframe* r);
int dms_refframe_get_prediction(dms_refframe* r, dms_predict_out* view);

int dms_fusion_predict(dms_fusion* f, float confidence, dms_stream s);

dms_model* dms_fusion_model(dms_fusion* f);
const float* dms_fusion_pose_device(dms_fusion* f);
dms_odometry* dms_fusion_odometry(dms_fusion* f);
int dms_fusion_get_image(dms_fusion* f, int which, dms_image2d* view);

int dms_fusion_thumbnails(dms_fusion* f, void* block_dev, dms_stream s);
size_t dms_thumb_block_bytes(int width, int height);
void dms_thumb_block_offsets(int width, int height, size_t* vertex_offset, size_t* normal_offset);
int dms_fusion_frame_block(dms_fusion* f, void* block_dev, float* pose16_dst_dev, int* tick_dst_dev, int tick, dms_stream s);
int dms_fusion_arm_frame_block(dms_fusion* f, void* block_dev, float* pose16_dst_dev, int* tick_dst_dev, int tick);
int dms_fusion_frame_block_written(dms_fusion* f);
int dms_fusion_wait_frame_done(dms_fusion* f, dms_stream waiter);

int dms_fusion_get_loop_constraints(dms_fusion* f, float* rows7_host, int max_rows, int* n);
enum {
  DMS_OPT_RGB_ONLY = 0,
  DMS_OPT_ICP_WEIGHT = 1,
  DMS_OPT_PYRAMID = 2,
// ... 34 lines not shown
```

Measured before the change: 2795 frames/s.

## Fuse tracking prediction resolve with model init and pyramid into one pass

```diff
diff --git a/densemonoslam_amd/csrc/fill.hpp b/densemonoslam_amd/csrc/fill.hpp
--- a/densemonoslam_amd/csrc/fill.hpp
+++ b/densemonoslam_amd/csrc/fill.hpp
@@ -36,8 +36,8 @@
   return mk3((((float)x - a.cx) * z) * a.ifx, (((float)y - a.cy) * z) * a.ify, z);
 }
 
-__device__ __forceinline__ void fill_pixel_out(const FillArgs& a, int px, int py, const float4& sv, const float4& sn, const uchar4& si, float4& ov,
-                                               float4& on, uchar4& oi) {
+__device__ __forceinline__ void fill_pixel_values(const FillArgs& a, int px, int py, const float4& sv, const float4& sn, const uchar4& si, float4& ov,
+                                                  float4& on, uchar4& oi) {
   const size_t i = (size_t)py * a.cols + px;
   const float colsf = (float)a.cols, rowsf = (float)a.rows;
   const float tcx = ((float)px + 0.5f) / colsf, tcy = ((float)py + 0.5f) / rowsf;
@@ -49,7 +49,6 @@
     } else {
       ov = sv;
     }
-    a.out_vertex[i] = ov;
   }
   {
     if (sn.z == 0.f || a.pass_geom == 1) {
@@ -63,15 +62,21 @@
     } else {
       on = sn;
     }
-    a.out_normal[i] = on;
   }
   {
     if ((si.x == 0 && si.y == 0 && si.z == 0) || a.pass_rgb == 1)
       oi = a.rgba[i];
     else
       oi = si;
-    a.out_image[i] = oi;
   }
+}
+__device__ __forceinline__ void fill_pixel_out(const FillArgs& a, int px, int py, const float4& sv, const float4& sn, const uchar4& si, float4& ov,
+                                               float4& on, uchar4& oi) {
+  const size_t i = (size_t)py * a.cols + px;
+  fill_pixel_values(a, px, py, sv, sn, si, ov, on, oi);
+  a.out_vertex[i] = ov;
+  a.out_normal[i] = on;
+  a.out_image[i] = oi;
 }
 __device__ __forceinline__ void fill_pixel(const FillArgs& a, int px, int py, const float4& sv, const float4& sn, const uchar4& si) {
   float4 ov, on;
@@ -150,11 +155,26 @@
   }
 }
 
+__device__ __forceinline__ int dense_from_count(unsigned tot, int samples) { return ((float)(int)tot / (float)samples > 0.95f) ? 0 : 1; }
 __device__ __forceinline__ int dense_from_counters(const unsigned* cnt, int samples) {
   unsigned tot = 0;
 #pragma unroll
   for (int k = 0; k < 16; ++k) tot += cnt[k * 16];
-  return ((float)(int)tot / (float)samples > 0.95f) ? 0 : 1;
+  return dense_from_count(tot, samples);
+}
+
+__host__ __device__ __forceinline__ int fill_sample_cell(int k, int cols, int rows) {
+  const int dw = cols / 20, dh = rows / 20;
+  const int i = k % dw, j = k / dw;
+  const int sx = texel(((float)i + 0.5f) / (float)dw, (float)cols, cols), sy = texel(((float)j + 0.5f) / (float)dh, (float)rows, rows);
+  return sx * rows + sy;
+}
+inline int fill_sample_cells(int cols, int rows, int* cells ) {
+  const int n = (cols / 20) * (rows / 20);
+  for (int k = 0; k < n; ++k) cells[k] = fill_sample_cell(k, cols, rows);
+  for (int k = 1; k < n; ++k)
+    if (cells[k] == cells[k - 1] || (k >= cols / 20 && cells[k] == cells[k - cols / 20])) return 0;
+  return n;
 }
 
 }
diff --git a/densemonoslam_amd/csrc/fusion_frame.hip b/densemonoslam_amd/csrc/fusion_frame.hip
--- a/densemonoslam_amd/csrc/fusion_frame.hip
+++ b/densemonoslam_amd/csrc/fusion_frame.hip
@@ -229,6 +229,12 @@
   unsigned* tickets = nullptr;
   bool fold_track_init = true;
   bool dense_by_counters = false;
+  int* sample_cells = nullptr;
+  int n_sample_cells = 0;
+  int predict_model_threads = 256;
+  bool one_call_now = false;
+  bool model_written = false;
+  long predict_fused = 0, predict_plain = 0;
   double host_wait_ms = 0.0;
   bool pre_valid = false;
   int pre_tick = 0;
@@ -336,6 +342,7 @@
   f->zbuf2 = (unsigned long long*)c.take(N * 8);
   f->zbuf_assoc = (unsigned long long*)c.take(N * 8);
   f->tickets = (unsigned*)c.take(2048 + 512 + 1024);
+  f->sample_cells = (int*)c.take((size_t)((W < 2048 ? W : 2048) / 20) * ((H < 2048 ? H : 2048) / 20) * sizeof(int));
   f->state = (FrameState*)c.take(sizeof(FrameState));
   f->lazy_pose = (dms_pose_block*)c.take(sizeof(dms_pose_block));
 }
@@ -362,7 +369,12 @@
   bool have_prior = false;
   const TrackInitArgs* track_init = nullptr;
   bool* track_init_taken = nullptr;
+  const PredictModelArgs* model = nullptr;
 };
+
+static bool tracking_resolves_shared(const dms_fusion* f, bool have_prior) {
+  return f->pre_valid && !have_prior && f->pre_tick == f->tick && f->pre_version == f->model->version;
+}
 
 int predict_body(dms_fusion* f, hipStream_t s, Predict kind, const PredictOpts& o) {
   const bool dense_test = kind == Predict::tracking;
@@ -397,10 +409,13 @@
     StageTimer t(f->clock, s, "predict", f->profiling);
     const int W = f->p.width, H = f->p.height;
     bool done = false;
+    DMS_REQUIRE(!o.model || (fused && dense_test), "the fused prediction + model pass needs the fused fill-in of a tracking prediction");
+    if (o.model) f->dense_by_counters = false;
     if (kind == Predict::tracking && f->pre_valid) {
-      if (!o.have_prior && f->pre_tick == f->tick && f->pre_version == f->model->version) {
+      if (tracking_resolves_shared(f, o.have_prior)) {
         if ((rc = splat_predict(f->model, &f->state->cur, &f->cam, f->p.maxDepthProcessed, o.confidence, f->tick, f->p.timeIdx, f->tick,
-                                f->p.timeDelta, 1, f->zbuf2, &f->pred, nullptr, 1, s, nullptr, nullptr, 1, fused, fused ? o.track_init : nullptr)))
+                                f->p.timeDelta, 1, f->zbuf2, &f->pred, nullptr, 1, s, nullptr, nullptr, 1, fused, fused ? o.track_init : nullptr,
+                                o.model)))
           return rc;
         done = true;
       } else if ((rc = clear_zbuf(f->zbuf2, W * H, s))) {
@@ -438,7 +453,7 @@
         f->lazy_deferred += 1;
       } else if ((rc = splat_predict(f->model, &f->state->cur, &f->cam, f->p.maxDepthProcessed, o.confidence, f->tick, f->p.timeIdx, f->tick,
                               f->p.timeDelta, 1, f->zbuf, &f->pred, nullptr, 1, s, dual ? second : nullptr, dual ? f->zbuf2 : nullptr, 0,
-                              fused, fused ? o.track_init : nullptr)))
+                              fused, fused ? o.track_init : nullptr, o.model)))
         return rc;
       if (dual) {
         f->pre_valid = true;
@@ -459,8 +474,9 @@
 
 int predict_view(dms_fusion* f, float confidence, hipStream_t s) { return predict_body(f, s, Predict::view, PredictOpts{confidence}); }
 
-int predict_tracking(dms_fusion* f, hipStream_t s, bool have_prior, const TrackInitArgs* track_init, bool* track_init_taken) {
-  return predict_body(f, s, Predict::tracking, PredictOpts{0.7f, nullptr, false, have_prior, track_init, track_init_taken});
+int predict_tracking(dms_fusion* f, hipStream_t s, bool have_prior, const TrackInitArgs* track_init, bool* track_init_taken,
+                     const PredictModelArgs* model = nullptr) {
+  return predict_body(f, s, Predict::tracking, PredictOpts{0.7f, nullptr, false, have_prior, track_init, track_init_taken, model});
 }
 
 int predict_final(dms_fusion* f, hipStream_t s, void* state_mirror, bool one_call) {
@@ -613,6 +629,7 @@
   p->hybrid_loops = 0;
   p->lazy_final_prediction = 1;
   p->fused_associate = 1;
+  p->fused_model_prediction = 1;
 }
 
 static int set_depth_bias(dms_fusion* f) {
@@ -700,6 +717,11 @@
   if (const char* lm = getenv("DMS_LATE_MAIN")) f->late.forced = atoi(lm) != 0 ? 1 : 0;
   if (const char* lz = getenv("DMS_LAZY_FINAL_PREDICTION")) f->p.lazy_final_prediction = atoi(lz) != 0 ? 1 : 0;
   if (const char* fa = getenv("DMS_FUSED_ASSOCIATE")) f->p.fused_associate = atoi(fa) != 0 ? 1 : 0;
+  if (const char* fm = getenv("DMS_FUSED_MODEL_PREDICTION")) f->p.fused_model_prediction = atoi(fm) != 0 ? 1 : 0;
+  if (const char* pt = getenv("DMS_PREDICT_MODEL_THREADS")) {
+    const int t = atoi(pt);
+    if (t == 256 || t == 512 || t == 1024) f->predict_model_threads = t;
+  }
   if (e == hipSuccess) e = hipEventCreateWithFlags(&f->ev_inputs, hipEventDisableTiming);
   if (e == hipSuccess) e = hipMemset(f->arena, 0, f->arena_bytes);
   if (e == hipSuccess) e = hipHostMalloc((void**)&f->h_state, 4 * sizeof(FrameState), hipHostMallocMapped);
@@ -732,6 +754,11 @@
     unsigned tm[256];
     f->thumb_masks_ok = thumb_sample_masks(p->width, p->height, tm);
     (void)hipMemcpy(f->tickets + 640, tm, sizeof(tm), hipMemcpyHostToDevice);
+    if (p->width <= 2048 && p->height <= 2048) {
+      std::vector<int> cells((size_t)(p->width / 20) * (p->height / 20));
+      f->n_sample_cells = fill_sample_cells(p->width, p->height, cells.data());
+      (void)hipMemcpy(f->sample_cells, cells.data(), (size_t)f->n_sample_cells * sizeof(int), hipMemcpyHostToDevice);
+    }
   }
   Pose16 I;
   for (int i = 0; i < 16; ++i) I.v[i] = (i % 5 == 0) ? 1.f : 0.f;
@@ -1045,7 +1072,25 @@
   memset(&early, 0, sizeof(early));
   bool early_taken = false;
   const bool want_early = f->p.hybrid_tracking && f->fold_track_init && !f->lost && odometry_early_init_args(f->odom, &fold, &early) != 0;
-  if ((rc = predict_tracking(f, s, inPose16 != nullptr, want_early ? &early : nullptr, &early_taken))) return rc;
+  PredictModelArgs pm;
+  memset(&pm, 0, sizeof(pm));
+  f->model_written = false;
+  if (f->p.fused_model_prediction && f->one_call_now && f->p.hybrid_tracking && f->p.fused_fill_in && f->fold_track_init && !want_early && !f->lost &&
+      !f->p.nid_keyframing && !f->p.local_loop_closure && !f->p.hybrid_loops && !f->p.frameToFrameRGB && f->n_sample_cells > 0 &&
+      odometry_model_views_begin(f->odom, &fold, &pm.maps, &early, tracking_resolves_shared(f, inPose16 != nullptr) ? f->zbuf2 : f->zbuf,
+                                 f->sample_cells, f->n_sample_cells) != 0) {
+    pm.pose16 = f->state->cur.pose;
+    pm.flag_out = &f->state->fill_in;
+    pm.sample_cells = f->sample_cells;
+    pm.n_cells = f->n_sample_cells;
+    pm.samples = (f->p.width / 20) * (f->p.height / 20);
+    pm.threads = f->predict_model_threads;
+    f->model_written = true;
+  }
+  (f->model_written ? f->predict_fused : f->predict_plain) += 1;
+  if ((rc = predict_tracking(f, s, inPose16 != nullptr, (want_early || f->model_written) ? &early : nullptr, &early_taken,
+                             f->model_written ? &pm : nullptr)))
+    return rc;
   if (want_early && !early_taken) odometry_early_init_args(f->odom, nullptr, &early);
   if (!f->p.hybrid_tracking) {
     hipLaunchKernelGGL(k_frame_after_track, dim3(1), dim3(64), 0, s, f->state, weightMultiplier);
@@ -1054,7 +1099,8 @@
   }
   {
     StageTimer t(f->clock, s, "odom_init", f->profiling);
-    if ((rc = odometry_initModel_fused(f->odom, f->pred.vertex.data, f->pred.normal.data, f->pred.image.data, f->fill.vertex.data,
+    if (!f->model_written &&
+        (rc = odometry_initModel_fused(f->odom, f->pred.vertex.data, f->pred.normal.data, f->pred.image.data, f->fill.vertex.data,
                                        f->fill.normal.data, f->fill.image.data, &f->state->fill_in, f->p.frameToFrameRGB ? 1 : 0,
                                        f->state->cur.pose, s, 1,
                                        f->dense_by_counters ? f->tickets : nullptr, (f->p.width / 20) * (f->p.height / 20),
@@ -1331,7 +1377,9 @@
                              float weightMultiplier, dms_stream st) {
   DMS_REQUIRE(!f || !f->loop_solver || (f->model->sharers == 1 && f->clusters.size() == 1 && f->req_cluster == 0),
               "the loop solver needs a map this camera owns alone, without clusters");
+  if (f) f->one_call_now = true;
   int rc = dms_fusion_process_frame_begin(f, rgb_dev, rgb_channels, depth_dev, inPose16, weightMultiplier, st);
+  if (f) f->one_call_now = false;
   if (rc) return rc;
   if (f->loop_solver && f->p.local_loop_closure && !f->cur_bootstrap && !f->lost) {
     const float* table_dev = nullptr;
@@ -1388,6 +1436,13 @@
   if (deferred) *deferred = f->lazy_deferred;
   if (materialised) *materialised = f->lazy_materialised;
   if (stale) *stale = f->lazy_stale;
+  return DMS_OK;
+}
+
+int dms_fusion_get_predict_stats(dms_fusion* f, long* fused, long* plain) {
+  DMS_REQUIRE(f, "null argument");
+  if (fused) *fused = f->predict_fused;
+  if (plain) *plain = f->predict_plain;
   return DMS_OK;
 }
 
diff --git a/densemonoslam_amd/csrc/fusion_map.hip b/densemonoslam_amd/csrc/fusion_map.hip
--- a/densemonoslam_amd/csrc/fusion_map.hip
+++ b/densemonoslam_amd/csrc/fusion_map.hip
@@ -8,6 +8,7 @@
 #include "internal.hpp"
 #include "host_util.hpp"
 #include "track_init.hpp"
+#include "model_bodies.hpp"
 
 namespace dms {
 
@@ -993,6 +994,16 @@
   }
 }
 
+__device__ __forceinline__ uchar4 resolved_image(float packed) {
+  const f3 rgb = decode_color(packed);
+  return make_uchar4((unsigned char)f2i_rn(rgb.x * 255.0f), (unsigned char)f2i_rn(rgb.y * 255.0f), (unsigned char)f2i_rn(rgb.z * 255.0f), 255);
+}
+__device__ __forceinline__ void resolved_geometry(const ProjArgs& a, const SplatSurfel& s, float z, int px, int py, float4& o_v, float4& o_n) {
+  const float fcx = (float)px + 0.5f, fcy = (float)py + 0.5f;
+  o_v = make_float4(((fcx - a.cx) * z) * (1.f / a.fx), ((fcy - a.cy) * z) * (1.f / a.fy), z, s.conf);
+  o_n = make_float4(s.nrm.x, s.nrm.y, s.nrm.z, s.rad);
+}
+
 template <bool DEPTH_ONLY, bool FILL>
 __global__ __launch_bounds__(256) void k_splat_resolve(ProjArgs a, SurfelPlanes sp, size_t cap, unsigned long long* __restrict__ zbuf,
                                                        uchar4* __restrict__ image, float4* __restrict__ vertex, float4* __restrict__ normal,
@@ -1052,15 +1063,11 @@
       continue;
     }
     const float4 cc = sp.col[i];
-    const f3 rgb = decode_color(cc.x);
-    const uchar4 o_img = make_uchar4((unsigned char)f2i_rn(rgb.x * 255.0f), (unsigned char)f2i_rn(rgb.y * 255.0f),
-                                     (unsigned char)f2i_rn(rgb.z * 255.0f), 255);
+    const uchar4 o_img = resolved_image(cc.x);
     image[p] = o_img;
     if (FILL && sampled && o_img.x > 0 && o_img.y > 0 && o_img.z > 0) atomicAdd(fa.dense_cnt + ((px + py) & 15) * 16, 1u);
-    const float z = c.z;
-    const float fcx = (float)px + 0.5f, fcy = (float)py + 0.5f;
-    const float4 o_v = make_float4(((fcx - a.cx) * z) * (1.f / a.fx), ((fcy - a.cy) * z) * (1.f / a.fy), z, s.conf);
-    const float4 o_n = make_float4(s.nrm.x, s.nrm.y, s.nrm.z, s.rad);
+    float4 o_v, o_n;
+    resolved_geometry(a, s, c.z, px, py, o_v, o_n);
     vertex[p] = o_v;
     normal[p] = o_n;
     const float tz = cc.z;
@@ -1076,11 +1083,107 @@
   }
 }
 
+template <int NT>
+__global__ __launch_bounds__(NT) void k_predict_model(ProjArgs a, SurfelPlanes sp, size_t cap, unsigned long long* __restrict__ zbuf, int clear_after,
+                                                      FillArgs fa, TrackInitArgs ti, PredictModelArgs pm) {
+  if ((int)blockIdx.x < ti.blocks) {
+    track_init_body((int)blockIdx.x, ti.blocks, (int)threadIdx.x, NT, ti.st, ti.prior, ti.prior_pose16, ti.fx, ti.fy, ti.cx, ti.cy, ti.so3, ti.first_level,
+                    ti.sync_words, ti.n_sync, ti.inject_timeout, nullptr);
+    return;
+  }
+  const unsigned b = blockIdx.x - (unsigned)ti.blocks, nres = gridDim.x - (unsigned)ti.blocks;
+  const int lane = threadIdx.x & 63, wave = threadIdx.x >> 6;
+  constexpr int kWaves = NT / 64;
+  __shared__ int s_cnt[kWaves];
+  {
+    int cnt = 0;
+    for (int k = (int)threadIdx.x; k < pm.n_cells; k += NT) {
+      const unsigned long long key = zbuf[pm.sample_cells[k]];
+      if ((unsigned)(key >> 32) < 0xFFFFFFu) {
+        const uchar4 c = resolved_image(sp.col[(unsigned)(key & 0xFFFFFFFFull)].x);
+        cnt += (c.x > 0 && c.y > 0 && c.z > 0) ? 1 : 0;
+      }
+    }
+    for (int off = 32; off > 0; off >>= 1) cnt += __shfl_down(cnt, off, 64);
+    if (lane == 0) s_cnt[wave] = cnt;
+  }
+  __syncthreads();
+  unsigned tot = 0;
+#pragma unroll
+  for (int w = 0; w < kWaves; ++w) tot += (unsigned)s_cnt[w];
+  const bool useB = dense_from_count(tot, pm.samples) != 0;
+  if (b == 0 && threadIdx.x == 0) *pm.flag_out = useB ? 1 : 0;
+  const Pose34 P = load_pose34(pm.pose16);
+  const bool xf = pm.pose16 != nullptr;
+  const int rows0 = a.rows, rows1 = pm.maps.v[1].rows / 3, cols1 = pm.maps.v[1].cols, rows2 = pm.maps.v[2].rows / 3, cols2 = pm.maps.v[2].cols;
+  const int tiles_y = (a.rows + 7) >> 3, tiles_x = (a.cols + 7) >> 3, ntiles = tiles_x * tiles_y;
+  for (int t = xcd_block(b, nres, a.xcd) * kWaves + wave; t < ntiles; t += nres * kWaves) {
+    const int tx = t / tiles_y, ty = t - tx * tiles_y;
+    const int px = tx * 8 + (lane >> 3), py = ty * 8 + (lane & 7);
+    const bool inside = px < a.cols && py < a.rows;
+    f3 rv = mk3(0.f, 0.f, 0.f), rn = mk3(0.f, 0.f, 0.f);
+    if (inside) {
+      const size_t cell = (size_t)px * a.rows + py;
+      const unsigned long long key = zbuf[cell];
+      if (clear_after) {
+        const bool sampled = ((fa.sample_mask[px >> 5] >> (px & 31)) & (fa.sample_mask[64 + (py >> 5)] >> (py & 31)) & 1u) != 0u;
+        if (!sampled) zbuf[cell] = kZClear;
+      }
+      float4 o_v = make_float4(0.f, 0.f, 0.f, 0.f), o_n = make_float4(0.f, 0.f, 0.f, 0.f);
+      uchar4 o_img = make_uchar4(0, 0, 0, 0);
+      if ((unsigned)(key >> 32) < 0xFFFFFFu) {
+        const unsigned i = (unsigned)(key & 0xFFFFFFFFull);
+        SplatSurfel s;
+        splat_vertex(a, sp.pos[i], sp.nrm + i, sp.times[(size_t)a.timeIdx * cap + i], s);
+        f3 c;
+        float zw;
+        splat_fragment(a, s, px, py, c, zw);
+        o_img = resolved_image(sp.col[i].x);
+        resolved_geometry(a, s, c.z, px, py, o_v, o_n);
+      }
+      if (useB) {
+        float4 ov, on;
+        uchar4 oi;
+        fill_pixel_values(fa, px, py, o_v, o_n, o_img, ov, on, oi);
+        o_v = ov;
+        o_n = on;
+        o_img = oi;
+      }
+      model_level0_store(px, py, rows0, o_v, o_n, o_img, P, xf, pm.maps.v[0], pm.maps.n[0], pm.maps.depth0, pm.maps.inten0, pm.maps.cutOff, rv, rn);
+    }
+    f3 qv[4], qn[4], lv, ln;
+#pragma unroll
+    for (int j = 0; j < 4; ++j) {
+      const int src = (lane & ~9) + (j & 1) * 8 + (j >> 1);
+      qv[j] = mk3(__shfl(rv.x, src, 64), __shfl(rv.y, src, 64), __shfl(rv.z, src, 64));
+      qn[j] = mk3(__shfl(rn.x, src, 64), __shfl(rn.y, src, 64), __shfl(rn.z, src, 64));
+    }
+    model_level_down(qv, qn, lv, ln);
+    const int x1 = px >> 1, y1 = py >> 1;
+    if ((lane & 9) == 0 && x1 < cols1 && y1 < rows1) store_transformed(pm.maps.v[1], pm.maps.n[1], rows1, y1, x1, lv, ln, P, xf);
+#pragma unroll
+    for (int j = 0; j < 4; ++j) {
+      const int src = (lane & ~27) + (j & 1) * 16 + (j >> 1) * 2;
+      qv[j] = mk3(__shfl(lv.x, src, 64), __shfl(lv.y, src, 64), __shfl(lv.z, src, 64));
+      qn[j] = mk3(__shfl(ln.x, src, 64), __shfl(ln.y, src, 64), __shfl(ln.z, src, 64));
+    }
+    const int x2 = px >> 2, y2 = py >> 2;
+    if ((lane & 27) == 0 && x2 < cols2 && y2 < rows2) {
+      f3 v2, n2;
+      model_level_down(qv, qn, v2, n2);
+      store_transformed(pm.maps.v[2], pm.maps.n[2], rows2, y2, x2, v2, n2, P, xf);
+    }
+  }
+}
+
 int splat_predict(dms_model* m, const dms_pose_block* pose, const dms_camera* cam, float maxDepth, float confThreshold, int time,
                   int timeIdx, int maxTime, int timeDelta, int active, unsigned long long* zbuf, dms_predict_out* out,
                   dms_image2d* depth_out, int zclean, hipStream_t s, const float* second_conf_time_maxtime, unsigned long long* zbuf2,
-                  int resolve_only, const FillArgs* fill, const TrackInitArgs* init) {
+                  int resolve_only, const FillArgs* fill, const TrackInitArgs* init, const PredictModelArgs* pm) {
   DMS_REQUIRE(m && pose && cam && zbuf, "null argument");
+  DMS_REQUIRE(!pm || (fill && !depth_out && fill->sample_mask && fill->mirror_words == 0 && !fill->thumb_block && zclean && pm->sample_cells && pm->n_cells == pm->samples &&
+                      pm->samples == (m->width / 20) * (m->height / 20) && pm->samples > 0 && pm->flag_out && (pm->threads == 256 || pm->threads == 512 || pm->threads == 1024)),
+              "the fused prediction + model pass takes the place of the fused resolve + fill-in pass of a tracking prediction only");
   DMS_REQUIRE(!init || init->blocks == 0 || (fill && !depth_out), "the tracker set-up rides on the fused resolve + fill-in pass only");
   DMS_REQUIRE(!m->pending_update, "a deferred update pass is still pending (index_map applies it)");
   DMS_REQUIRE(timeIdx >= 0 && timeIdx < DMS_MAX_SENSORS, "timeIdx out of range");
@@ -1124,6 +1227,19 @@
   if (depth_out) {
     hipLaunchKernelGGL((k_splat_resolve<true, false>), rg, dim3(256), 0, s, a, m->buf[m->cur], m->cap, zbuf, (uchar4*)nullptr,
                        (float4*)nullptr, (float4*)nullptr, (unsigned short*)nullptr, (float*)depth_out->data, zclean, no_fill, no_init);
+  } else if (pm) {
+    DMS_REQUIRE(fill->cols == W && fill->rows == H && W <= 2048 && H <= 2048 && pm->maps.v[0].cols == W && pm->maps.v[0].rows == 3 * H &&
+                    pm->maps.v[1].cols == W / 2 && pm->maps.v[1].rows == 3 * (H / 2) && pm->maps.v[2].cols == W / 4 && pm->maps.v[2].rows == 3 * (H / 4),
+                "model maps do not describe this prediction's pyramid");
+    const TrackInitArgs& ti = (init && init->blocks > 0) ? *init : no_init;
+    const int waves = pm->threads / 64, ntiles = ((W + 7) / 8) * ((H + 7) / 8);
+    const dim3 g(ti.blocks + min((ntiles + waves - 1) / waves, 2048));
+    if (pm->threads == 1024)
+      hipLaunchKernelGGL(k_predict_model<1024>, g, dim3(1024), 0, s, a, m->buf[m->cur], m->cap, zbuf, zclean, *fill, ti, *pm);
+    else if (pm->threads == 512)
+      hipLaunchKernelGGL(k_predict_model<512>, g, dim3(512), 0, s, a, m->buf[m->cur], m->cap, zbuf, zclean, *fill, ti, *pm);
+    else
+      hipLaunchKernelGGL(k_predict_model<256>, g, dim3(256), 0, s, a, m->buf[m->cur], m->cap, zbuf, zclean, *fill, ti, *pm);
   } else if (fill) {
     DMS_REQUIRE(fill->ex_image == (const uchar4*)out->image.data && fill->ex_vertex == (const float4*)out->vertex.data &&
                     fill->ex_normal == (const float4*)out->normal.data && fill->cols == W && fill->rows == H &&
diff --git a/densemonoslam_amd/csrc/internal.hpp b/densemonoslam_amd/csrc/internal.hpp
--- a/densemonoslam_amd/csrc/internal.hpp
+++ b/densemonoslam_amd/csrc/internal.hpp
@@ -18,6 +18,21 @@
   const unsigned* copy_src;
   unsigned* copy_dst;
   int copy_words;
+};
+
+struct ModelMapViews {
+  View<float> v[3], n[3], depth0;
+  View<unsigned char> inten0;
+  float cutOff;
+};
+struct PredictModelArgs {
+  ModelMapViews maps;
+  const float* pose16;
+  int* flag_out;
+  const int* sample_cells;
+  int n_cells;
+  int samples;
+  int threads;
 };
 
 int pyrDown(const dms_image2d* src, dms_image2d* dst, hipStream_t s);
@@ -83,7 +98,8 @@
 int splat_predict(dms_model* m, const dms_pose_block* pose, const dms_camera* cam, float maxDepth, float confThreshold, int time,
                   int timeIdx, int maxTime, int timeDelta, int active, unsigned long long* zbuf, dms_predict_out* out,
                   dms_image2d* depth_out, int zclean, hipStream_t s, const float* second_conf_time_maxtime = nullptr,
-                  unsigned long long* zbuf2 = nullptr, int resolve_only = 0, const FillArgs* fill = nullptr, const TrackInitArgs* init = nullptr);
+                  unsigned long long* zbuf2 = nullptr, int resolve_only = 0, const FillArgs* fill = nullptr, const TrackInitArgs* init = nullptr,
+                  const PredictModelArgs* pm = nullptr);
 int splat_project_only(dms_model* m, const dms_pose_block* pose, const dms_camera* cam, float maxDepth, float confThreshold, int time,
                        int timeIdx, int maxTime, int timeDelta, int active, unsigned long long* zbuf, hipStream_t s, const ProjectRider* rider);
 int model_sample_graph(dms_model* m, int sampleRate, float* rows4_host, int max_rows, int* n_host, hipStream_t s);
@@ -116,6 +132,8 @@
 int odometry_initModel_fused(dms_odometry* o, const void* vA, const void* nA, const void* iA, const void* vB, const void* nB,
                              const void* iB, const int* flag_dev, int force_b_img, const float* pose16_dev, hipStream_t s,
                              int defer_last_step = 0, unsigned* dense_cnt = nullptr, int dense_samples = 0, const TrackFold* fold = nullptr);
+int odometry_model_views_begin(dms_odometry* o, const TrackFold* fold, ModelMapViews* mv, TrackInitArgs* ti, unsigned long long* zbuf,
+                               const int* cells, int n_cells);
 int odometry_initLive_fused(dms_odometry* o, const void* verts, const void* norms, const void* rgba, const int* any_flag_dev,
                             hipStream_t s);
 int odometry_enable_ring(dms_odometry* o);
diff --git a/densemonoslam_amd/csrc/model_bodies.hpp b/densemonoslam_amd/csrc/model_bodies.hpp
--- a/densemonoslam_amd/csrc/model_bodies.hpp
+++ b/densemonoslam_amd/csrc/model_bodies.hpp
@@ -66,6 +66,16 @@
   }
 }
 
+__device__ __forceinline__ void model_level0_store(int x, int y, int rows, const float4 v, const float4 q, const uchar4 c, const Pose34& P, bool xf,
+                                                   View<float> vmap, View<float> nmap, View<float> depth, View<unsigned char> inten, float cutOff, f3& rv,
+                                                   f3& rn) {
+  raw_maps(v, q, rv, rn);
+  store_transformed(vmap, nmap, rows, y, x, rv, rn, P, xf);
+  depth.at(y, x) = (v.z > cutOff || v.z <= 0.f) ? qnan() : v.z;
+  const float f = ((float)c.x * 0.114f + (float)c.y * 0.299f) + (float)c.z * 0.587f;
+  inten.at(y, x) = (unsigned char)f2i_rz(f);
+}
+
 __device__ __forceinline__ void model_level0_body(int tx, int ty, int BYv, int bx, int by, const ModelSrc& m, int rows, int cols, View<float> vmap,
                                                   View<float> nmap, View<float> depth, View<unsigned char> inten, float cutOff) {
   const int x = bx * 64 + tx;
@@ -78,11 +88,7 @@
   const uchar4 c = (useB || m.force_b_img) ? m.iB[i] : m.iA[i];
   const Pose34 P = load_pose34(m.pose16);
   f3 rv, rn;
-  raw_maps(v, q, rv, rn);
-  store_transformed(vmap, nmap, rows, y, x, rv, rn, P, m.pose16 != nullptr);
-  depth.at(y, x) = (v.z > cutOff || v.z <= 0.f) ? qnan() : v.z;
-  const float f = ((float)c.x * 0.114f + (float)c.y * 0.299f) + (float)c.z * 0.587f;
-  inten.at(y, x) = (unsigned char)f2i_rz(f);
+  model_level0_store(x, y, rows, v, q, c, P, m.pose16 != nullptr, vmap, nmap, depth, inten, cutOff, rv, rn);
 }
 
 template <bool NORMALIZE>
@@ -94,6 +100,11 @@
   n.z = (a.z + b.z + c.z + d.z) / 4;
   if (NORMALIZE) n = normalized3(n);
   return n;
+}
+
+__device__ __forceinline__ void model_level_down(const f3 (&v)[4], const f3 (&n)[4], f3& lv, f3& ln) {
+  lv = resize4<false>(v[0], v[1], v[2], v[3]);
+  ln = resize4<true>(n[0], n[1], n[2], n[3]);
 }
 
 __device__ __forceinline__ void model_levels12_body(int tx, int ty, int BYv, int bx, int by, const ModelSrc& m, int cols0, int rows1, int cols1, int rows2,
@@ -114,8 +125,7 @@
       const size_t i = (size_t)(2 * y1 + (j >> 1)) * cols0 + (2 * x1 + (j & 1));
       raw_maps(vs[i], ns[i], rv[j], rn[j]);
     }
-    lv = resize4<false>(rv[0], rv[1], rv[2], rv[3]);
-    ln = resize4<true>(rn[0], rn[1], rn[2], rn[3]);
+    model_level_down(rv, rn, lv, ln);
     store_transformed(v1, n1, rows1, y1, x1, lv, ln, P, m.pose16 != nullptr);
   }
   f3 qv[4], qn[4];
@@ -126,22 +136,45 @@
     qn[j] = mk3(__shfl(ln.x, src, 64), __shfl(ln.y, src, 64), __shfl(ln.z, src, 64));
   }
   if (k == 0 && x2 < cols2 && y2 < rows2) {
-    const f3 a = resize4<false>(qv[0], qv[1], qv[2], qv[3]);
-    const f3 b = resize4<true>(qn[0], qn[1], qn[2], qn[3]);
+    f3 a, b;
+    model_level_down(qv, qn, a, b);
     store_transformed(v2, n2, rows2, y2, x2, a, b, P, m.pose16 != nullptr);
   }
 }
 
-template <int BYV>
-__device__ __forceinline__ void model_pyr_step1_body(int tx, int ty, int bx, int by, const ModelSrc& m, int rows0, int cols0, float cutOff, View<float> ddst,
+struct SourceTaps {
+  const float4* vs;
+  const uchar4* is;
+  int cols0;
+  float cutOff;
+  __device__ __forceinline__ SourceTaps(const ModelSrc& m, int cols0_, float cutOff_) : cols0(cols0_), cutOff(cutOff_) {
+    const bool useB = model_use_b(m);
+    vs = useB ? m.vB : m.vA;
+    is = (useB || m.force_b_img) ? m.iB : m.iA;
+  }
+  __device__ __forceinline__ float depth(int gy, int gx) const {
+    const float z = vs[(size_t)gy * cols0 + gx].z;
+    return (z > cutOff || z <= 0.f) ? qnan() : z;
+  }
+  __device__ __forceinline__ unsigned char inten(int gy, int gx) const {
+    const uchar4 cc = is[(size_t)gy * cols0 + gx];
+    return (unsigned char)f2i_rz(((float)cc.x * 0.114f + (float)cc.y * 0.299f) + (float)cc.z * 0.587f);
+  }
+};
+struct PlaneTaps {
+  View<const float> d0;
+  View<const unsigned char> i0;
+  __device__ __forceinline__ float depth(int gy, int gx) const { return d0.at(gy, gx); }
+  __device__ __forceinline__ unsigned char inten(int gy, int gx) const { return i0.at(gy, gx); }
+};
+
+template <int BYV, class Taps>
+__device__ __forceinline__ void model_pyr_step1_taps(int tx, int ty, int bx, int by, const Taps& src, int rows0, int cols0, View<float> ddst,
                                                      View<unsigned char> idst) {
   constexpr int BX = 64, BY = BYV;
   constexpr int TW = 2 * BX + 3, TH = 2 * BY + 3;
   __shared__ float s_d[TH][TW + 1];
   __shared__ unsigned char s_c[TH][TW + 1];
-  const bool useB = model_use_b(m);
-  const float4* vs = useB ? m.vB : m.vA;
-  const uchar4* is = (useB || m.force_b_img) ? m.iB : m.iA;
   const int sx0 = 2 * (bx * BX) - 2, sy0 = 2 * (by * BY) - 2;
   for (int e = ty * BX + tx; e < TH * TW; e += BX * BY) {
     const int r = e / TW, c = e - r * TW;
@@ -149,11 +182,8 @@
     float sv = qnan();
     unsigned char cv = 0;
     if (gx >= 0 && gy >= 0 && gx < cols0 && gy < rows0) {
-      const size_t i = (size_t)gy * cols0 + gx;
-      const float z = vs[i].z;
-      sv = (z > cutOff || z <= 0.f) ? qnan() : z;
-      const uchar4 cc = is[i];
-      cv = (unsigned char)f2i_rz(((float)cc.x * 0.114f + (float)cc.y * 0.299f) + (float)cc.z * 0.587f);
+      sv = src.depth(gy, gx);
+      cv = src.inten(gy, gx);
     }
     s_d[r][c] = sv;
     s_c[r][c] = cv;
@@ -167,19 +197,21 @@
   ddst.at(y, x) = live::float_half(dt, x, y, cols0, rows0);
   idst.at(y, x) = live::u8_half(ct, x, y, cols0, rows0);
 }
-
-template <int NT>
-__device__ __forceinline__ void model_pyr_step2_body(int t, int bx, int by, const ModelSrc& m, int rows0, int cols0, float cutOff, int rows1, int cols1,
-                                                     View<float> ddst2, View<unsigned char> idst2) {
+template <int BYV>
+__device__ __forceinline__ void model_pyr_step1_body(int tx, int ty, int bx, int by, const ModelSrc& m, int rows0, int cols0, float cutOff, View<float> ddst,
+                                                     View<unsigned char> idst) {
+  model_pyr_step1_taps<BYV>(tx, ty, bx, by, SourceTaps(m, cols0, cutOff), rows0, cols0, ddst, idst);
+}
+
+template <int NT, class Taps>
+__device__ __forceinline__ void model_pyr_step2_taps(int t, int bx, int by, const Taps& src, int rows0, int cols0, int rows1, int cols1, View<float> ddst2,
+                                                     View<unsigned char> idst2) {
   constexpr int OX = 16, OY = 8;
   constexpr int W1 = 2 * OX + 3, H1 = 2 * OY + 3, W0 = 2 * W1 + 3, H0 = 2 * H1 + 3;
   __shared__ float s_d0[H0][W0 + 1];
   __shared__ unsigned char s_c0[H0][W0 + 1];
   __shared__ float s_d1[H1][W1 + 1];
   __shared__ unsigned char s_c1[H1][W1 + 1];
-  const bool useB = model_use_b(m);
-  const float4* vs = useB ? m.vB : m.vA;
-  const uchar4* is = (useB || m.force_b_img) ? m.iB : m.iA;
   const int x1o = 2 * (bx * OX) - 2, y1o = 2 * (by * OY) - 2;
   const int x0o = 2 * x1o - 2, y0o = 2 * y1o - 2;
   for (int e = t; e < H0 * W0; e += NT) {
@@ -188,11 +220,8 @@
     float sv = qnan();
     unsigned char cv = 0;
     if (gx >= 0 && gy >= 0 && gx < cols0 && gy < rows0) {
-      const size_t i = (size_t)gy * cols0 + gx;
-      const float z = vs[i].z;
-      sv = (z > cutOff || z <= 0.f) ? qnan() : z;
-      const uchar4 cc = is[i];
-      cv = (unsigned char)f2i_rz(((float)cc.x * 0.114f + (float)cc.y * 0.299f) + (float)cc.z * 0.587f);
+      sv = src.depth(gy, gx);
+      cv = src.inten(gy, gx);
     }
     s_d0[r][c] = sv;
     s_c0[r][c] = cv;
@@ -220,5 +249,10 @@
     idst2.at(y, x) = live::u8_half(ct, x, y, cols1, rows1);
   }
 }
-
-}
+template <int NT>
+__device__ __forceinline__ void model_pyr_step2_body(int t, int bx, int by, const ModelSrc& m, int rows0, int cols0, float cutOff, int rows1, int cols1,
+                                                     View<float> ddst2, View<unsigned char> idst2) {
+  model_pyr_step2_taps<NT>(t, bx, by, SourceTaps(m, cols0, cutOff), rows0, cols0, rows1, cols1, ddst2, idst2);
+}
+
+}
diff --git a/densemonoslam_amd/csrc/track.hip b/densemonoslam_amd/csrc/track.hip
--- a/densemonoslam_amd/csrc/track.hip
+++ b/densemonoslam_amd/csrc/track.hip
@@ -52,6 +52,10 @@
   int last_shape_P[DMS_NUM_PYRS] = {1, 1, 1}, last_shape_nb[DMS_NUM_PYRS] = {0, 0, 0};
   bool deferred_pyr = false;
   bool init_folded = false;
+  bool pyr_from_planes = false;
+  unsigned long long* rider_zbuf = nullptr;
+  const int* rider_cells = nullptr;
+  int rider_n_cells = 0;
   bool early_init = false, so3_in_model = false;
   bool so3_beside_model = false;
   int folded_so3 = 0, folded_first_level = 0;
@@ -1208,7 +1212,16 @@
   View<float> ddst;
   View<const unsigned char> isrc;
   View<unsigned char> idst;
+  int planes, g2x, g2y;
+  View<const float> d0;
+  View<const unsigned char> i0;
+  View<float> ddst2;
+  View<unsigned char> idst2;
+  unsigned long long* zbuf;
+  const int* cells;
+  int n_cells;
 };
+static inline int so3_rider_blocks(const So3Extra& ex) { return ex.planes ? ex.g2x * ex.g2y + ex.gx * ex.gy + 1 : ex.gx * ex.gy; }
 
 struct So3Args {
   const unsigned char* lastImage;
@@ -1345,7 +1358,21 @@
                                                    const unsigned char* nextImage, size_t next_pitch, int cols, int rows,
                                                    unsigned long long* ar, SolveCam cam, int first_gn_level, int max_iter, int exp_bias, int first_delay, So3Extra ex) {
   if ((int)blockIdx.x >= ex.nb_so3) {
-    const int c = (int)blockIdx.x - ex.nb_so3, by = c / ex.gx, bx = c - by * ex.gx;
+    int c = (int)blockIdx.x - ex.nb_so3;
+    if (ex.planes) {
+      const PlaneTaps taps = {ex.d0, ex.i0};
+      const int n2 = ex.g2x * ex.g2y, n1 = ex.gx * ex.gy;
+      if (c < n2) {
+        model_pyr_step2_taps<kPB>((int)threadIdx.x, c % ex.g2x, c / ex.g2x, taps, ex.d0.rows, ex.d0.cols, ex.ddst.rows, ex.ddst.cols, ex.ddst2, ex.idst2);
+      } else if (c < n2 + n1) {
+        c -= n2;
+        model_pyr_step1_taps<kPB / 64>((int)(threadIdx.x & 63), (int)(threadIdx.x >> 6), c % ex.gx, c / ex.gx, taps, ex.d0.rows, ex.d0.cols, ex.ddst, ex.idst);
+      } else {
+        for (int k = (int)threadIdx.x; k < ex.n_cells; k += kPB) ex.zbuf[ex.cells[k]] = kZClear;
+      }
+      return;
+    }
+    const int by = c / ex.gx, bx = c - by * ex.gx;
     model_pyr_step_pixel(bx * 64 + (int)(threadIdx.x & 63), by * (kPB / 64) + (int)(threadIdx.x >> 6), ex.dsrc, ex.ddst, ex.isrc, ex.idst);
     return;
   }
@@ -2101,7 +2128,26 @@
                 "track call differs from the one its folded set-up was prepared for");
     ex.zero16 = o->dense_cnt_zero;
     o->dense_cnt_zero = nullptr;
-    if (o->deferred_pyr) {
+    if (o->pyr_from_planes) {
+      o->pyr_from_planes = false;
+      DMS_REQUIRE(!o->fuse_coarse && !o->deferred_pyr, "the pyramid steps from the level-0 planes ride on the SO3 launch only");
+      dms_image2d d0 = o->lastDepth[0].img(), d1 = o->lastDepth[1].img(), d2 = o->lastDepth[2].img();
+      dms_image2d i0 = o->lastImage[0].img(), i1 = o->lastImage[1].img(), i2 = o->lastImage[2].img();
+      ex.planes = 1;
+      ex.gx = (d1.cols + 63) / 64;
+      ex.gy = (d1.rows + kPB / 64 - 1) / (kPB / 64);
+      ex.g2x = (d2.cols + 15) / 16;
+      ex.g2y = (d2.rows + 7) / 8;
+      ex.d0 = view<const float>(&d0);
+      ex.i0 = view<const unsigned char>(&i0);
+      ex.ddst = view<float>(&d1);
+      ex.idst = view<unsigned char>(&i1);
+      ex.ddst2 = view<float>(&d2);
+      ex.idst2 = view<unsigned char>(&i2);
+      ex.zbuf = o->rider_zbuf;
+      ex.cells = o->rider_cells;
+      ex.n_cells = o->rider_n_cells;
+    } else if (o->deferred_pyr) {
       o->deferred_pyr = false;
       dms_image2d d1 = o->lastDepth[1].img(), d2 = o->lastDepth[2].img(), i1 = o->lastImage[1].img(), i2 = o->lastImage[2].img();
       ex.gx = (d2.cols + 63) / 64;
@@ -2263,7 +2309,7 @@
       StageTimer t(o->clock, s, "so3_level", timed(o));
       SolveCam cam = {o->fx, o->fy, o->cx, o->cy};
       ex.nb_so3 = nbp;
-      hipLaunchKernelGGL(k_so3_level, dim3(nbp + ex.gx * ex.gy), dim3(kPB), 0, s, o->state, (const unsigned char*)li.p, li.pitch,
+      hipLaunchKernelGGL(k_so3_level, dim3(nbp + so3_rider_blocks(ex)), dim3(kPB), 0, s, o->state, (const unsigned char*)li.p, li.pitch,
                          (const unsigned char*)ni.p, ni.pitch, ni.cols, ni.rows, o->ar, cam, first_level, 10, o->exp_bias + o->depth_bias, o->first_delay_for(nbp, 3), ex);
       DMS_CHECK_LAUNCH();
     } else
@@ -2630,6 +2676,53 @@
   return 1;
 }
 
+static void fold_init_args(dms_odometry* o, const TrackFold* fold, TrackInitArgs* ti) {
+  const int it1 = fold->pyramid ? 5 : 0, it2 = fold->pyramid ? 4 : 0;
+  ti->st = o->state;
+  ti->prior_pose16 = fold->prior_pose16;
+  ti->fx = o->fx;
+  ti->fy = o->fy;
+  ti->cx = o->cx;
+  ti->cy = o->cy;
+  ti->so3 = 1;
+  ti->first_level = it2 > 0 ? 2 : (it1 > 0 ? 1 : 0);
+  ti->sync_words = o->ar;
+  ti->n_sync = (int)((size_t)kArSets * kArWords / 2);
+  ti->inject_timeout = (!o->early_init && o->inject_timeouts > 0) ? 1 : 0;
+  if (!o->early_init && o->inject_timeouts > 0) o->inject_timeouts -= 1;
+  ti->blocks = 16;
+  o->init_folded = true;
+  o->folded_so3 = 1;
+  o->folded_first_level = ti->first_level;
+  o->folded_prior = fold->prior_pose16;
+}
+
+int odometry_model_views_begin(dms_odometry* o, const TrackFold* fold, ModelMapViews* mv, TrackInitArgs* ti, unsigned long long* zbuf,
+                               const int* cells, int n_cells) {
+  if (!o || !fold || !mv || !ti || !zbuf || !cells) return 0;
+  if (!o->resident || o->fuse_coarse || o->so3_beside_model || !fold->prior_pose16 || !fold->so3 || fold->interMap || so3_resident_blocks(o) <= 0) return 0;
+  for (int i = 0; i < DMS_NUM_PYRS; ++i) {
+    dms_image2d v = o->vmaps_g_prev[i].img(), n = o->nmaps_g_prev[i].img();
+    mv->v[i] = view<float>(&v);
+    mv->n[i] = view<float>(&n);
+  }
+  dms_image2d d0 = o->lastDepth[0].img(), i0 = o->lastImage[0].img();
+  mv->depth0 = view<float>(&d0);
+  mv->inten0 = view<unsigned char>(&i0);
+  mv->cutOff = o->maxDepthRGB;
+  memset(ti, 0, sizeof(*ti));
+  o->early_init = false;
+  o->so3_in_model = false;
+  o->deferred_pyr = false;
+  o->dense_cnt_zero = nullptr;
+  fold_init_args(o, fold, ti);
+  o->pyr_from_planes = true;
+  o->rider_zbuf = zbuf;
+  o->rider_cells = cells;
+  o->rider_n_cells = n_cells;
+  return 1;
+}
+
 int odometry_initModel_fused(dms_odometry* o, const void* vA, const void* nA, const void* iA, const void* vB, const void* nB,
                              const void* iB, const int* flag_dev, int force_b_img, const float* pose16_dev, hipStream_t s,
                              int defer_last_step, unsigned* dense_cnt, int dense_samples, const TrackFold* fold) {
@@ -2646,26 +2739,8 @@
   TrackInitArgs ti;
   memset(&ti, 0, sizeof(ti));
   o->init_folded = false;
-  if (fold && fold->prior_pose16 && fold->so3 && !fold->interMap && defer_last_step && so3_resident_blocks(o) > 0) {
-    const int it1 = fold->pyramid ? 5 : 0, it2 = fold->pyramid ? 4 : 0;
-    ti.st = o->state;
-    ti.prior_pose16 = fold->prior_pose16;
-    ti.fx = o->fx;
-    ti.fy = o->fy;
-    ti.cx = o->cx;
-    ti.cy = o->cy;
-    ti.so3 = 1;
-    ti.first_level = it2 > 0 ? 2 : (it1 > 0 ? 1 : 0);
-    ti.sync_words = o->ar;
-    ti.n_sync = (int)((size_t)kArSets * kArWords / 2);
-    ti.inject_timeout = (!o->early_init && o->inject_timeouts > 0) ? 1 : 0;
-    if (!o->early_init && o->inject_timeouts > 0) o->inject_timeouts -= 1;
-    ti.blocks = 16;
-    o->init_folded = true;
-    o->folded_so3 = 1;
-    o->folded_first_level = ti.first_level;
-    o->folded_prior = fold->prior_pose16;
-  }
+  o->pyr_from_planes = false;
+  if (fold && fold->prior_pose16 && fold->so3 && !fold->interMap && defer_last_step && so3_resident_blocks(o) > 0) fold_init_args(o, fold, &ti);
   if (o->early_init && o->init_folded) {
     o->init_folded = false;
     o->deferred_pyr = false;
diff --git a/densemonoslam_amd/fusion.py b/densemonoslam_amd/fusion.py
--- a/densemonoslam_amd/fusion.py
+++ b/densemonoslam_amd/fusion.py
@@ -35,7 +35,7 @@
         ("nid_bins_depth", C.c_int), ("nid_pyramid_level", C.c_int),
         ("local_loop_closure", C.c_int), ("reloc", C.c_int), ("num_sensors", C.c_int), ("share_projection", C.c_int),
         ("fused_fill_in", C.c_int), ("hybrid_loops", C.c_int), ("lazy_final_prediction", C.c_int),
-        ("fused_associate", C.c_int),
+        ("fused_associate", C.c_int), ("fused_model_prediction", C.c_int),
     ]
 
 
@@ -121,6 +121,7 @@
 lib.dms_pose_compose.argtypes = [C.POINTER(C.c_float), C.POINTER(C.c_float), C.POINTER(C.c_float)]
 lib.dms_fusion_set_profiling.argtypes = [_P, _I]
 lib.dms_fusion_get_lazy_stats.argtypes = [_P, C.POINTER(C.c_int), C.POINTER(C.c_long), C.POINTER(C.c_long), C.POINTER(C.c_long)]
+lib.dms_fusion_get_predict_stats.argtypes = [_P, C.POINTER(C.c_long), C.POINTER(C.c_long)]
 
 
 class InterMapResult(C.Structure):
@@ -658,6 +659,11 @@
         check(lib.dms_fusion_get_lazy_stats(self.h, C.byref(e), C.byref(d), C.byref(m), C.byref(st)), "dms_fusion_get_lazy_stats")
         return {"eager": bool(e.value), "deferred": int(d.value), "materialised": int(m.value), "stale": int(st.value)}
 
+    def predictStats(self):
+        a, b = C.c_long(0), C.c_long(0)
+        check(lib.dms_fusion_get_predict_stats(self.h, C.byref(a), C.byref(b)), "dms_fusion_get_predict_stats")
+        return {"fused": int(a.value), "plain": int(b.value)}
+
     def loopConstraints(self):
         n = C.c_int(0)
         cap = (self.width // 20) * (self.height // 20)
diff --git a/include/dmslam_fusion.h b/include/dmslam_fusion.h
--- a/include/dmslam_fusion.h
+++ b/include/dmslam_fusion.h
@@ -126,6 +126,7 @@
   int hybrid_loops;
   int lazy_final_prediction;
   int fused_associate;
+  int fused_model_prediction;
 } dms_fusion_params;
 
 void dms_fusion_default_params(dms_fusion_params* p, int width, int height, float fx, float fy, float cx, float cy);
@@ -164,6 +165,7 @@
 int dms_fusion_fetch_loop(dms_fusion* f, dms_frame_result* r, dms_stream s);
 int dms_fusion_process_frame_end(dms_fusion* f, const float* graph_host, int graph_nodes, const float* newPose16, dms_stream s);
 int dms_fusion_get_lazy_stats(dms_fusion* f, int* eager, long* deferred, long* materialised, long* stale);
+int dms_fusion_get_predict_stats(dms_fusion* f, long* fused, long* plain);
 int dms_fusion_debug_keep_assoc_zbuf(dms_fusion* f, int on);
 
 int dms_fusion_set_orb_loop(dms_fusion* f, const float* orbTcwOld16, const float* orbTcwNew16);
```

After: 2846 frames/s, median of 6. 1.02x the previous value.
